# zhaihongjia/SplatLoc

Hardware: AMD Instinct MI355X
Metric: fwd+bwd frames/s @1080p, 500k Gaussians, 32 feat-ch; HBM GB/s vs roofline (higher is better)
Workload: dtype f32

## Files before the change

### include/splatraster.h

```cpp
#ifndef SPLATRASTER_H
#define SPLATRASTER_H

#include <stddef.h>
#include <stdint.h>

#ifdef __cplusplus
extern "C" {
#endif

#define SPLATRASTER_ABI_VERSION 14

#define SPLATRASTER_TILE 16

#define SPLATRASTER_OK 0
#define SPLATRASTER_ERR_BAD_ARG 1
#define SPLATRASTER_ERR_HIP 2
#define SPLATRASTER_ERR_UNSUPPORTED 3
#define SPLATRASTER_ERR_OVERFLOW 4
#define SPLATRASTER_WARN_LOOKBACK_STALL 5

typedef struct splatraster_settings {
    int32_t image_height;
    int32_t image_width;
    float tanfovx;
    float tanfovy;
    float scale_modifier;
    int32_t sh_degree;
    int32_t sh_coeffs;
    int32_t channels;
    int32_t bg_channels;
    int32_t prefiltered;
    int32_t debug;
} splatraster_settings;


size_t splatraster_geometry_bytes(int32_t P);
size_t splatraster_binning_bytes(int32_t P, int64_t R, int32_t width, int32_t height, int32_t channels);
size_t splatraster_image_bytes(int32_t width, int32_t height);


int splatraster_forward_geometry(const splatraster_settings* s, int32_t P,
                                 const float* means3D,
                                 const float* shs,
                                 const float* opacities,
                                 const float* scales,
                                 const float* rotations,
                                 const float* cov3D_precomp,
                                 const float* viewmatrix,
                                 const float* projmatrix,
                                 const float* campos,
                                 void* geometry, int32_t* radii, int64_t* num_rendered,
                                 void* stream);

int splatraster_forward_render(const splatraster_settings* s, int32_t P, int64_t R,
                               const float* bg,
                               const float* colors_precomp,
                               void* geometry, void* binning, void* image,
                               float* out_color, float* out_depth, float* out_alpha,
                               void* stream);


int splatraster_backward(const splatraster_settings* s, int32_t P, int64_t R,
                         const float* bg, const float* means3D, const float* shs,
                         const float* colors_precomp, const float* opacities,
                         const float* scales, const float* rotations,
                         const float* cov3D_precomp, const float* viewmatrix,
                         const float* projmatrix, const float* campos,
                         const int32_t* radii,
                         void* geometry ,
                         const void* binning, const void* image,
                         const float* out_color, const float* out_depth, const float* out_alpha,
                         const float* dL_dout_color,
                         const float* dL_dout_depth,
                         const float* dL_dout_alpha,
                         float* dL_dmeans3D,
                         float* dL_dmeans2D,
                         float* dL_dcolors,
                         float* dL_dopacities,
                         float* dL_dscales,
                         float* dL_drotations,
                         float* dL_dcov3D,
                         float* dL_dshs,
                         float* dL_dviewmatrix,
                         float* dL_dprojmatrix,
                         float* dL_dcampos,
                         void* stream);


#define SPLATRASTER_MAX_WINDOW_VIEWS 8

typedef struct splatraster_window_view {
    const float* viewmatrix;
    const float* projmatrix;
    const float* campos;
    float tanfovx, tanfovy;
    int32_t* radii;
    float* out_color;
    float* out_depth;
    float* out_alpha;
    const float* dL_dout_color;
    const float* dL_dout_depth;
    const float* dL_dout_alpha;
    float* dL_dmeans2D;
    const float* dL_dout_last;
    int32_t color_grad_channels;
} splatraster_window_view;

size_t splatraster_window_geometry_bytes(int32_t P, int32_t n_views);
size_t splatraster_window_binning_bytes(int32_t P, int32_t n_views, int64_t R_total, int32_t width, int32_t height,
                                        int32_t channels);
size_t splatraster_window_image_bytes(int32_t width, int32_t height, int32_t n_views);

int splatraster_forward_window_geometry(const splatraster_settings* s, int32_t n_views,
                                        const splatraster_window_view* views, int32_t P,
                                        const float* means3D, const float* opacities, const float* scales,
                                        const float* rotations, const float* cov3D_precomp, void* geometry,
                                        int64_t* num_rendered , void* stream);
int splatraster_forward_window_render(const splatraster_settings* s, int32_t n_views,
                                      const splatraster_window_view* views, int32_t P,
                                      const int64_t* num_rendered, const float* bg, const float* colors_precomp,
                                      void* geometry, void* binning, void* image, void* stream);
int splatraster_backward_window(const splatraster_settings* s, int32_t n_views, const splatraster_window_view* views,
                                int32_t P, const int64_t* num_rendered, const float* bg, const float* means3D,
                                const float* colors_precomp, const float* scales, const float* rotations,
                                const float* cov3D_precomp, void* geometry, const void* binning, const void* image,
                                float* dL_dmeans3D,
                                float* dL_dcolors,
                                float* dL_dopacities,
                                float* dL_dscales,
                                float* dL_drotations,
                                float* dL_dcov3D,
                                void* stream);

typedef struct splatraster_raw_forward {
    const float* scaling;
    const float* rotation;
    const float* opacity;
    const float* f_dc;
    const float* extra;
    int32_t extra_channels;
    float* scales;
    float* rotations;
    float* opacities;
    float* colors;
} splatraster_raw_forward;
int splatraster_forward_window_geometry_raw(const splatraster_settings* s, int32_t n_views, const splatraster_window_view* views,
                                            int32_t P, const float* means3D, const splatraster_raw_forward* raw, void* geometry,
                                            int64_t* num_rendered , void* stream);

typedef struct splatraster_raw_params {
    const float* scaling;
    const float* rotation;
    const float* opacity;
    const float* f_dc;
    int32_t extra_channels;
    float* dL_dscaling;
    float* dL_drotation;
    float* dL_dopacity;
    float* dL_df_dc;
    float* dL_dextra;
    const float* reg_row_grad;
    const float* reg_out;
    float reg_weight;
// ... 69 lines not shown
                                           float* max_radii2D, void* stream);


typedef struct splatraster_model {
    int32_t P;
    int32_t f_rest_width;
    int32_t marker_width;
    int32_t kp_width;
    int32_t scaling_width;
    float* xyz;
    float* f_dc;
    float* f_rest;
    float* opacity;
    float* marker;
    float* kp_score;
    float* scaling;
    float* rotation;
} splatraster_model;

size_t splatraster_densify_workspace_bytes(int32_t P);
int splatraster_densify_plan(const splatraster_model* model, const float* xyz_gradient_accum ,
                             const float* denom , float max_grad, float min_opacity, float extent,
                             float percent_dense, int32_t use_size_prune, int32_t primitive_reg, void* workspace,
                             int32_t* new_P, void* stream);
int splatraster_densify_apply(const splatraster_model* model, const splatraster_model* exp_avg ,
                              const splatraster_model* exp_avg_sq , const float* unit_noise ,
                              uint64_t seed, uint64_t draw_id, void* workspace , int32_t new_P,
                              splatraster_model* out_model, splatraster_model* out_exp_avg,
                              splatraster_model* out_exp_avg_sq, int32_t* source_row ,
                              int32_t* source_kind ,
                              void* stream);

int splatraster_model_append(const splatraster_model* model, const splatraster_model* exp_avg ,
                             const splatraster_model* exp_avg_sq , const splatraster_model* extra,
                             splatraster_model* out_model, splatraster_model* out_exp_avg,
                             splatraster_model* out_exp_avg_sq, void* stream);

typedef struct splatraster_adam_group {
    float* param;
    const float* grad;
    float* exp_avg;
    float* exp_avg_sq;
    const float* row_gate;
    int64_t numel;
    int32_t row_width;
    float lr;
    double step;
} splatraster_adam_group;
int splatraster_adam_step(int32_t n_groups, const splatraster_adam_group* groups, double beta1, double beta2, double eps,
                          float row_gate_threshold, void* stream);
int splatraster_adam_step_radii(int32_t n_groups, const splatraster_adam_group* groups, double beta1, double beta2, double eps,
                                float row_gate_threshold, int32_t P, const int32_t* radii, float* max_radii2D, void* stream);

size_t splatraster_isotropic_loss_workspace_bytes(int32_t P);
int splatraster_isotropic_loss(int32_t P, int32_t scaling_cols, const float* scaling, const float* marker,
                               float* row_grad , float* out , void* workspace, void* stream);


size_t splatraster_mapping_loss_workspace_bytes(int32_t pixels);
int splatraster_mapping_loss(int32_t pixels, const float* image, const float* depth, const float* marker,
                             const float* gt_image, const float* gt_depth, const float* kp,
                             float rgb_boundary_threshold, const float* exposure ,
                             float* g_image, float* g_depth, float* g_marker, float* out ,
                             void* workspace, void* stream);

typedef struct splatraster_loss_view {
    const float* image;
    const float* depth;
    const float* marker;
    const float* gt_image;
    const float* gt_depth;
    const float* kp;
    const float* exposure;
    float* g_image;
    float* g_depth;
    float* g_marker;
} splatraster_loss_view;
int splatraster_mapping_loss_window(int32_t n_views, int32_t pixels, const splatraster_loss_view* views,
                                    float rgb_boundary_threshold, float* out , void* workspace,
                                    void* stream);

size_t splatraster_refinement_loss_workspace_bytes(int32_t channels, int32_t height, int32_t width);
int splatraster_refinement_loss(int32_t channels, int32_t height, int32_t width, float lambda_dssim,
                                const float* image, const float* gt, float* g_image, float* out ,
                                void* workspace, void* stream);

size_t splatraster_eval_metrics_workspace_bytes(int32_t channels, int32_t height, int32_t width);
int splatraster_eval_metrics(int32_t channels, int32_t height, int32_t width, const float* render, const float* gt,
                             float* out , void* workspace, void* stream);


size_t splatknn_workspace_bytes(int32_t N);
int splatknn_dist2(int32_t N, const float* points , float* out ,
                   void* workspace, void* stream);

int splatknn_debug_set_grid_min(int32_t n);

#define SPLATRASTER_GRID_MAX_LEVELS 32
#define SPLATRASTER_GRID_HASH 0
#define SPLATRASTER_GRID_DENSE 1
#define SPLATRASTER_GRID_TILED 2
typedef struct splatraster_grid_layout {
    int32_t n_dims;
    int32_t n_levels;
    int32_t n_features;
    int32_t grid_type;
    uint32_t offset[SPLATRASTER_GRID_MAX_LEVELS];
    uint32_t size[SPLATRASTER_GRID_MAX_LEVELS];
    uint32_t resolution[SPLATRASTER_GRID_MAX_LEVELS];
    float scale[SPLATRASTER_GRID_MAX_LEVELS];
    int64_t n_params;
} splatraster_grid_layout;

int splatraster_grid_encoding_layout(int32_t n_dims, int32_t n_levels, int32_t n_features, int32_t log2_hashmap_size,
                                     int32_t base_resolution, double per_level_scale, int32_t grid_type,
                                     splatraster_grid_layout* out);
int splatraster_grid_encoding_forward(const splatraster_grid_layout* layout, int64_t N, const float* x, const float* params,
                                      float* out, void* stream);
int splatraster_grid_encoding_backward(const splatraster_grid_layout* layout, int64_t N, const float* x, const float* params,
                                       const float* dL_dout, float* dL_dparams, float* dL_dx, void* stream);

int splatraster_l1_rgbd_loss(int64_t n_color, const float* color, const float* target_color, int64_t n_depth, const float* depth,
                             const float* target_depth, float depth_weight, float* g_color, float* g_depth, float* loss_out,
                             void* stream);
int splatraster_pose_step(const float* dL_dviewmatrix, const float* dL_dprojmatrix, const float* dL_dcampos, const float* W2C_init,
                          const float* projection_matrix, float lr_rot, float lr_trans, float beta1, float beta2, float eps,
                          int advance, float* state, float* viewmatrix, float* projmatrix, float* campos, void* stream);


#define SPLATRASTER_STAGE_PREPROCESS 0
#define SPLATRASTER_STAGE_DEPTH_SORT 1
#define SPLATRASTER_STAGE_SCAN 2
#define SPLATRASTER_STAGE_EMIT 3
#define SPLATRASTER_STAGE_TILE_SORT 4
#define SPLATRASTER_STAGE_RANGES 5
#define SPLATRASTER_STAGE_COMPOSITE_FWD 6
#define SPLATRASTER_STAGE_COMPOSITE_BWD 7
#define SPLATRASTER_STAGE_PREPROCESS_BWD 8
#define SPLATRASTER_STAGE_PAYLOAD 9
#define SPLATRASTER_STAGE_COUNT 10

int splatraster_timing_enable(int on);
int splatraster_timing_select(uint32_t stage_mask);
int splatraster_timing_collect(double* ms, int64_t* counts);


int splatraster_poll_errors(void);
int splatraster_debug_set_spin_limit(uint32_t limit);
int splatraster_debug_set_deterministic(int on);
int splatraster_debug_set_small_panel_max_waves(int waves);
int splatraster_debug_set_split_max_waves(int waves);
int splatraster_debug_set_fwd_team(int mode);
int splatraster_debug_set_payload_stream_min(int64_t instances);
int splatraster_debug_set_front_end(int mode);
int splatraster_debug_set_tile_sort_cap(int keys);
int splatraster_debug_set_sort_fork(int mode);
int splatraster_debug_exp2(int64_t n, const float* x, float* y, void* stream);
int splatraster_debug_poison_lds(uint32_t pattern, void* stream);

const char* splatraster_error_string(int status);
const char* splatraster_last_hip_error(void);
int splatraster_abi_version(void);

#ifdef __cplusplus
}
#endif
#endif
```

### splatloc_amd/_native.py

```python
from __future__ import annotations

import ctypes as C
import os

from . import build as _build

_LIB = None
ABI_VERSION = 14

OK = 0
WARN_LOOKBACK_STALL = 5
_ERR_NAMES = {1: "bad argument", 2: "HIP runtime error", 3: "unsupported configuration",
              4: "tile instance count overflow", 5: "look-back stall (results late, never wrong)"}


class Settings(C.Structure):
    _fields_ = [
        ("image_height", C.c_int32),
        ("image_width", C.c_int32),
        ("tanfovx", C.c_float),
        ("tanfovy", C.c_float),
        ("scale_modifier", C.c_float),
        ("sh_degree", C.c_int32),
        ("sh_coeffs", C.c_int32),
        ("channels", C.c_int32),
        ("bg_channels", C.c_int32),
        ("prefiltered", C.c_int32),
        ("debug", C.c_int32),
    ]


MAX_WINDOW_VIEWS = 8


class WindowView(C.Structure):
    _fields_ = [("viewmatrix", C.c_void_p), ("projmatrix", C.c_void_p), ("campos", C.c_void_p),
                ("tanfovx", C.c_float), ("tanfovy", C.c_float),
                ("radii", C.c_void_p), ("out_color", C.c_void_p), ("out_depth", C.c_void_p), ("out_alpha", C.c_void_p),
                ("dL_dout_color", C.c_void_p), ("dL_dout_depth", C.c_void_p), ("dL_dout_alpha", C.c_void_p),
                ("dL_dmeans2D", C.c_void_p), ("dL_dout_last", C.c_void_p), ("color_grad_channels", C.c_int32)]


class LossView(C.Structure):
    _fields_ = [(n, C.c_void_p) for n in ("image", "depth", "marker", "gt_image", "gt_depth", "kp", "exposure", "g_image", "g_depth",
                                          "g_marker")]


class RawParams(C.Structure):
    _fields_ = [("scaling", C.c_void_p), ("rotation", C.c_void_p), ("opacity", C.c_void_p), ("f_dc", C.c_void_p),
                ("extra_channels", C.c_int32), ("dL_dscaling", C.c_void_p), ("dL_drotation", C.c_void_p), ("dL_dopacity", C.c_void_p),
                ("dL_df_dc", C.c_void_p), ("dL_dextra", C.c_void_p), ("reg_row_grad", C.c_void_p), ("reg_out", C.c_void_p),
                ("reg_weight", C.c_float)]


class RawForward(C.Structure):
    _fields_ = [("scaling", C.c_void_p), ("rotation", C.c_void_p), ("opacity", C.c_void_p), ("f_dc", C.c_void_p), ("extra", C.c_void_p),
                ("extra_channels", C.c_int32), ("scales", C.c_void_p), ("rotations", C.c_void_p), ("opacities", C.c_void_p),
                ("colors", C.c_void_p)]


class GeometryLayout(C.Structure):
    _fields_ = [(n, C.c_size_t) for n in
                ("rec0", "rec1", "tiles_touched", "depth_order", "offsets", "rgb", "clamped", "total")]


class BinningLayout(C.Structure):
    _fields_ = [(n, C.c_size_t) for n in ("point_list", "tile_list", "ranges", "total")]


class ImageLayout(C.Structure):
    _fields_ = [(n, C.c_size_t) for n in ("final_T", "n_contrib", "total")]


class Model(C.Structure):
    _fields_ = [("P", C.c_int32), ("f_rest_width", C.c_int32), ("marker_width", C.c_int32), ("kp_width", C.c_int32),
                ("scaling_width", C.c_int32)] + [(n, C.c_void_p) for n in
                                                 ("xyz", "f_dc", "f_rest", "opacity", "marker", "kp_score", "scaling",
                                                  "rotation")]


class AdamGroup(C.Structure):
    _fields_ = [("param", C.c_void_p), ("grad", C.c_void_p), ("exp_avg", C.c_void_p), ("exp_avg_sq", C.c_void_p),
                ("row_gate", C.c_void_p), ("numel", C.c_int64), ("row_width", C.c_int32), ("lr", C.c_float),
                ("step", C.c_double)]


GRID_MAX_LEVELS = 32
GRID_HASH, GRID_DENSE, GRID_TILED = 0, 1, 2


class GridLayout(C.Structure):
    _fields_ = [("n_dims", C.c_int32), ("n_levels", C.c_int32), ("n_features", C.c_int32), ("grid_type", C.c_int32),
                ("offset", C.c_uint32 * GRID_MAX_LEVELS), ("size", C.c_uint32 * GRID_MAX_LEVELS),
                ("resolution", C.c_uint32 * GRID_MAX_LEVELS), ("scale", C.c_float * GRID_MAX_LEVELS), ("n_params", C.c_int64)]


_vp, _i32, _i64, _sz = C.c_void_p, C.c_int32, C.c_int64, C.c_size_t
SYMBOLS = {
    "splatraster_geometry_bytes": (_sz, [_i32]),
    "splatraster_binning_bytes": (_sz, [_i32, _i64, _i32, _i32, _i32]),
    "splatraster_image_bytes": (_sz, [_i32, _i32]),
    "splatraster_forward_geometry": (C.c_int, [C.POINTER(Settings), _i32] + [_vp] * 9 + [_vp, _vp, C.POINTER(_i64), _vp]),
    "splatraster_forward_render": (C.c_int, [C.POINTER(Settings), _i32, _i64] + [_vp] * 9),
    "splatraster_backward": (C.c_int, [C.POINTER(Settings), _i32, _i64] + [_vp] * 33),
    "splatraster_window_geometry_bytes": (_sz, [_i32, _i32]),
    "splatraster_window_binning_bytes": (_sz, [_i32, _i32, _i64, _i32, _i32, _i32]),
    "splatraster_window_image_bytes": (_sz, [_i32, _i32, _i32]),
    "splatraster_forward_window_geometry": (C.c_int, [C.POINTER(Settings), _i32, C.POINTER(WindowView), _i32] + [_vp] * 6
                                            + [C.POINTER(_i64), _vp]),
    "splatraster_forward_window_render": (C.c_int, [C.POINTER(Settings), _i32, C.POINTER(WindowView), _i32, C.POINTER(_i64)]
                                          + [_vp] * 6),
    "splatraster_backward_window": (C.c_int, [C.POINTER(Settings), _i32, C.POINTER(WindowView), _i32, C.POINTER(_i64)]
                                    + [_vp] * 16),
    "splatraster_forward_window_geometry_raw": (C.c_int, [C.POINTER(Settings), _i32, C.POINTER(WindowView), _i32, _vp, C.POINTER(RawForward),
                                                          _vp, C.POINTER(_i64), _vp]),
    "splatraster_backward_window_raw": (C.c_int, [C.POINTER(Settings), _i32, C.POINTER(WindowView), _i32, C.POINTER(_i64)]
                                        + [_vp] * 8 + [C.POINTER(RawParams)] + [_vp] * 2),
    "splatraster_get_window_geometry_layout": (C.c_int, [_i32, _i32, C.POINTER(GeometryLayout)]),
    "splatraster_get_window_binning_layout": (C.c_int, [_i32, _i32, _i64, _i32, _i32, _i32, C.POINTER(BinningLayout)]),
    "splatraster_get_window_image_layout": (C.c_int, [_i32, _i32, _i32, C.POINTER(ImageLayout)]),
    "splatraster_debug_set_small_panel_max_waves": (C.c_int, [C.c_int]),
    "splatraster_debug_set_split_max_waves": (C.c_int, [C.c_int]),
    "splatraster_debug_set_fwd_team": (C.c_int, [C.c_int]),
    "splatraster_debug_set_front_end": (C.c_int, [C.c_int]),
    "splatraster_debug_set_tile_sort_cap": (C.c_int, [C.c_int]),
    "splatraster_debug_set_sort_fork": (C.c_int, [C.c_int]),
    "splatraster_debug_set_payload_stream_min": (C.c_int, [C.c_int64]),
    "splatraster_mark_visible": (C.c_int, [_i32, _vp, _vp, _vp, _vp, _vp]),
    "splatraster_get_geometry_layout": (C.c_int, [_i32, C.POINTER(GeometryLayout)]),
    "splatraster_get_binning_layout": (C.c_int, [_i32, _i64, _i32, _i32, _i32, C.POINTER(BinningLayout)]),
    "splatraster_get_image_layout": (C.c_int, [_i32, _i32, C.POINTER(ImageLayout)]),
    "splatraster_sort_tmp_bytes": (_sz, [_i64]),
    "splatraster_sort_pairs_u32": (C.c_int, [_i64, _vp, _vp, _i32, _vp, _vp]),
    "splatraster_timing_enable": (C.c_int, [C.c_int]),
    "splatraster_timing_select": (C.c_int, [C.c_uint32]),
    "splatraster_timing_collect": (C.c_int, [_vp, _vp]),
    "splatknn_workspace_bytes": (_sz, [_i32]),
    "splatknn_dist2": (C.c_int, [_i32, _vp, _vp, _vp, _vp]),
    "splatknn_debug_set_grid_min": (C.c_int, [_i32]),
    "splatraster_grid_encoding_layout": (C.c_int, [_i32] * 5 + [C.c_double, _i32, C.POINTER(GridLayout)]),
    "splatraster_grid_encoding_forward": (C.c_int, [C.POINTER(GridLayout), _i64, _vp, _vp, _vp, _vp]),
    "splatraster_grid_encoding_backward": (C.c_int, [C.POINTER(GridLayout), _i64] + [_vp] * 6),
    "splatraster_activate_forward": (C.c_int, [_i32] * 5 + [_vp] * 13),
    "splatraster_activate_backward": (C.c_int, [_i32] * 5 + [_vp] * 19),
    "splatraster_densification_stats": (C.c_int, [_i32] + [_vp] * 6),
    "splatraster_densification_stats_window": (C.c_int, [_i32, _i32] + [_vp] * 6),
    "splatraster_densify_workspace_bytes": (_sz, [_i32]),
    "splatraster_densify_plan": (C.c_int, [C.POINTER(Model), _vp, _vp, C.c_float, C.c_float, C.c_float, C.c_float, _i32,
                                           _i32, _vp, C.POINTER(_i32), _vp]),
    "splatraster_densify_apply": (C.c_int, [C.POINTER(Model), C.POINTER(Model), C.POINTER(Model), _vp, C.c_uint64,
                                            C.c_uint64, _vp, _i32, C.POINTER(Model), C.POINTER(Model), C.POINTER(Model),
                                            _vp, _vp, _vp]),
    "splatraster_model_append": (C.c_int, [C.POINTER(Model)] * 7 + [_vp]),
    "splatraster_adam_step": (C.c_int, [_i32, C.POINTER(AdamGroup), C.c_double, C.c_double, C.c_double, C.c_float, _vp]),
    "splatraster_adam_step_radii": (C.c_int, [_i32, C.POINTER(AdamGroup), C.c_double, C.c_double, C.c_double, C.c_float, _i32, _vp, _vp, _vp]),
    "splatraster_isotropic_loss_workspace_bytes": (_sz, [_i32]),
    "splatraster_isotropic_loss": (C.c_int, [_i32, _i32, _vp, _vp, _vp, _vp, _vp, _vp]),
    "splatraster_mapping_loss_workspace_bytes": (_sz, [_i32]),
    "splatraster_mapping_loss": (C.c_int, [_i32] + [_vp] * 6 + [C.c_float] + [_vp] * 7),
    "splatraster_mapping_loss_window": (C.c_int, [_i32, _i32, _vp, C.c_float, _vp, _vp, _vp]),
    "splatraster_refinement_loss_workspace_bytes": (_sz, [_i32, _i32, _i32]),
    "splatraster_refinement_loss": (C.c_int, [_i32, _i32, _i32, C.c_float] + [_vp] * 6),
    "splatraster_eval_metrics_workspace_bytes": (_sz, [_i32, _i32, _i32]),
    "splatraster_eval_metrics": (C.c_int, [_i32, _i32, _i32] + [_vp] * 5),
    "splatraster_l1_rgbd_loss": (C.c_int, [_i64, _vp, _vp, _i64, _vp, _vp, C.c_float, _vp, _vp, _vp, _vp]),
    "splatraster_pose_step": (C.c_int, [_vp] * 5 + [C.c_float] * 5 + [C.c_int] + [_vp] * 5),
    "splatraster_error_string": (C.c_char_p, [C.c_int]),
    "splatraster_last_hip_error": (C.c_char_p, []),
    "splatraster_abi_version": (C.c_int, []),
    "splatraster_poll_errors": (C.c_int, []),
    "splatraster_debug_set_spin_limit": (C.c_int, [C.c_uint32]),
    "splatraster_debug_set_deterministic": (C.c_int, [C.c_int]),
    "splatraster_debug_exp2": (C.c_int, [_i64, _vp, _vp, _vp]),
    "splatraster_debug_poison_lds": (C.c_int, [C.c_uint32, _vp]),
}


def lib_path() -> str:
    return _build.LIB_PATH


def load(build_if_missing: bool = True):
    global _LIB
    if _LIB is not None:
        return _LIB
    path = os.environ.get("SPLATRASTER_LIB", _build.LIB_PATH)
    if path == _build.LIB_PATH and build_if_missing and _build.have_hipcc():
        try:
            _build.build()
        except Exception as e:
            raise RuntimeError(
                "splatloc_amd: the HIP extension libsplatraster.so could not be built "
                f"({e}). There is no CPU fallback.") from e
    if not os.path.exists(path):
        raise RuntimeError(f"{path} is missing and hipcc is not available: run `python -m splatloc_amd.build` "
                           "on a machine with ROCm. There is no CPU fallback.")
    lib = C.CDLL(path)
    lib.splatraster_abi_version.restype = C.c_int
    got = int(lib.splatraster_abi_version())
    if got != ABI_VERSION:
        raise RuntimeError(f"{path} has ABI version {got}, this binding needs {ABI_VERSION}: stale library, "
                           "rebuild with `python -m splatloc_amd.build --force`")
    for name, (res, args) in SYMBOLS.items():
        fn = getattr(lib, name)
        fn.restype = res
        fn.argtypes = args
    _LIB = lib
    if os.environ.get("SPLATRASTER_SPLIT_MAX_WAVES"):
        lib.splatraster_debug_set_split_max_waves(int(os.environ["SPLATRASTER_SPLIT_MAX_WAVES"]))
    if os.environ.get("SPLATRASTER_FWD_TEAM"):
        lib.splatraster_debug_set_fwd_team(int(os.environ["SPLATRASTER_FWD_TEAM"]))
    if os.environ.get("SPLATRASTER_FRONT_END"):
        lib.splatraster_debug_set_front_end(int(os.environ["SPLATRASTER_FRONT_END"]))
    if os.environ.get("SPLATRASTER_TILE_SORT_CAP"):
        lib.splatraster_debug_set_tile_sort_cap(int(os.environ["SPLATRASTER_TILE_SORT_CAP"]))
    if os.environ.get("SPLATRASTER_SORT_FORK"):
        lib.splatraster_debug_set_sort_fork(int(os.environ["SPLATRASTER_SORT_FORK"]))
    if os.environ.get("SPLATRASTER_SMALL_PANEL_MAX_WAVES"):
        lib.splatraster_debug_set_small_panel_max_waves(int(os.environ["SPLATRASTER_SMALL_PANEL_MAX_WAVES"]))
    return lib


def check(status: int, what: str) -> None:
    if status != OK:
        lib = load()
        detail = lib.splatraster_last_hip_error().decode() if status in (2, 5) else ""
        raise RuntimeError(f"{what} failed: {_ERR_NAMES.get(status, status)} {detail}".strip())


STAGES = ("preprocess", "depth_sort", "scan", "emit", "tile_sort", "ranges", "composite_fwd", "composite_bwd",
          "preprocess_bwd", "payload")


def timing_enable(on: bool) -> None:
    check(load().splatraster_timing_enable(int(on)), "timing_enable")


def timing_select(stages) -> None:
    mask = 0
    for st in stages:
        mask |= 1 << STAGES.index(st)
    check(load().splatraster_timing_select(mask), "timing_select")


def timing_collect() -> dict:
    n = len(STAGES)
    ms = (C.c_double * n)()
    cnt = (C.c_int64 * n)()
    check(load().splatraster_timing_collect(ms, cnt), "timing_collect")
    return {s: (ms[i], cnt[i]) for i, s in enumerate(STAGES)}


def set_deterministic(on: bool) -> None:
    check(load().splatraster_debug_set_deterministic(int(bool(on))), "set_deterministic")


def set_front_end(mode: int) -> None:
    check(load().splatraster_debug_set_front_end(int(mode)), "set_front_end")


def poll_stall() -> bool:
    st = load().splatraster_poll_errors()
    if st == WARN_LOOKBACK_STALL:
        return True
    check(st, "poll_errors")
    return False
```

### splatloc_amd/csrc/binning.hip

```cpp
#include "tile_order.h"
#include "composite_common.h"

namespace sr {

__device__ __forceinline__ int f2i_sat_b(float v)
{
    if (!(v > -1.0e9f)) v = -1.0e9f;
    if (!(v < 1.0e9f)) v = 1.0e9f;
    return (int)v;
}

constexpr int EMIT_BLOCK = 256;
constexpr int EMIT_IPT = 4;
static_assert(EMIT_SPAN == EMIT_BLOCK * EMIT_IPT, "common.h: EMIT_SPAN");

__global__ void __launch_bounds__(EMIT_BLOCK)
emit_kernel(int64_t R, int P , int Pv , int tiles_per_view, int W, int H,
            const uint32_t* __restrict__ offsets,
            const uint32_t* __restrict__ depth_order, const float4* __restrict__ rec,
            uint32_t* __restrict__ keys, uint32_t* __restrict__ vals,
            const uint32_t* __restrict__ span_owner ,
            uint32_t* __restrict__ ranges, uint32_t nranges )
{
    for (uint32_t w = blockIdx.x * blockDim.x + threadIdx.x; w < nranges; w += gridDim.x * blockDim.x) ranges[w] = 0u;
    __shared__ uint32_t s_off[EMIT_SPAN + 1];
    __shared__ uint32_t s_gid[EMIT_SPAN], s_org[EMIT_SPAN], s_w[EMIT_SPAN];
    __shared__ int s_min;
    const int t = threadIdx.x;
    const int64_t j0 = (int64_t)blockIdx.x * EMIT_SPAN;
    const uint32_t j0u = (uint32_t)j0;
    int lo = 0, hi = P;
    if (span_owner && blockIdx.x < SPAN_OWNER_CAP) {
        lo = (int)span_owner[blockIdx.x];
        hi = lo + 1;
    }
    while (hi - lo > 1) {
        const int n = hi - lo;
        const int step = (n + EMIT_BLOCK - 1) / EMIT_BLOCK;
        if (t == 0) s_min = EMIT_BLOCK;
        __syncthreads();
        const int last = lo + (t + 1) * step - 1;
        if (last >= hi - 1 || offsets[last] > j0u) atomicMin(&s_min, t);
        __syncthreads();
        const int seg = s_min;
        __syncthreads();
        lo = lo + seg * step;
        hi = min(hi, lo + step);
    }
    const int r_lo = lo;
    for (int q = t; q <= EMIT_SPAN; q += EMIT_BLOCK) {
        const int r = r_lo - 1 + q;
        s_off[q] = r < 0 ? 0u : offsets[min(r, P - 1)];
    }
    __syncthreads();
    const int gx = (W + TILE - 1) / TILE, gy = (H + TILE - 1) / TILE;
    const uint32_t j_last = (uint32_t)(min(R, j0 + (int64_t)EMIT_SPAN) - 1);
    int nr;
    {
        int a = 1, b = EMIT_SPAN + 1;
        while (a < b) {
            const int mid = (a + b) >> 1;
            if (s_off[mid] > j_last) b = mid; else a = mid + 1;
        }
        nr = a;
    }
    for (int q = t; q < nr; q += EMIT_BLOCK) {
        const uint32_t g = depth_order[r_lo + q] & 0xFFFFFFu;
        const float4 p = rec[2 * g];
        const float rf = p.w;
        const int rminx = min(gx, max(0, f2i_sat_b((p.x - rf) / (float)TILE)));
        const int rminy = min(gy, max(0, f2i_sat_b((p.y - rf) / (float)TILE)));
        const int rmaxx = min(gx, max(0, f2i_sat_b((p.x + rf + (float)(TILE - 1)) / (float)TILE)));
        s_gid[q] = g;
        const uint32_t v = (P == Pv) ? 0u : g / (uint32_t)Pv;
        s_org[q] = v * (uint32_t)tiles_per_view + (uint32_t)rminy * (uint32_t)gx + (uint32_t)rminx;
        s_w[q] = (uint32_t)(rmaxx - rminx);
    }
    __syncthreads();
#pragma unroll
    for (int it = 0; it < EMIT_IPT; ++it) {
        const int64_t j = j0 + it * EMIT_BLOCK + t;
        if (j < R) {
            const uint32_t ju = (uint32_t)j;
            int a = 1, b = nr + 1;
            while (a < b) {
                const int mid = (a + b) >> 1;
                if (s_off[mid] > ju) b = mid; else a = mid + 1;
            }
            const uint32_t k = ju - s_off[a - 1];
            const uint32_t w = s_w[a - 1];
            const uint32_t row = k / w;
            keys[j] = s_org[a - 1] + row * (uint32_t)gx + (k - row * w);
            vals[j] = s_gid[a - 1];
        }
    }
}

int launch_emit(const splatraster_settings& s, int32_t P, int32_t V, int64_t R, const GeomView& g, uint32_t* keys,
                uint32_t* vals, uint32_t* ranges, uint32_t nranges, hipStream_t stream)
{
    if (R == 0) return SPLATRASTER_OK;
    const int64_t blocks = (R + EMIT_SPAN - 1) / EMIT_SPAN;
    const int n = P * V;
    const int tiles = ((s.image_width + TILE - 1) / TILE) * ((s.image_height + TILE - 1) / TILE);
    hipLaunchKernelGGL(emit_kernel, dim3((unsigned)blocks), dim3(EMIT_BLOCK), 0, stream, R, n, P, tiles, s.image_width,
                       s.image_height, g.offsets, g.depth_order, g.rec, keys, vals,
                       scan_state_bytes(n) ? g.span_owner : nullptr, ranges, nranges);
    SR_LAUNCH_CHECK();
    return SPLATRASTER_OK;
}

int launch_ranges_clear(int32_t tiles, uint32_t* ranges, hipStream_t stream)
{
    SR_HIP_CHECK(hipMemsetAsync(ranges, 0, sizeof(uint32_t) * 2 * (size_t)tiles, stream));
    return SPLATRASTER_OK;
}

#ifndef SR_PAYLOAD_NT_MIN
#define SR_PAYLOAD_NT_MIN (8ll << 20)
#endif
static int64_t g_payload_stream_min = SR_PAYLOAD_NT_MIN;
void set_payload_stream_min(int64_t instances) { g_payload_stream_min = instances < 0 ? (int64_t)SR_PAYLOAD_NT_MIN : instances; }

template <bool NT>
__global__ void __launch_bounds__(256)
payload_kernel(int64_t R, int gx, int tiles_per_view, int V, const uint32_t* __restrict__ point_list,
               const uint32_t* __restrict__ tile_list, const float4* __restrict__ rec,
               float4* __restrict__ irec, uint32_t* __restrict__ ipack, uint32_t* __restrict__ ranges)
{
    const int64_t j = (int64_t)blockIdx.x * blockDim.x + threadIdx.x;
    if (j >= R) return;
    const uint32_t g = point_list[j], t = tile_list[j];
    const float4 a0 = rec[2 * (size_t)g], a1 = rec[2 * (size_t)g + 1];
    uint32_t tl = t;
#pragma unroll 1
    for (int v = 1; v < V && tl >= (uint32_t)tiles_per_view; ++v) tl -= (uint32_t)tiles_per_view;
    const uint32_t ty = tl / (uint32_t)gx, tx = tl - ty * (uint32_t)gx;
    const float4 c1 = payload_conic(a1);
    const uint32_t m = g | (quadrant_reach_mask(a0, a1, (float)(tx * TILE), (float)(ty * TILE)) << 24);
    if (NT) {
        typedef float f32x4_t __attribute__((ext_vector_type(4)));
        f32x4_t* out = reinterpret_cast<f32x4_t*>(irec) + 2 * j;
        __builtin_nontemporal_store((f32x4_t){a0.x, a0.y, a0.z, a0.w}, out);
        __builtin_nontemporal_store((f32x4_t){c1.x, c1.y, c1.z, c1.w}, out + 1);
        __builtin_nontemporal_store(m, ipack + j);
    } else {
        irec[2 * j] = a0;
        irec[2 * j + 1] = c1;
        ipack[j] = m;
    }
    if (j == 0 || tile_list[j - 1] != t) ranges[2 * t] = (uint32_t)j;
    if (j == R - 1 || tile_list[j + 1] != t) ranges[2 * t + 1] = (uint32_t)(j + 1);
}

int launch_payload(const splatraster_settings& s, int32_t V, int64_t R, const GeomView& g, const BinView& b, hipStream_t stream)
{
    if (R == 0) return SPLATRASTER_OK;
    const int gx = (s.image_width + TILE - 1) / TILE, gy = (s.image_height + TILE - 1) / TILE;
    if (R >= g_payload_stream_min)
        hipLaunchKernelGGL(payload_kernel<true>, dim3((unsigned)((R + 255) / 256)), dim3(256), 0, stream, R, gx, gx * gy, V,
                           b.point_list, b.tile_list, g.rec, b.irec, b.ipack, b.ranges);
    else
        hipLaunchKernelGGL(payload_kernel<false>, dim3((unsigned)((R + 255) / 256)), dim3(256), 0, stream, R, gx, gx * gy, V,
                           b.point_list, b.tile_list, g.rec, b.irec, b.ipack, b.ranges);
    SR_LAUNCH_CHECK();
    return SPLATRASTER_OK;
}

__global__ void __launch_bounds__(ORDER_THREADS)
tile_order_kernel(int T, const uint32_t* __restrict__ ranges, uint32_t* __restrict__ order, uint32_t* __restrict__ nparts)
{
    __shared__ uint32_t s_cnt[ORDER_BUCKETS];
    __shared__ uint32_t s_wsum[ORDER_THREADS / WAVE];
    tile_order_block(T, [&](int i) { return ranges[2 * i + 1] - ranges[2 * i]; }, order, s_cnt, s_wsum, nparts);
}

int launch_tile_order(const splatraster_settings& s, int32_t V, const BinView& b, hipStream_t stream)
{
    const int gx = (s.image_width + TILE - 1) / TILE, gy = (s.image_height + TILE - 1) / TILE;
    if (!use_tile_order(V, gx * gy)) return SPLATRASTER_OK;
    hipLaunchKernelGGL(tile_order_kernel, dim3(1), dim3(ORDER_THREADS), 0, stream, V * gx * gy, b.ranges, b.tile_order, b.nparts);
    SR_LAUNCH_CHECK();
    return SPLATRASTER_OK;
}

__global__ void __launch_bounds__(256)
pad_features_kernel(int64_t n4 , int C, int PPR, const float* __restrict__ feat,
                    float4* __restrict__ featp4)
{
    const int64_t e = (int64_t)blockIdx.x * blockDim.x + threadIdx.x;
    if (e >= n4) return;
    const int64_t row = e / PPR;
    const int c = (int)(e - row * PPR) * 4;
    const float* src = feat + row * C + c;
    float4 v;
    v.x = src[0];
    v.y = c + 1 < C ? src[1] : 0.0f;
    v.z = c + 2 < C ? src[2] : 0.0f;
    v.w = c + 3 < C ? src[3] : 0.0f;
    featp4[e] = v;
}

int launch_pad_features(int32_t P, int C, const float* feat, float* featp, hipStream_t stream)
{
    const int CP = padded_channels(C);
    const int64_t n4 = (int64_t)P * CP / 4;
    if (n4 == 0 || CP == C) return SPLATRASTER_OK;
    hipLaunchKernelGGL(pad_features_kernel, dim3((unsigned)((n4 + 255) / 256)), dim3(256), 0, stream, n4, C, CP / 4,
                       feat, reinterpret_cast<float4*>(featp));
    SR_LAUNCH_CHECK();
    return SPLATRASTER_OK;
}

}
```

### splatloc_amd/csrc/capi.hip

```cpp
#include <string.h>

#include <mutex>
#include <unordered_map>
#include <string>
#include <vector>

#include "common.h"

namespace sr {

static thread_local std::string g_last_error;
static int g_deterministic = 0;
static int g_split_max_waves = SPLIT_MAX_WAVES;
void set_split_max_waves(int waves) { g_split_max_waves = waves < 0 ? SPLIT_MAX_WAVES : (waves > SPLIT_MAX_WAVES ? SPLIT_MAX_WAVES : waves); }
int split_max_waves() { return g_split_max_waves; }

void set_hip_error(hipError_t e, const char* what)
{
    g_last_error = std::string(what) + ": " + hipGetErrorString(e);
}

void set_error_text(const char* text) { g_last_error = text; }

struct StageRec { int stage; hipEvent_t a, b; };
static uint32_t g_timing_mask = 0;
static std::mutex g_timing_mu;
static std::vector<StageRec> g_recs;
static std::vector<hipEvent_t> g_pool;

static hipEvent_t get_event()
{
    if (!g_pool.empty()) { hipEvent_t e = g_pool.back(); g_pool.pop_back(); return e; }
    hipEvent_t e = nullptr;
    if (hipEventCreate(&e) != hipSuccess) return nullptr;
    return e;
}

struct StageTimer {
    hipStream_t stream;
    StageRec rec{};
    bool on;
    StageTimer(int stage, hipStream_t s) : stream(s), on((g_timing_mask >> stage) & 1u)
    {
        if (!on) return;
        std::lock_guard<std::mutex> lk(g_timing_mu);
        rec.stage = stage; rec.a = get_event(); rec.b = get_event();
        if (!rec.a || !rec.b) { on = false; return; }
        (void)hipEventRecord(rec.a, stream);
    }
    ~StageTimer()
    {
        if (!on) return;
        (void)hipEventRecord(rec.b, stream);
        std::lock_guard<std::mutex> lk(g_timing_mu);
        g_recs.push_back(rec);
    }
};

struct HostSlot {
    uint32_t* p = nullptr;
    uint32_t* dp = nullptr;
    size_t cap = 0;
    hipEvent_t ev = nullptr;
    int device = -1;
};
static thread_local HostSlot t_slot;

static int host_slot(size_t n, HostSlot** out)
{
    HostSlot& s = t_slot;
    int dev = 0;
    SR_HIP_CHECK(hipGetDevice(&dev));
    if (s.cap < n) {
        if (s.p) (void)hipHostFree(s.p);
        s.p = nullptr;
        s.dp = nullptr;
        s.cap = 0;
        const size_t cap = n < 4096 ? 4096 : n + n / 2;
        SR_HIP_CHECK(hipHostMalloc(reinterpret_cast<void**>(&s.p), sizeof(uint32_t) * cap, hipHostMallocMapped | hipHostMallocPortable | hipHostMallocCoherent));
        SR_HIP_CHECK(hipHostGetDevicePointer(reinterpret_cast<void**>(&s.dp), s.p, 0));
        s.cap = cap;
    }
    if (!s.ev || s.device != dev) {
        if (s.ev) (void)hipEventDestroy(s.ev);
        s.ev = nullptr;
        SR_HIP_CHECK(hipEventCreateWithFlags(&s.ev, hipEventDisableTiming));
        s.device = dev;
    }
    *out = &s;
    return SPLATRASTER_OK;
}

static inline int tile_bits(int tiles)
{
    int b = 1;
    while ((1 << b) < tiles) ++b;
    return b;
}

struct GeomLayout {
    size_t rec0, rec1, tiles_touched, depth_order, offsets, rgb, clamped, sort_keys, keys_alt, vals_alt,
        sort_tmp, scan_tmp, total, block_tiles, span_owner, bytes;
};
static GeomLayout geom_layout(int32_t P, int32_t V)
{
    const size_t p1 = (size_t)(P > 0 ? P : 1);
    const size_t n = p1 * (size_t)(V > 0 ? V : 1);
    GeomLayout L;
    size_t o = 0;
    auto take = [&](size_t bytes) { size_t at = o; o = align_up(o + bytes, 256); return at; };
    L.rec0 = take(32 * n);
    L.rec1 = L.rec0 + 16;
    L.tiles_touched = take(4 * n);
    L.depth_order = take(4 * n);
    L.offsets = take(4 * n);
    L.rgb = take(12 * p1);
    L.clamped = take(3 * p1);
    L.sort_keys = take(4 * n);
    L.keys_alt = take(4 * n);
    L.vals_alt = take(4 * n);
    L.sort_tmp = take(sort_tmp_bytes((int64_t)n));
    L.scan_tmp = take(scan_tmp_bytes((int64_t)n));
    L.total = take(16);
    L.block_tiles = take(4 * (size_t)preprocess_blocks((int32_t)p1) * (size_t)(V > 0 ? V : 1));
    L.span_owner = take(4 * (size_t)SPAN_OWNER_CAP);
    L.bytes = o;
    return L;
}

GeomView geom_view(void* base, int32_t P, int32_t V)
{
    const GeomLayout L = geom_layout(P, V);
    char* b = reinterpret_cast<char*>(base);
    GeomView g;
    g.rec = reinterpret_cast<float4*>(b + L.rec0);
    g.tiles_touched = reinterpret_cast<uint32_t*>(b + L.tiles_touched);
    g.depth_order = reinterpret_cast<uint32_t*>(b + L.depth_order);
    g.offsets = reinterpret_cast<uint32_t*>(b + L.offsets);
    g.rgb = reinterpret_cast<float*>(b + L.rgb);
    g.clamped = reinterpret_cast<uint8_t*>(b + L.clamped);
    g.sort_keys = reinterpret_cast<uint32_t*>(b + L.sort_keys);
    g.sort_tmp = reinterpret_cast<uint32_t*>(b + L.sort_tmp);
    g.total = reinterpret_cast<uint32_t*>(b + L.total);
    g.block_tiles = reinterpret_cast<uint32_t*>(b + L.block_tiles);
    g.span_owner = reinterpret_cast<uint32_t*>(b + L.span_owner);
    return g;
}

struct BinLayout {
    size_t keysA, valsA, keysB, valsB, ranges, sort_tmp, irec, ipack, featp, gacc, pose_acc, ckpt, tile_order, nparts, bytes;
};
static BinLayout bin_layout(int32_t P, int32_t V, int64_t R, int32_t W, int32_t H, int32_t C)
{
    const size_t n = (size_t)(R > 0 ? R : 1);
    const size_t nv = (size_t)(V > 0 ? V : 1);
    const size_t tiles = (size_t)((W + TILE - 1) / TILE) * (size_t)((H + TILE - 1) / TILE) * nv;
    BinLayout L;
    size_t o = 0;
    auto take = [&](size_t bytes) { size_t at = o; o = align_up(o + bytes, 256); return at; };
    L.valsA = take(4 * n);
    L.keysA = take(4 * n);
    L.keysB = take(4 * n);
    L.valsB = take(4 * n);
    L.ranges = take(8 * (tiles > 0 ? tiles : 1));
    L.sort_tmp = take(sort_tmp_bytes((int64_t)n));
    L.irec = take(32 * n);
    L.ipack = take(4 * n);
    L.featp = take((C % 4) ? (size_t)(P > 0 ? P : 1) * padded_channels(C) * sizeof(float) : 16);
    L.gacc = take((size_t)(P > 0 ? P : 1) * nv * gacc_row_floats(C) * sizeof(float));
    L.pose_acc = take(POSE_ACC_BYTES);
    const bool ck = C <= 4 && 4 * (size_t)tiles <= (size_t)SPLIT_MAX_WAVES;
    L.ckpt = take(ck ? nv * (size_t)SPLIT_PARTS_MAX * (size_t)(C + 2) * (size_t)W * (size_t)H * sizeof(float) : 16);
    L.tile_order = take(4 * (tiles > 0 ? tiles : 1));
    L.nparts = take(4 * (tiles > 0 ? tiles : 1));
    L.bytes = o;
    return L;
}

BinView bin_view(void* base, int32_t P, int32_t V, int64_t R, int32_t W, int32_t H, int32_t C)
{
    const BinLayout L = bin_layout(P, V, R, W, H, C);
    char* b = reinterpret_cast<char*>(base);
    BinView v;
    v.point_list = reinterpret_cast<uint32_t*>(b + L.valsA);
    v.tile_list = reinterpret_cast<uint32_t*>(b + L.keysA);
    v.keys_tmp = reinterpret_cast<uint32_t*>(b + L.keysB);
    v.vals_tmp = reinterpret_cast<uint32_t*>(b + L.valsB);
    v.ranges = reinterpret_cast<uint32_t*>(b + L.ranges);
    v.sort_tmp = b + L.sort_tmp;
    v.irec = reinterpret_cast<float4*>(b + L.irec);
    v.ipack = reinterpret_cast<uint32_t*>(b + L.ipack);
    v.featp = reinterpret_cast<float*>(b + L.featp);
    v.gacc = reinterpret_cast<float*>(b + L.gacc);
    v.pose_acc = reinterpret_cast<float*>(b + L.pose_acc);
    v.ckpt = reinterpret_cast<float*>(b + L.ckpt);
    v.tile_order = reinterpret_cast<uint32_t*>(b + L.tile_order);
    v.nparts = reinterpret_cast<uint32_t*>(b + L.nparts);
    return v;
}

static size_t img_plane_bytes(int32_t W, int32_t H, int32_t V)
{
    return align_up((size_t)W * H * 4 * (size_t)(V > 0 ? V : 1), 256);
}

ImgView img_view(void* base, int32_t W, int32_t H, int32_t V)
{
    char* b = reinterpret_cast<char*>(base);
    ImgView v;
    v.final_T = reinterpret_cast<float*>(b);
    v.n_contrib = reinterpret_cast<uint32_t*>(b + img_plane_bytes(W, H, V));
    return v;
}

static int check_row_index_range(int32_t P, int32_t V, int32_t C)
{
    const uint64_t row = (uint64_t)(gacc_row_floats(C) > padded_channels(C) ? gacc_row_floats(C) : padded_channels(C));
    const uint64_t n = (uint64_t)P * (uint64_t)V;
    if (n > (1ull << 24) || n * row >= (1ull << 32)) return SPLATRASTER_ERR_UNSUPPORTED;
    return SPLATRASTER_OK;
}

static int check_settings(const splatraster_settings* s)
{
    if (!s) return SPLATRASTER_ERR_BAD_ARG;
    if (s->image_width <= 0 || s->image_height <= 0 || s->channels <= 0) return SPLATRASTER_ERR_BAD_ARG;
    if (s->bg_channels < 0) return SPLATRASTER_ERR_BAD_ARG;
    return SPLATRASTER_OK;
}

}

using namespace sr;

extern "C" {

int splatraster_abi_version(void) { return SPLATRASTER_ABI_VERSION; }

const char* splatraster_error_string(int status)
{
    switch (status) {
        case SPLATRASTER_OK: return "ok";
        case SPLATRASTER_ERR_BAD_ARG: return "bad argument";
        case SPLATRASTER_ERR_HIP: return "HIP runtime error";
        case SPLATRASTER_ERR_UNSUPPORTED: return "unsupported configuration";
        case SPLATRASTER_ERR_OVERFLOW: return "tile instance count overflow";
        case SPLATRASTER_WARN_LOOKBACK_STALL: return "look-back stall (results late, never wrong)";
        default: return "unknown status";
    }
}

const char* splatraster_last_hip_error(void) { return g_last_error.c_str(); }

size_t splatraster_geometry_bytes(int32_t P) { return geom_layout(P, 1).bytes; }
size_t splatraster_binning_bytes(int32_t P, int64_t R, int32_t width, int32_t height, int32_t channels)
{
    return bin_layout(P, 1, R, width, height, channels).bytes;
}
size_t splatraster_image_bytes(int32_t width, int32_t height) { return 2 * img_plane_bytes(width, height, 1); }

size_t splatraster_window_geometry_bytes(int32_t P, int32_t n_views) { return geom_layout(P, n_views).bytes; }
size_t splatraster_window_binning_bytes(int32_t P, int32_t n_views, int64_t R_total, int32_t width, int32_t height,
                                        int32_t channels)
{
    return bin_layout(P, n_views, R_total, width, height, channels).bytes;
}
size_t splatraster_window_image_bytes(int32_t width, int32_t height, int32_t n_views)
{
    return 2 * img_plane_bytes(width, height, n_views);
}

int splatraster_get_geometry_layout(int32_t P, splatraster_geometry_layout* out)
{
    return splatraster_get_window_geometry_layout(P, 1, out);
}
int splatraster_get_window_geometry_layout(int32_t P, int32_t n_views, splatraster_geometry_layout* out)
{
    if (!out || n_views < 1 || n_views > MAX_VIEWS) return SPLATRASTER_ERR_BAD_ARG;
    const GeomLayout L = geom_layout(P, n_views);
    out->rec0 = L.rec0; out->rec1 = L.rec1; out->tiles_touched = L.tiles_touched;
    out->depth_order = L.depth_order; out->offsets = L.offsets; out->rgb = L.rgb;
    out->clamped = L.clamped; out->total = L.bytes;
    return SPLATRASTER_OK;
}
int splatraster_get_binning_layout(int32_t P, int64_t R, int32_t width, int32_t height, int32_t channels,
                                   splatraster_binning_layout* out)
{
    return splatraster_get_window_binning_layout(P, 1, R, width, height, channels, out);
}
int splatraster_get_window_binning_layout(int32_t P, int32_t n_views, int64_t R_total, int32_t width, int32_t height,
                                          int32_t channels, splatraster_binning_layout* out)
{
    if (!out || n_views < 1 || n_views > MAX_VIEWS) return SPLATRASTER_ERR_BAD_ARG;
    const BinLayout L = bin_layout(P, n_views, R_total, width, height, channels);
    out->point_list = L.valsA; out->tile_list = L.keysA; out->ranges = L.ranges; out->total = L.bytes;
    return SPLATRASTER_OK;
}
int splatraster_get_image_layout(int32_t width, int32_t height, splatraster_image_layout* out)
{
    return splatraster_get_window_image_layout(width, height, 1, out);
}
int splatraster_get_window_image_layout(int32_t width, int32_t height, int32_t n_views, splatraster_image_layout* out)
{
    if (!out || n_views < 1 || n_views > MAX_VIEWS) return SPLATRASTER_ERR_BAD_ARG;
    out->final_T = 0;
    out->n_contrib = img_plane_bytes(width, height, n_views);
    out->total = 2 * img_plane_bytes(width, height, n_views);
    return SPLATRASTER_OK;
}

}

namespace sr {

static int check_window(const splatraster_settings* s, int32_t V, const splatraster_window_view* views)
{
    int st = check_settings(s);
    if (st) return st;
    if (V < 1 || V > MAX_VIEWS || !views) return SPLATRASTER_ERR_BAD_ARG;
    return SPLATRASTER_OK;
}

static WinCams make_cams(int32_t V, const splatraster_window_view* views)
{
    WinCams c{};
    for (int v = 0; v < V; ++v) {
        c.view[v] = views[v].viewmatrix;
        c.proj[v] = views[v].projmatrix;
        c.campos[v] = views[v].campos;
        c.tanfovx[v] = views[v].tanfovx;
        c.tanfovy[v] = views[v].tanfovy;
        c.radii[v] = views[v].radii;
    }
    return c;
}

struct BinScratch { bool on; uint32_t* table; void* scan_tmp; int64_t entries; };

static std::mutex g_front_end_mu;
static std::unordered_map<const void*, bool> g_front_end;
static void front_end_record(const void* geometry, bool on)
{
    std::lock_guard<std::mutex> lk(g_front_end_mu);
    if (g_front_end.size() > (1u << 14)) g_front_end.clear();
    g_front_end[geometry] = on;
}
static int front_end_recorded(const void* geometry)
{
    std::lock_guard<std::mutex> lk(g_front_end_mu);
    auto it = g_front_end.find(geometry);
    return it == g_front_end.end() ? -1 : (it->second ? 1 : 0);
}

static BinScratch bin_scratch(const splatraster_settings& s, int32_t P, int32_t V, void* geometry, bool geometry_stage)
{
    const int gx = (s.image_width + TILE - 1) / TILE, gy = (s.image_height + TILE - 1) / TILE, tiles = gx * gy;
    const GeomLayout L = geom_layout(P, V);
    BinScratch b{};
    if (!geometry || P <= 0) return b;
    const int recorded = geometry_stage ? -1 : front_end_recorded(geometry);
    b.on = recorded >= 0 ? recorded == 1 : use_bins(P, V, gx, gy, L.total - L.sort_keys);
    if (geometry_stage) front_end_record(geometry, b.on);
    if (!b.on) return b;
    char* base = reinterpret_cast<char*>(geometry);
    b.entries = (int64_t)bin_table_entries(P, V, tiles);
    b.table = reinterpret_cast<uint32_t*>(base + L.sort_keys);
    b.scan_tmp = base + L.sort_keys + align_up((size_t)b.entries * sizeof(uint32_t), 256);
    return b;
}

static int window_geometry(const splatraster_settings* s, int32_t V, const splatraster_window_view* views, int32_t P,
                           const float* means3D, const float* shs, const float* opacities, const float* scales,
                           const float* rotations, const float* cov3D_precomp, void* geometry, int64_t* num_rendered,
                           hipStream_t stream, const RawFwd* raw = nullptr)
{
    int st = check_window(s, V, views);
    if (st) return st;
    if (P < 0 || !num_rendered) return SPLATRASTER_ERR_BAD_ARG;
    for (int v = 0; v < V; ++v) num_rendered[v] = 0;
    if (P == 0) return SPLATRASTER_OK;
    if (raw) {
        if (shs || cov3D_precomp || !raw->scaling || !raw->rotation || !raw->opacity || !raw->f_dc || !raw->scales || !raw->rotations ||
            !raw->opacities || !raw->colors || raw->E != s->channels - 3 || (raw->E > 0 && !raw->extra))
            return SPLATRASTER_ERR_BAD_ARG;
        opacities = raw->opacities; scales = raw->scales; rotations = raw->rotations;
    }
    if (!means3D || !opacities || !geometry) return SPLATRASTER_ERR_BAD_ARG;
    for (int v = 0; v < V; ++v)
        if (!views[v].viewmatrix || !views[v].projmatrix || !views[v].radii) return SPLATRASTER_ERR_BAD_ARG;
    const bool have_sr = scales && rotations;
    if (have_sr == (cov3D_precomp != nullptr)) return SPLATRASTER_ERR_BAD_ARG;
    if ((scales == nullptr) != (rotations == nullptr)) return SPLATRASTER_ERR_BAD_ARG;
    if (shs) {
        if (V != 1) return SPLATRASTER_ERR_UNSUPPORTED;
        if (s->channels != 3 || !views[0].campos) return SPLATRASTER_ERR_BAD_ARG;
        if (s->sh_degree < 0 || s->sh_degree > 3) return SPLATRASTER_ERR_UNSUPPORTED;
        if (s->sh_coeffs < (s->sh_degree + 1) * (s->sh_degree + 1)) return SPLATRASTER_ERR_BAD_ARG;
    }
    if ((int64_t)P * V >= ((int64_t)1 << 31)) return SPLATRASTER_ERR_OVERFLOW;
    st = check_row_index_range(P, V, s->channels);
    if (st) return st;
    st = lookback_error_init();
    if (st) return st;
    const int32_t n = P * V;
    const GeomLayout L = geom_layout(P, V);
    GeomView g = geom_view(geometry, P, V);
    char* base = reinterpret_cast<char*>(geometry);
    const WinCams cams = make_cams(V, views);
    const BinScratch bins = bin_scratch(*s, P, V, geometry, true);
    HostSlot* slot = nullptr;
    const size_t nblk = (size_t)preprocess_blocks(P);
    st = host_slot(nblk * (size_t)V, &slot);
    if (st) return st;
    g.block_tiles = slot->dp;
    struct SlotGuard {
        HostSlot* slot; hipStream_t stream; int state;
        ~SlotGuard() { if (state == 2) (void)hipEventSynchronize(slot->ev); else if (state == 1) (void)hipStreamSynchronize(stream); }
    } guard{slot, stream, 1};
    {
        StageTimer t(SPLATRASTER_STAGE_PREPROCESS, stream);
        if (bins.on)
            st = launch_preprocess(*s, P, V, cams, means3D, shs, opacities, scales, rotations, cov3D_precomp, g, nullptr, 0u,
                                   reinterpret_cast<uint32_t*>(bins.scan_tmp), (uint32_t)(scan_state_bytes(bins.entries) / 4),
                                   stream, false, raw);
        else
            st = launch_preprocess(*s, P, V, cams, means3D, shs, opacities, scales, rotations, cov3D_precomp, g,
                                   g.sort_tmp, (uint32_t)(sort_zero_bytes(n, 32) / 4),
                                   reinterpret_cast<uint32_t*>(base + L.scan_tmp), (uint32_t)(scan_state_bytes(n) / 4), stream, true, raw);
    }
    if (st) return st;
    SR_HIP_CHECK(hipEventRecord(slot->ev, stream));
    guard.state = 2;
    if (bins.on) {
        StageTimer t(SPLATRASTER_STAGE_DEPTH_SORT, stream);
        st = launch_bin_count(*s, P, V, g, bins.table, bins.scan_tmp, stream);
        if (st) return st;
    } else {
    {
        StageTimer t(SPLATRASTER_STAGE_DEPTH_SORT, stream);
        bool in_alt = false;
        uint32_t* keys_alt = reinterpret_cast<uint32_t*>(base + L.keys_alt);
        uint32_t* vals_alt = reinterpret_cast<uint32_t*>(base + L.vals_alt);
        st = sort_pairs_u32(n, g.sort_keys, g.depth_order, keys_alt, vals_alt, 32, g.sort_tmp, stream, &in_alt, true);
        if (st) return st;
        if (in_alt) return SPLATRASTER_ERR_UNSUPPORTED;
    }
    {
        StageTimer t(SPLATRASTER_STAGE_SCAN, stream);
        st = inclusive_scan_u32(n, g.tiles_touched, g.depth_order, g.offsets, g.total, base + L.scan_tmp, stream, true,
                                g.span_owner, (uint32_t)EMIT_SPAN, SPAN_OWNER_CAP);
    }
    if (st) return st;
    }
    SR_HIP_CHECK(hipEventSynchronize(slot->ev));
    guard.state = 0;
    uint64_t total = 0;
    for (int v = 0; v < V; ++v) {
        uint64_t tv = 0;
        for (size_t k = 0; k < nblk; ++k) tv += slot->p[(size_t)v * nblk + k];
        num_rendered[v] = (int64_t)tv;
        total += tv;
    }
    if (total >= ((uint64_t)1 << 31)) return SPLATRASTER_ERR_OVERFLOW;
    return SPLATRASTER_OK;
}

static int window_render(const splatraster_settings* s, int32_t V, const splatraster_window_view* views, int32_t P,
                         int64_t R, const float* bg, const float* colors_precomp, void* geometry, void* binning,
                         void* image, hipStream_t stream)
{
    int st = check_window(s, V, views);
    if (st) return st;
    if (P < 0 || R < 0 || !image) return SPLATRASTER_ERR_BAD_ARG;
    for (int v = 0; v < V; ++v)
        if (!views[v].out_color || !views[v].out_depth || !views[v].out_alpha) return SPLATRASTER_ERR_BAD_ARG;
    if (s->bg_channels > 0 && !bg) return SPLATRASTER_ERR_BAD_ARG;
    if (P > 0 && (!geometry || !binning)) return SPLATRASTER_ERR_BAD_ARG;
    if (V > 1 && !colors_precomp && P > 0) return SPLATRASTER_ERR_UNSUPPORTED;
    st = check_row_index_range(P, V, s->channels);
    if (st) return st;
    if (!binning) return SPLATRASTER_ERR_BAD_ARG;
    const int W = s->image_width, H = s->image_height;
    const int tiles = ((W + TILE - 1) / TILE) * ((H + TILE - 1) / TILE);
    const int64_t gtiles = (int64_t)tiles * V;
    if (gtiles >= ((int64_t)1 << 31)) return SPLATRASTER_ERR_OVERFLOW;
    ImgView im = img_view(image, W, H, V);
    GeomView g{};
    if (geometry) g = geom_view(geometry, P, V);
    BinView b = bin_view(binning, P, V, R, W, H, s->channels);
    const float* feat = colors_precomp ? colors_precomp : g.rgb;
    if (R > 0 && !feat) return SPLATRASTER_ERR_BAD_ARG;
    const int bits = tile_bits((int)gtiles);
    const int passes = (bits + 7) / 8;
    uint32_t* k0 = (passes & 1) ? b.keys_tmp : b.tile_list;
    uint32_t* v0 = (passes & 1) ? b.vals_tmp : b.point_list;
    uint32_t* k1 = (passes & 1) ? b.tile_list : b.keys_tmp;
    uint32_t* v1 = (passes & 1) ? b.point_list : b.vals_tmp;
    const BinScratch bins = bin_scratch(*s, P, V, geometry, false);
    if (R > 0 && bins.on) {
        StageTimer t(SPLATRASTER_STAGE_TILE_SORT, stream);
        st = launch_bin_scatter_sort(*s, P, V, R, g, bins.table, b, reinterpret_cast<uint64_t*>(b.keys_tmp), stream);
        if (st) return st;
    }
    if (R > 0 && !bins.on) {
        {
            StageTimer t(SPLATRASTER_STAGE_EMIT, stream);
            st = launch_emit(*s, P, V, R, g, k0, v0, b.ranges, 2u * (uint32_t)gtiles, stream);
        }
        if (st) return st;
        bool in_alt = false;
        {
            StageTimer t(SPLATRASTER_STAGE_TILE_SORT, stream);
            st = sort_pairs_u32(R, k0, v0, k1, v1, bits, b.sort_tmp, stream, &in_alt);
        }
        if (st) return st;
    }
    if (R == 0) {
        StageTimer t(SPLATRASTER_STAGE_RANGES, stream);
        st = launch_ranges_clear((int32_t)gtiles, b.ranges, stream);
    }
    if (st) return st;
    const float* featp = feat;
    if (R > 0) {
        StageTimer t(SPLATRASTER_STAGE_PAYLOAD, stream);
        if (!bins.on) st = launch_payload(*s, V, R, g, b, stream);
        if (st) return st;
        if (s->channels % 4) {
            st = launch_pad_features(P, s->channels, feat, b.featp, stream);
            featp = b.featp;
        }
    }
    if (st) return st;
    if (!(R > 0 && bins.on)) {
        StageTimer t(SPLATRASTER_STAGE_RANGES, stream);
        st = launch_tile_order(*s, V, b, stream);
    }
    if (st) return st;
    WinOut outs{};
    for (int v = 0; v < V; ++v) {
        outs.color[v] = views[v].out_color;
        outs.depth[v] = views[v].out_depth;
        outs.alpha[v] = views[v].out_alpha;
    }
    StageTimer t(SPLATRASTER_STAGE_COMPOSITE_FWD, stream);
    return launch_composite_fwd(*s, P, V, R, g, b, im, featp, bg, outs, stream);
}

static int window_backward(const splatraster_settings* s, int32_t V, const splatraster_window_view* views, int32_t P,
                           int64_t R, const float* bg, const float* means3D, const float* shs, const float* colors_precomp,
                           const float* scales, const float* rotations, const float* cov3D_precomp, void* geometry,
                           const void* binning, const void* image, float* dL_dmeans3D, float* dL_dcolors,
                           float* dL_dopacities, float* dL_dscales, float* dL_drotations, float* dL_dcov3D,
                           float* dL_dshs, float* dL_dviewmatrix, float* dL_dprojmatrix, float* dL_dcampos,
                           hipStream_t stream, const RawBwd* raw = nullptr)
{
    int st = check_window(s, V, views);
    if (st) return st;
    if (P < 0 || R < 0) return SPLATRASTER_ERR_BAD_ARG;
    if (V > 1 && (shs || dL_dviewmatrix || dL_dprojmatrix || dL_dcampos)) return SPLATRASTER_ERR_UNSUPPORTED;
    if (raw && (shs || cov3D_precomp || dL_dviewmatrix || dL_dprojmatrix || dL_dcampos)) return SPLATRASTER_ERR_UNSUPPORTED;
    if (P == 0) {
        if (dL_dviewmatrix) SR_HIP_CHECK(hipMemsetAsync(dL_dviewmatrix, 0, 16 * sizeof(float), stream));
        if (dL_dprojmatrix) SR_HIP_CHECK(hipMemsetAsync(dL_dprojmatrix, 0, 16 * sizeof(float), stream));
        if (dL_dcampos) SR_HIP_CHECK(hipMemsetAsync(dL_dcampos, 0, 3 * sizeof(float), stream));
        return SPLATRASTER_OK;
    }
    if (!means3D || !geometry || !binning || !image || !dL_dmeans3D || (!dL_dopacities && !raw)) return SPLATRASTER_ERR_BAD_ARG;
    if (raw && (P > 0) && (!raw->scaling || !raw->rotation || !raw->opacity || !raw->f_dc || !raw->d_scaling || !raw->d_rotation ||
                           !raw->d_opacity || !raw->d_f_dc || raw->E != s->channels - 3 || (raw->E > 0 && !raw->d_extra)))
        return SPLATRASTER_ERR_BAD_ARG;
    for (int v = 0; v < V; ++v)
        if (!views[v].viewmatrix || !views[v].projmatrix || !views[v].radii || !views[v].out_color || !views[v].out_depth ||
            !views[v].dL_dout_color || !views[v].dL_dmeans2D)
            return SPLATRASTER_ERR_BAD_ARG;
    if (shs && (!dL_dshs || !views[0].campos)) return SPLATRASTER_ERR_BAD_ARG;
    if (!shs && (!colors_precomp || (!dL_dcolors && !raw))) return SPLATRASTER_ERR_BAD_ARG;
    if (cov3D_precomp ? !dL_dcov3D : (!scales || !rotations || ((!dL_dscales || !dL_drotations) && !raw)))
        return SPLATRASTER_ERR_BAD_ARG;
    st = check_row_index_range(P, V, s->channels);
    if (st) return st;
    const int W = s->image_width, H = s->image_height;
    GeomView g = geom_view(geometry, P, V);
    BinView b = bin_view(const_cast<void*>(binning), P, V, R, W, H, s->channels);
    ImgView im = img_view(const_cast<void*>(image), W, H, V);
    const int C = s->channels;
    const float* feat = shs ? g.rgb : colors_precomp;
    const WinCams cams = make_cams(V, views);
    WinGrad grads{};
    grads.gc = C;
    for (int v = 0; v < V; ++v) {
        const int gcv = views[v].color_grad_channels;
        if (gcv < 0 || gcv > C) return SPLATRASTER_ERR_BAD_ARG;
        if (gcv != 0 && gcv < C) grads.gc = gcv;
    }
    for (int v = 0; v < V; ++v) {
        const int gcv = views[v].color_grad_channels ? views[v].color_grad_channels : C;
        if (gcv != grads.gc) return SPLATRASTER_ERR_BAD_ARG;
        grads.dL_dlast[v] = grads.gc < C ? views[v].dL_dout_last : nullptr;
    }
    for (int v = 0; v < V; ++v) {
        grads.out_color[v] = views[v].out_color;
        grads.out_depth[v] = views[v].out_depth;
        grads.dL_dcolor[v] = views[v].dL_dout_color;
        grads.dL_ddepth[v] = views[v].dL_dout_depth;
        grads.dL_dalpha[v] = views[v].dL_dout_alpha;
        grads.dL_dmeans2D[v] = views[v].dL_dmeans2D;
    }
    const size_t gacc_n = (size_t)gacc_row_floats(C) * (size_t)P * (size_t)V;
    const bool det = g_deterministic != 0;
    long long* gacc64 = nullptr;
    if (det) {
        SR_HIP_CHECK(hipMallocAsync(reinterpret_cast<void**>(&gacc64), sizeof(long long) * gacc_n, stream));
        SR_HIP_CHECK(hipMemsetAsync(gacc64, 0, sizeof(long long) * gacc_n, stream));
    }
    const bool pose = dL_dviewmatrix && dL_dprojmatrix;
    const size_t fill = pose ? (size_t)(reinterpret_cast<char*>(b.pose_acc) - reinterpret_cast<char*>(b.gacc)) + POSE_ACC_BYTES
                             : sizeof(float) * gacc_n;
    SR_HIP_CHECK(hipMemsetAsync(b.gacc, 0, fill, stream));
    grads.bg = bg;
    grads.bg_channels = bg ? s->bg_channels : 0;
    {
        StageTimer t(SPLATRASTER_STAGE_COMPOSITE_BWD, stream);
        if (det) st = launch_composite_bwd(*s, P, V, R, g, b, im, (C % 4) ? b.featp : feat, C, grads, b.gacc, gacc64, 0, stream);
        if (!st) st = launch_composite_bwd(*s, P, V, R, g, b, im, (C % 4) ? b.featp : feat, C, grads, b.gacc, gacc64, 1, stream);
    }
    if (det) {
        if (!st) st = launch_fixed_to_float((int64_t)gacc_n, gacc64, b.gacc, stream);
        (void)hipFreeAsync(gacc64, stream);
    }
    if (st) return st;
    StageTimer t(SPLATRASTER_STAGE_PREPROCESS_BWD, stream);
    return launch_preprocess_bwd(*s, P, V, cams, grads, means3D, shs, scales, rotations, cov3D_precomp, g.clamped, g.rec,
                                 b.gacc, C, shs ? nullptr : dL_dcolors, dL_dmeans3D, dL_dopacities,
                                 cov3D_precomp ? nullptr : dL_dscales, cov3D_precomp ? nullptr : dL_drotations,
                                 cov3D_precomp ? dL_dcov3D : nullptr, dL_dshs, dL_dviewmatrix, dL_dprojmatrix, dL_dcampos,
                                 b.pose_acc, stream, raw);
}

}

extern "C" {

int splatraster_forward_geometry(const splatraster_settings* s, int32_t P, const float* means3D,
                                 const float* shs, const float* opacities, const float* scales,
                                 const float* rotations, const float* cov3D_precomp,
                                 const float* viewmatrix, const float* projmatrix, const float* campos,
                                 void* geometry, int32_t* radii, int64_t* num_rendered, void* stream_)
{
    if (!s) return SPLATRASTER_ERR_BAD_ARG;
    splatraster_window_view w{};
    w.viewmatrix = viewmatrix; w.projmatrix = projmatrix; w.campos = campos;
    w.tanfovx = s->tanfovx; w.tanfovy = s->tanfovy; w.radii = radii;
    if (num_rendered) *num_rendered = 0;
    if (P > 0 && !radii) return SPLATRASTER_ERR_BAD_ARG;
    return window_geometry(s, 1, &w, P, means3D, shs, opacities, scales, rotations, cov3D_precomp, geometry, num_rendered,
                           reinterpret_cast<hipStream_t>(stream_));
}

int splatraster_forward_render(const splatraster_settings* s, int32_t P, int64_t R, const float* bg,
                               const float* colors_precomp, void* geometry, void* binning, void* image,
                               float* out_color, float* out_depth, float* out_alpha, void* stream_)
{
    if (!s) return SPLATRASTER_ERR_BAD_ARG;
    splatraster_window_view w{};
    w.tanfovx = s->tanfovx; w.tanfovy = s->tanfovy;
    w.out_color = out_color; w.out_depth = out_depth; w.out_alpha = out_alpha;
    return window_render(s, 1, &w, P, R, bg, colors_precomp, geometry, binning, image, reinterpret_cast<hipStream_t>(stream_));
}

int splatraster_backward(const splatraster_settings* s, int32_t P, int64_t R, const float* bg,
                         const float* means3D, const float* shs, const float* colors_precomp,
                         const float* opacities, const float* scales, const float* rotations,
                         const float* cov3D_precomp, const float* viewmatrix, const float* projmatrix,
                         const float* campos, const int32_t* radii, void* geometry,
                         const void* binning, const void* image, const float* out_color,
                         const float* out_depth, const float* out_alpha, const float* dL_dout_color,
                         const float* dL_dout_depth, const float* dL_dout_alpha, float* dL_dmeans3D,
                         float* dL_dmeans2D, float* dL_dcolors, float* dL_dopacities, float* dL_dscales,
                         float* dL_drotations, float* dL_dcov3D, float* dL_dshs, float* dL_dviewmatrix,
                         float* dL_dprojmatrix, float* dL_dcampos, void* stream_)
{
    (void)opacities; (void)out_alpha;
    if (!s) return SPLATRASTER_ERR_BAD_ARG;
    splatraster_window_view w{};
    w.viewmatrix = viewmatrix; w.projmatrix = projmatrix; w.campos = campos;
    w.tanfovx = s->tanfovx; w.tanfovy = s->tanfovy; w.radii = const_cast<int32_t*>(radii);
    w.out_color = const_cast<float*>(out_color); w.out_depth = const_cast<float*>(out_depth);
    w.dL_dout_color = dL_dout_color; w.dL_dout_depth = dL_dout_depth; w.dL_dout_alpha = dL_dout_alpha;
    w.dL_dmeans2D = dL_dmeans2D;
    return window_backward(s, 1, &w, P, R, bg, means3D, shs, colors_precomp, scales, rotations, cov3D_precomp, geometry, binning,
                           image, dL_dmeans3D, dL_dcolors, dL_dopacities, dL_dscales, dL_drotations, dL_dcov3D, dL_dshs,
                           dL_dviewmatrix, dL_dprojmatrix, dL_dcampos, reinterpret_cast<hipStream_t>(stream_));
}

int splatraster_forward_window_geometry(const splatraster_settings* s, int32_t n_views, const splatraster_window_view* views,
                                        int32_t P, const float* means3D, const float* opacities, const float* scales,
                                        const float* rotations, const float* cov3D_precomp, void* geometry,
                                        int64_t* num_rendered, void* stream)
{
    return window_geometry(s, n_views, views, P, means3D, nullptr, opacities, scales, rotations, cov3D_precomp, geometry,
                           num_rendered, reinterpret_cast<hipStream_t>(stream));
}

int splatraster_forward_window_render(const splatraster_settings* s, int32_t n_views, const splatraster_window_view* views,
                                      int32_t P, const int64_t* num_rendered, const float* bg, const float* colors_precomp,
                                      void* geometry, void* binning, void* image, void* stream)
{
    if (!num_rendered || n_views < 1 || n_views > MAX_VIEWS) return SPLATRASTER_ERR_BAD_ARG;
    int64_t R = 0;
    for (int v = 0; v < n_views; ++v) {
        if (num_rendered[v] < 0) return SPLATRASTER_ERR_BAD_ARG;
        R += num_rendered[v];
    }
    return window_render(s, n_views, views, P, R, bg, colors_precomp, geometry, binning, image,
                         reinterpret_cast<hipStream_t>(stream));
}

int splatraster_backward_window(const splatraster_settings* s, int32_t n_views, const splatraster_window_view* views,
                                int32_t P, const int64_t* num_rendered, const float* bg, const float* means3D, const float* colors_precomp,
                                const float* scales, const float* rotations, const float* cov3D_precomp, void* geometry,
                                const void* binning, const void* image, float* dL_dmeans3D, float* dL_dcolors,
                                float* dL_dopacities, float* dL_dscales, float* dL_drotations, float* dL_dcov3D, void* stream)
{
    if (!num_rendered || n_views < 1 || n_views > MAX_VIEWS) return SPLATRASTER_ERR_BAD_ARG;
    int64_t R = 0;
    for (int v = 0; v < n_views; ++v) {
        if (num_rendered[v] < 0) return SPLATRASTER_ERR_BAD_ARG;
        R += num_rendered[v];
    }
    return window_backward(s, n_views, views, P, R, bg, means3D, nullptr, colors_precomp, scales, rotations, cov3D_precomp,
                           geometry, binning, image, dL_dmeans3D, dL_dcolors, dL_dopacities, dL_dscales, dL_drotations,
                           dL_dcov3D, nullptr, nullptr, nullptr, nullptr, reinterpret_cast<hipStream_t>(stream));
}

int splatraster_forward_window_geometry_raw(const splatraster_settings* s, int32_t n_views, const splatraster_window_view* views,
                                            int32_t P, const float* means3D, const splatraster_raw_forward* rf, void* geometry,
                                            int64_t* num_rendered, void* stream)
{
    if (!rf) return SPLATRASTER_ERR_BAD_ARG;
    const RawFwd raw{rf->scaling, rf->rotation, rf->opacity, rf->f_dc, rf->extra, rf->extra_channels, rf->scales, rf->rotations,
                     rf->opacities, rf->colors};
    return window_geometry(s, n_views, views, P, means3D, nullptr, nullptr, nullptr, nullptr, nullptr, geometry, num_rendered,
                           reinterpret_cast<hipStream_t>(stream), &raw);
}

int splatraster_backward_window_raw(const splatraster_settings* s, int32_t n_views, const splatraster_window_view* views,
                                    int32_t P, const int64_t* num_rendered, const float* bg, const float* means3D,
                                    const float* colors_precomp, const float* scales, const float* rotations, void* geometry,
                                    const void* binning, const void* image, const splatraster_raw_params* rp, float* dL_dmeans3D,
                                    void* stream)
{
    if (!num_rendered || n_views < 1 || n_views > MAX_VIEWS || !rp) return SPLATRASTER_ERR_BAD_ARG;
    int64_t R = 0;
    for (int v = 0; v < n_views; ++v) {
        if (num_rendered[v] < 0) return SPLATRASTER_ERR_BAD_ARG;
        R += num_rendered[v];
    }
    if (rp->reg_row_grad && !rp->reg_out) return SPLATRASTER_ERR_BAD_ARG;
    const RawBwd raw{rp->scaling, rp->rotation, rp->opacity, rp->f_dc, rp->extra_channels, rp->dL_dscaling, rp->dL_drotation,
                     rp->dL_dopacity, rp->dL_df_dc, rp->dL_dextra, rp->reg_row_grad, rp->reg_out, rp->reg_weight};
    return window_backward(s, n_views, views, P, R, bg, means3D, nullptr, colors_precomp, scales, rotations, nullptr,
                           geometry, binning, image, dL_dmeans3D, nullptr, nullptr, nullptr, nullptr, nullptr, nullptr, nullptr,
                           nullptr, nullptr, reinterpret_cast<hipStream_t>(stream), &raw);
}

int splatraster_debug_set_small_panel_max_waves(int waves)
{
    set_small_panel_max_waves(waves);
    return SPLATRASTER_OK;
}

int splatraster_debug_set_payload_stream_min(int64_t instances)
{
    sr::set_payload_stream_min(instances);
    return SPLATRASTER_OK;
}

int splatraster_debug_set_front_end(int mode)
{
    set_bin_mode(mode);
    return SPLATRASTER_OK;
}

int splatraster_debug_set_sort_fork(int mode)
{
    set_bin_fork(mode);
    return SPLATRASTER_OK;
}

int splatraster_debug_set_tile_sort_cap(int keys)
{
    set_bin_tile_cap(keys);
    return SPLATRASTER_OK;
}

int splatraster_debug_set_split_max_waves(int waves)
{
    set_split_max_waves(waves);
    return SPLATRASTER_OK;
}

int splatraster_debug_set_fwd_team(int mode)
{
    set_fwd_team(mode < 0 ? -1 : (mode > 2 ? 2 : mode));
    return SPLATRASTER_OK;
}

int splatraster_mark_visible(int32_t P, const float* means3D, const float* viewmatrix,
                             const float* projmatrix, uint8_t* present, void* stream)
{
    (void)projmatrix;
    if (P < 0) return SPLATRASTER_ERR_BAD_ARG;
    if (P == 0) return SPLATRASTER_OK;
    if (!means3D || !viewmatrix || !present) return SPLATRASTER_ERR_BAD_ARG;
    return launch_mark_visible(P, means3D, viewmatrix, present, reinterpret_cast<hipStream_t>(stream));
}

int splatraster_poll_errors(void) { return lookback_error_poll(); }

int splatraster_debug_set_deterministic(int on)
{
    g_deterministic = on ? 1 : 0;
    return SPLATRASTER_OK;
}

int splatraster_debug_set_spin_limit(uint32_t limit)
{
    int st = lookback_error_init();
    if (st) return st;
    return lookback_set_spin_limit(limit);
}

int splatraster_debug_exp2(int64_t n, const float* x, float* y, void* stream)
{
    if (n < 0) return SPLATRASTER_ERR_BAD_ARG;
    if (n == 0) return SPLATRASTER_OK;
    if (!x || !y) return SPLATRASTER_ERR_BAD_ARG;
    return launch_debug_exp2(n, x, y, reinterpret_cast<hipStream_t>(stream));
}

int splatraster_debug_poison_lds(uint32_t pattern, void* stream)
{
    return launch_poison_lds(pattern, reinterpret_cast<hipStream_t>(stream));
}

size_t splatraster_sort_tmp_bytes(int64_t n)
{
    const size_t m = (size_t)(n > 0 ? n : 1);
    return align_up(4 * m, 256) * 2 + sort_tmp_bytes(n);
}

int splatraster_sort_pairs_u32(int64_t n, uint32_t* keys, uint32_t* vals, int32_t key_bits, void* tmp,
                               void* stream_)
{
    if (n < 0 || key_bits < 0 || key_bits > 32) return SPLATRASTER_ERR_BAD_ARG;
    if (n == 0 || key_bits == 0) return SPLATRASTER_OK;
    if (!keys || !vals || !tmp) return SPLATRASTER_ERR_BAD_ARG;
    {
        int st0 = lookback_error_init();
        if (st0) return st0;
    }
    hipStream_t stream = reinterpret_cast<hipStream_t>(stream_);
    char* t = reinterpret_cast<char*>(tmp);
    const size_t stride = align_up(4 * (size_t)n, 256);
    uint32_t* ka = reinterpret_cast<uint32_t*>(t);
    uint32_t* va = reinterpret_cast<uint32_t*>(t + stride);
    bool in_alt = false;
    int st = sort_pairs_u32(n, keys, vals, ka, va, key_bits, t + 2 * stride, stream, &in_alt);
    if (st) return st;
    if (in_alt) {
        SR_HIP_CHECK(hipMemcpyAsync(keys, ka, 4 * (size_t)n, hipMemcpyDeviceToDevice, stream));
        SR_HIP_CHECK(hipMemcpyAsync(vals, va, 4 * (size_t)n, hipMemcpyDeviceToDevice, stream));
    }
    return SPLATRASTER_OK;
}

int splatraster_timing_enable(int on)
{
    std::lock_guard<std::mutex> lk(g_timing_mu);
    g_timing_mask = on ? 0xffffffffu : 0u;
    return SPLATRASTER_OK;
}

int splatraster_timing_select(uint32_t stage_mask)
{
    std::lock_guard<std::mutex> lk(g_timing_mu);
    g_timing_mask = stage_mask;
    return SPLATRASTER_OK;
}

int splatraster_timing_collect(double* ms, int64_t* counts)
{
    if (!ms || !counts) return SPLATRASTER_ERR_BAD_ARG;
    std::lock_guard<std::mutex> lk(g_timing_mu);
    for (const StageRec& r : g_recs) {
        SR_HIP_CHECK(hipEventSynchronize(r.b));
        float t = 0.f;
        SR_HIP_CHECK(hipEventElapsedTime(&t, r.a, r.b));
        if (r.stage >= 0 && r.stage < SPLATRASTER_STAGE_COUNT) { ms[r.stage] += (double)t; counts[r.stage] += 1; }
        g_pool.push_back(r.a);
        g_pool.push_back(r.b);
    }
    g_recs.clear();
    return SPLATRASTER_OK;
}

size_t splatknn_workspace_bytes(int32_t N) { return knn_workspace_bytes(N); }

static int check_activate(int32_t P, int32_t K, int32_t deg, int32_t SC, int32_t E, const void* f_rest,
                          const void* extra)
{
    if (P < 0 || K < 1 || deg < 0 || E < 0) return SPLATRASTER_ERR_BAD_ARG;
    if (deg > 3) return SPLATRASTER_ERR_UNSUPPORTED;
    if ((deg + 1) * (deg + 1) > K) return SPLATRASTER_ERR_BAD_ARG;
    if (SC != 1 && SC != 3) return SPLATRASTER_ERR_BAD_ARG;
    if (P > 0 && K > 1 && !f_rest) return SPLATRASTER_ERR_BAD_ARG;
    if (P > 0 && E > 0 && !extra) return SPLATRASTER_ERR_BAD_ARG;
    return SPLATRASTER_OK;
}

int splatraster_activate_forward(int32_t P, int32_t sh_coeffs, int32_t active_sh_degree, int32_t scaling_cols,
                                 int32_t extras, const float* xyz, const float* f_dc, const float* f_rest,
                                 const float* scaling, const float* rotation, const float* opacity,
                                 const float* extra, const float* campos, float* scales, float* rotations,
                                 float* opacities, float* colors, void* stream)
{
    int st = check_activate(P, sh_coeffs, active_sh_degree, scaling_cols, extras, f_rest, extra);
    if (st) return st;
    if (P == 0) return SPLATRASTER_OK;
    if (!xyz || !f_dc || !scaling || !rotation || !opacity || !scales || !rotations || !opacities || !colors)
// ... 169 lines not shown
```

### splatloc_amd/csrc/common.h

```cpp
#pragma once
#include <hip/hip_runtime.h>
#include <stdint.h>

#include "../../include/splatraster.h"

namespace sr {

constexpr int TILE = SPLATRASTER_TILE;
constexpr int TILE_PIX = TILE * TILE;
constexpr float NEAR_Z = 0.2f;
constexpr float DILATION = 0.3f;
constexpr float ALPHA_MAX = 0.99f;
constexpr float ALPHA_MIN = 1.0f / 255.0f;
constexpr float T_EPS = 0.0001f;
constexpr int WAVE = 64;
constexpr int PREPROCESS_BLOCK = 256;
static inline int preprocess_blocks(int32_t P) { return (P + PREPROCESS_BLOCK - 1) / PREPROCESS_BLOCK; }

void set_hip_error(hipError_t e, const char* what);
void set_error_text(const char* text);

int lookback_error_init();
int lookback_error_poll();
int lookback_set_spin_limit(uint32_t limit);
int launch_debug_exp2(int64_t n, const float* x, float* y, hipStream_t stream);
int launch_poison_lds(uint32_t pattern, hipStream_t stream);

#define SR_HIP_CHECK(expr)                                 \
    do {                                                   \
        hipError_t _e = (expr);                            \
        if (_e != hipSuccess) {                            \
            ::sr::set_hip_error(_e, #expr);                \
            return SPLATRASTER_ERR_HIP;                    \
        }                                                  \
    } while (0)

#define SR_LAUNCH_CHECK()                                  \
    do {                                                   \
        hipError_t _e = hipGetLastError();                 \
        if (_e != hipSuccess) {                            \
            ::sr::set_hip_error(_e, "kernel launch");      \
            return SPLATRASTER_ERR_HIP;                    \
        }                                                  \
    } while (0)

static inline size_t align_up(size_t v, size_t a) { return (v + a - 1) / a * a; }

constexpr int MAX_VIEWS = SPLATRASTER_MAX_WINDOW_VIEWS;
struct WinCams {
    const float* view[MAX_VIEWS];
    const float* proj[MAX_VIEWS];
    const float* campos[MAX_VIEWS];
    float tanfovx[MAX_VIEWS], tanfovy[MAX_VIEWS];
    int32_t* radii[MAX_VIEWS];
};
struct WinOut {
    float* color[MAX_VIEWS];
    float* depth[MAX_VIEWS];
    float* alpha[MAX_VIEWS];
};
struct WinGrad {
    const float* out_color[MAX_VIEWS];
    const float* out_depth[MAX_VIEWS];
    const float* dL_dcolor[MAX_VIEWS];
    const float* dL_ddepth[MAX_VIEWS];
    const float* dL_dalpha[MAX_VIEWS];
    const float* dL_dlast[MAX_VIEWS];
    float* dL_dmeans2D[MAX_VIEWS];
    int gc;
    const float* bg;
    int bg_channels;
};

struct GeomView {
    float4* rec;
    uint32_t* tiles_touched;
    uint32_t* depth_order;
    uint32_t* offsets;
    float* rgb;
    uint8_t* clamped;
    uint32_t* sort_keys;
    uint32_t* sort_tmp;
    uint32_t* total;
    uint32_t* block_tiles;
    uint32_t* span_owner;
};
struct BinView {
    uint32_t* point_list;
    uint32_t* tile_list;
    uint32_t* ranges;
    uint32_t* keys_tmp;
    uint32_t* vals_tmp;
    void* sort_tmp;
    float4* irec;
    uint32_t* ipack;
    float* featp;
    float* gacc;
    float* pose_acc;
    uint32_t* nparts;
    float* ckpt;
    uint32_t* tile_order;
};
struct ImgView {
    float* final_T;
    uint32_t* n_contrib;
};

GeomView geom_view(void* base, int32_t P, int32_t V);
BinView bin_view(void* base, int32_t P, int32_t V, int64_t R, int32_t W, int32_t H, int32_t C);
ImgView img_view(void* base, int32_t W, int32_t H, int32_t V);

struct RawFwd {
    const float* scaling;
    const float* rotation;
    const float* opacity;
    const float* f_dc;
    const float* extra;
    int E;
    float* scales;
    float* rotations;
    float* opacities;
    float* colors;
};
int launch_preprocess(const splatraster_settings& s, int32_t P, int32_t V, const WinCams& cams, const float* means3D,
                      const float* shs , const float* opacities, const float* scales, const float* rotations,
                      const float* cov3D_precomp, GeomView g, uint32_t* zero0, uint32_t nzero0, uint32_t* zero1, uint32_t nzero1,
                      hipStream_t stream, bool depth_keys = true ,
                      const RawFwd* raw = nullptr);
struct RawBwd {
    const float* scaling;
    const float* rotation;
    const float* opacity;
    const float* f_dc;
    int E;
    float* d_scaling;
    float* d_rotation;
    float* d_opacity;
    float* d_f_dc;
    float* d_extra;
    const float* reg_row_grad;
    const float* reg_out;
    float reg_weight;
};
int launch_preprocess_bwd(const splatraster_settings& s, int32_t P, int32_t V, const WinCams& cams, const WinGrad& grads,
                          const float* means3D, const float* shs ,
                          const float* scales, const float* rotations, const float* cov3D_precomp,
                          const uint8_t* clamped, const float4* rec, const float* gacc, int C,
                          float* dL_dcolors,
                          float* dL_dmeans3D, float* dL_dopacities, float* dL_dscales,
                          float* dL_drotations, float* dL_dcov3D, float* dL_dshs,
                          float* dL_dview , float* dL_dproj, float* dL_dcampos,
                          float* pose_acc , hipStream_t stream,
                          const RawBwd* raw = nullptr);
int launch_mark_visible(int32_t P, const float* means3D, const float* view, uint8_t* present,
                        hipStream_t stream);

size_t sort_tmp_bytes(int64_t n);
size_t sort_zero_bytes(int64_t n, int key_bits);
int sort_pairs_u32(int64_t n, uint32_t* keys, uint32_t* vals, uint32_t* keys_alt, uint32_t* vals_alt,
                   int key_bits, void* tmp, hipStream_t stream, bool* result_in_alt, bool tmp_zeroed = false);
size_t scan_tmp_bytes(int64_t n);
size_t scan_state_bytes(int64_t n);
int inclusive_scan_u32(int64_t n, const uint32_t* in, const uint32_t* perm, uint32_t* out, uint32_t* total,
                       void* tmp, hipStream_t stream, bool state_zeroed = false, uint32_t* span_owner = nullptr,
                       uint32_t span = 0, uint32_t span_cap = 0);
constexpr int EMIT_SPAN = 1024;
constexpr uint32_t SPAN_OWNER_CAP = 1u << 16;

int exclusive_scan_u32(int64_t n, uint32_t* inout, uint32_t* total, void* tmp, hipStream_t stream, bool state_zeroed = false);

constexpr int BIN_THREADS = 1024;
#ifndef SR_BIN_SMALL_BLOCKS
#define SR_BIN_SMALL_BLOCKS 128
#endif
static inline int bin_rows_per_thread(int32_t P, int32_t V, int tiles)
{
    if (tiles > 2048) return 8;
    const int64_t blocks2 = (int64_t)(V > 0 ? V : 1) * ((P + 2 * BIN_THREADS - 1) / (2 * BIN_THREADS));
    return blocks2 < SR_BIN_SMALL_BLOCKS ? 1 : 2;
}
static inline int bin_chunk_rows(int32_t P, int32_t V, int tiles) { return BIN_THREADS * bin_rows_per_thread(P, V, tiles); }
static inline int bin_chunks(int32_t P, int32_t V, int tiles) { return (P + bin_chunk_rows(P, V, tiles) - 1) / bin_chunk_rows(P, V, tiles); }
constexpr int BIN_MAX_TILES = 16384;
#ifndef SR_BIN_AUTO_MAX_TILES
#define SR_BIN_AUTO_MAX_TILES 6144
#endif
constexpr int BIN_AUTO_MAX_TILES = SR_BIN_AUTO_MAX_TILES;
constexpr int BIN_SORT_TILE_NARROW = 2048, BIN_SORT_TILE_WIDE = 4096;
constexpr int BIN_WIDE_FRAMES = 64;
void set_bin_fork(int mode);
void set_bin_tile_cap(int cap);
constexpr int BIN_SORT_BIG = 16384, BIN_BIG_BLOCKS = 128;
constexpr int BIN_BIG_MINE = 1024;
static_assert((size_t)BIN_MAX_TILES * MAX_VIEWS <= (size_t)BIN_BIG_MINE * BIN_BIG_BLOCKS, "every (view, tile) list could be a long one");
void set_bin_mode(int mode);
size_t bin_table_entries(int32_t P, int32_t V, int tiles);
size_t bin_scratch_bytes(int32_t P, int32_t V, int tiles);
bool use_bins(int32_t P, int32_t V, int gx, int gy , size_t scratch_bytes);
int launch_bin_count(const splatraster_settings& s, int32_t P, int32_t V, const GeomView& g, uint32_t* table, void* scan_tmp,
                     hipStream_t stream);
int launch_bin_scatter_sort(const splatraster_settings& s, int32_t P, int32_t V, int64_t R, const GeomView& g,
                            const uint32_t* table, const BinView& b, uint64_t* keys, hipStream_t stream);

int launch_emit(const splatraster_settings& s, int32_t P, int32_t V, int64_t R, const GeomView& g, uint32_t* keys,
                uint32_t* vals, uint32_t* ranges, uint32_t nranges, hipStream_t stream);
int launch_ranges_clear(int32_t tiles, uint32_t* ranges, hipStream_t stream);
int launch_payload(const splatraster_settings& s, int32_t V, int64_t R, const GeomView& g, const BinView& b, hipStream_t stream);
int launch_pad_features(int32_t P, int C, const float* feat, float* featp, hipStream_t stream);
static inline int padded_channels(int C) { return (C + 3) & ~3; }
constexpr int POSE_SETS = 16, POSE_SET_FLOATS = 64;
constexpr size_t POSE_ACC_BYTES = (size_t)POSE_SETS * POSE_SET_FLOATS * sizeof(float) + 256;
__host__ __device__ static inline int gacc_moment_offset(int C) { return ((C & 15) + 7 <= 16) ? C : ((C + 15) & ~15); }
__host__ __device__ static inline int gacc_row_floats(int C) { return (gacc_moment_offset(C) + 7 + 15) & ~15; }
#ifndef SR_SPLIT_MAX_WAVES
#define SR_SPLIT_MAX_WAVES 6144
#endif
constexpr int SPLIT_MAX_WAVES = SR_SPLIT_MAX_WAVES;
constexpr int SPLIT_MIN_LIST = 256;
#ifndef SR_SPLIT_PARTS
#define SR_SPLIT_PARTS 4
#endif
constexpr int SPLIT_PARTS = SR_SPLIT_PARTS;
constexpr int SPLIT_PARTS_MAX = 4 * SPLIT_PARTS;
#ifndef SR_SPLIT_LONG
#define SR_SPLIT_LONG 1024
#endif
#ifndef SR_SPLIT_EXTRA_TILES
#define SR_SPLIT_EXTRA_TILES 512
#endif
constexpr int SPLIT_LONG = SR_SPLIT_LONG, SPLIT_EXTRA_TILES = SR_SPLIT_EXTRA_TILES;
static_assert(SPLIT_EXTRA_TILES % 8 == 0, "the extra workgroups use the quadrant id scheme (8 tiles per 32 ids)");
void set_split_max_waves(int waves);
void set_fwd_team(int mode);
void set_payload_stream_min(int64_t instances);
int split_max_waves();
static inline bool split_lists(int C, int V, int tiles) { return C <= 4 && 4 * V * tiles <= split_max_waves(); }
__host__ __device__ static inline uint32_t split_count(uint32_t len, uint32_t rank)
{
    if (rank >= (uint32_t)SPLIT_EXTRA_TILES || len < (uint32_t)SPLIT_LONG) return (uint32_t)SPLIT_PARTS;
    return len < 2u * (uint32_t)SPLIT_LONG ? 2u * (uint32_t)SPLIT_PARTS : (uint32_t)SPLIT_PARTS_MAX;
}
__host__ __device__ static inline uint32_t split_part(uint32_t len, uint32_t np = (uint32_t)SPLIT_PARTS)
{
    return len < (uint32_t)SPLIT_MIN_LIST ? len : ((len / np + 63u) & ~63u);
}

int launch_composite_fwd(const splatraster_settings& s, int32_t P, int32_t V, int64_t R, const GeomView& g, const BinView& b,
                         const ImgView& im, const float* featp , const float* bg,
                         const WinOut& out, hipStream_t stream);
#ifndef SR_TILE_ORDER
#define SR_TILE_ORDER 1
#endif
constexpr int TILE_ORDER_MAX_WAVES = 32768;
static inline bool use_tile_order(int V, int tiles_per_view) { return SR_TILE_ORDER && 4ll * V * tiles_per_view <= TILE_ORDER_MAX_WAVES; }
int launch_tile_order(const splatraster_settings& s, int32_t V, const BinView& b, hipStream_t stream);
int launch_composite_bwd(const splatraster_settings& s, int32_t P, int32_t V, int64_t R, const GeomView& g,
                         const BinView& b, const ImgView& im, const float* feat, int feat_stride,
                         const WinGrad& grads,
                         float* gacc ,
                         long long* gacc64 ,
                         int det_pass ,
                         hipStream_t stream);
void set_small_panel_max_waves(int waves);
int launch_fixed_to_float(int64_t n, const long long* src, float* dst, hipStream_t stream);

int launch_activate_fwd(int32_t P, int32_t K, int32_t deg, int32_t SC, int32_t E, const float* xyz,
                        const float* f_dc, const float* f_rest, const float* scaling, const float* rotation,
                        const float* opacity, const float* extra, const float* campos, float* scales,
                        float* rotations, float* opacities, float* colors, hipStream_t stream);
int launch_activate_bwd(int32_t P, int32_t K, int32_t deg, int32_t SC, int32_t E, const float* xyz,
                        const float* f_dc, const float* f_rest, const float* scaling, const float* rotation,
                        const float* opacity, const float* campos, const float* g_scales,
                        const float* g_rotations, const float* g_opacities, const float* g_colors, float* d_xyz,
                        float* d_f_dc, float* d_f_rest, float* d_scaling, float* d_rotation, float* d_opacity,
                        float* d_extra, hipStream_t stream);

struct StatsViews {
    const float* vs_grad[MAX_VIEWS];
    const int32_t* radii[MAX_VIEWS];
};
int launch_densification_stats(int32_t P, int32_t V, const StatsViews& views, float* accum ,
                               float* denom , float* max_radii, hipStream_t stream);
size_t mapping_loss_workspace_bytes(int32_t HW);
int launch_mapping_loss_window(int32_t V, int32_t HW, const splatraster_loss_view* views, float threshold, float* out,
                               void* workspace, hipStream_t stream);
int launch_mapping_loss(int32_t HW, const float* image, const float* depth, const float* marker,
                        const float* gt_image, const float* gt_depth, const float* kp, float threshold,
                        const float* exposure, float* g_image, float* g_depth, float* g_marker, float* out,
                        void* workspace, hipStream_t stream);

size_t refinement_loss_workspace_bytes(int32_t C, int32_t H, int32_t W);
int launch_refinement_loss(int32_t C, int32_t H, int32_t W, float lambda, const float* image, const float* gt,
                           float* g_image, float* out, void* workspace, hipStream_t stream);

size_t eval_metrics_workspace_bytes(int32_t C, int32_t H, int32_t W);
int launch_eval_metrics(int32_t C, int32_t H, int32_t W, const float* image, const float* gt, float* out, void* workspace,
                        hipStream_t stream);

int launch_l1_rgbd_loss(int64_t n_color, const float* color, const float* tgt_c, int64_t n_depth, const float* depth,
                        const float* tgt_d, float depth_weight, float* g_color, float* g_depth, float* loss_out, hipStream_t stream);
int launch_pose_step(const float* dL_dview, const float* dL_dproj, const float* dL_dcampos, const float* W2C0, const float* Pm,
                     float lr_rot, float lr_trans, float beta1, float beta2, float eps, int advance, float* state, float* view_out,
                     float* proj_out, float* campos_out, hipStream_t stream);

int knn_dist2(int32_t N, const float* points, float* out, void* workspace, hipStream_t stream);
size_t knn_workspace_bytes(int32_t N);
void knn_set_grid_min(int n);

int grid_layout(int32_t D, int32_t L, int32_t F, int32_t log2_T, int32_t base_res, double per_level_scale, int32_t grid_type,
                splatraster_grid_layout* out);
int grid_forward(const splatraster_grid_layout* lay, int64_t N, const float* x, const float* params, float* out, hipStream_t s);
int grid_backward(const splatraster_grid_layout* lay, int64_t N, const float* x, const float* params, const float* dL_dout,
                  float* dL_dparams, float* dL_dx, hipStream_t s);

}
```

### splatloc_amd/csrc/composite_bwd.hip

```cpp
#include <type_traits>

#include "composite_common.h"

#ifndef SR_BWD_FS
#define SR_BWD_FS 32
#endif
#ifndef SR_BWD_STAGE_UNROLL
#define SR_BWD_STAGE_UNROLL 3
#endif

#ifndef SR_BWD_MINW
#define SR_BWD_MINW 4
#endif

#ifndef SR_BWD_DOT_CHAINS
#define SR_BWD_DOT_CHAINS 2
#endif
#ifndef SR_BWD_SMALL_PANEL_MAX_WAVES
#define SR_BWD_SMALL_PANEL_MAX_WAVES 6144
#endif
#ifndef SR_BWD_DOT_PREFETCH
#define SR_BWD_DOT_PREFETCH 1
#endif
#ifndef SR_BWD_TM
#define SR_BWD_TM 1
#endif
#ifndef SR_BWD_MINW_TM
#define SR_BWD_MINW_TM 3
#endif
#ifndef SR_BWD_DOTM_MIN
#define SR_BWD_DOTM_MIN 8
#endif

namespace sr {

typedef float f32x4 __attribute__((ext_vector_type(4)));

template <int NC, bool SP, bool AUX = true>
struct BwdCfg {
    static constexpr bool SMALLP = NC <= 15 && SP;
    static constexpr bool MFMA = NC >= 32 || SMALLP;
    static constexpr int NM = NC >= 32 ? 32 : (SMALLP ? NC : 0);
    static constexpr int NB = NC >= 32 ? 2 : 1;
    static constexpr bool XD = SMALLP && AUX;
    static constexpr int NV = NC - NM;
    static constexpr bool TM = SR_BWD_TM && SMALLP;
    static constexpr int EG = 8;
    static constexpr int ES = 9;
    static constexpr int KV = NV + ((XD || !AUX) ? 0 : 1) + (TM ? 0 : 6);
    static constexpr int NCP = (NC + 3) & ~3;
    static constexpr int FS = SR_BWD_FS;
    static constexpr int GROUP = 16;
    static constexpr int WS = 17;
};

constexpr int DET_HEADROOM_EXP = 170;
__device__ __forceinline__ int det_scale_exp(unsigned max_bits)
{
    const int eb = (int)((max_bits >> 23) & 0xffu);
    return DET_HEADROOM_EXP - (eb > 0 ? eb : 1);
}
template <bool DET>
__device__ __forceinline__ void acc_add(float* gacc, long long* gacc64, size_t idx, float v, int det_pass)
{
    if (DET) {
        if (det_pass == 0) {
            atomicMax(reinterpret_cast<unsigned*>(gacc) + idx, __float_as_uint(fabsf(v)));
        } else {
            const unsigned mb = __builtin_nontemporal_load(reinterpret_cast<const unsigned*>(gacc) + idx);
            if (((mb >> 23) & 0xffu) == 0xffu) {
                if (__builtin_isinf(v)) atomicAdd(reinterpret_cast<unsigned long long*>(gacc64) + idx, v > 0.f ? 1ull : (1ull << 32));
                return;
            }
            const double scaled = ldexp((double)v, det_scale_exp(mb));
            atomicAdd(reinterpret_cast<unsigned long long*>(gacc64) + idx, (unsigned long long)__double2ll_rn(scaled));
        }
    } else {
        (void)det_pass;
        atomicAdd(gacc + idx, v);
    }
}

template <int NC, bool SP, bool AUX>
constexpr int bwd_min_waves() { return (BwdCfg<NC, SP, AUX>::TM && NC >= 32) ? SR_BWD_MINW_TM : SR_BWD_MINW; }

template <int NC, bool DET, bool SP, bool AUX>
__global__ void __launch_bounds__(WAVE, (bwd_min_waves<NC, SP, AUX>()))
composite_bwd_kernel(int W, int H, int C_total, int CP4, int c0, int first_pass, int tiles , int V,
                     int P ,
                     const uint32_t* __restrict__ ranges, const uint32_t* __restrict__ ipack ,
                     const float4* __restrict__ irec, const float4* __restrict__ featp4,
                     WinGrad grads,
                     const float* __restrict__ final_T_all, const uint32_t* __restrict__ n_contrib_all,
                     float* __restrict__ gacc , int GROW,
                     int MO, long long* __restrict__ gacc64 ,
                     const float* __restrict__ ckpt_all ,
                     const uint32_t* __restrict__ nparts ,
                     int extra_blocks ,
                     const uint32_t* __restrict__ tile_order ,
                     int det_pass )
{
    using Cfg = BwdCfg<NC, SP, AUX>;
    using ST = typename std::conditional<DET, double, float>::type;
    constexpr int NCP = Cfg::NCP, NM = Cfg::NM, NV = Cfg::NV, KV = Cfg::KV, FS = Cfg::FS;
    constexpr int WS = Cfg::WS, GROUP = Cfg::GROUP;
    constexpr bool MFMA = Cfg::MFMA, XD = Cfg::XD;
    constexpr int NB = Cfg::NB;
    constexpr bool TM = Cfg::TM;
    constexpr int EG = Cfg::EG, ES = Cfg::ES;
    constexpr bool DOTM = NC >= SR_BWD_DOTM_MIN;
    constexpr int PPR = NCP / 4;
    static_assert(2 * KV <= WAVE, "at most 25 butterfly-reduced channels per pass");
    __shared__ __attribute__((aligned(16))) float4 s_rec0[FS + 1];
    __shared__ __attribute__((aligned(16))) float4 s_rec1[FS + 1];
    __shared__ __attribute__((aligned(16))) float s_feat[(FS + (DOTM ? 0 : 1)) * NCP];
    __shared__ uint32_t s_cgid[FS + 1];
    __shared__ float s_w[MFMA ? WAVE * WS : 1];
    __shared__ uint32_t s_gid[MFMA ? GROUP : 1];
    __shared__ float s_e[TM ? WAVE * ES : 1];
    __shared__ float2 s_emean[TM ? GROUP : 1];

    int gtile, quad;
    const int gx = (W + TILE - 1) / TILE;
    int seg_y = (int)blockIdx.y;
    if (NC <= 4 && (int)blockIdx.x < extra_blocks) {
        const unsigned per = quadrant_blocks(SPLIT_EXTRA_TILES, gx);
        const unsigned group = blockIdx.x / per;
        int r;
        quadrant_of_block(blockIdx.x - group * per, SPLIT_EXTRA_TILES, gx, r, quad);
        if (r >= SPLIT_EXTRA_TILES || r >= V * tiles) return;
        gtile = (int)tile_order[r];
        seg_y += SPLIT_PARTS * (int)(group + 1u);
        if (seg_y >= (int)nparts[gtile]) return;
    } else {
        quadrant_of_block(blockIdx.x - (NC <= 4 ? (unsigned)extra_blocks : 0u), V * tiles, gx, gtile, quad, tile_order);
        if (gtile >= V * tiles) return;
    }
    const int view = (V == 1) ? 0 : gtile / tiles;
    const int tile = gtile - view * tiles;
    const uint32_t row0 = (uint32_t)view * (uint32_t)P;
    const float* __restrict__ dL_dcolor = grads.dL_dcolor[view];
    const float* __restrict__ dL_ddepth = grads.dL_ddepth[view];
    const float* __restrict__ dL_dalpha = grads.dL_dalpha[view];
    const float* __restrict__ dL_dlast = grads.dL_dlast[view];
    const int gc = grads.gc;
    const float* __restrict__ final_T = final_T_all + (size_t)view * H * W;
    const uint32_t* __restrict__ n_contrib = n_contrib_all + (size_t)view * H * W;
    const int lane = threadIdx.x;
    const int qx = (tile % gx) * TILE + (quad & 1) * 8, qy = (tile / gx) * TILE + (quad >> 1) * 8;
    const int px = qx + (lane & 7), py = qy + (lane >> 3);
    const bool inside = px < W && py < H;
    const float fx = (float)px, fy = (float)py;
    const size_t plane = (size_t)H * W;
    const size_t pix = inside ? (size_t)py * W + px : 0;
    uint32_t beg = ranges[2 * gtile], end0 = ranges[2 * gtile + 1];
    const uint32_t list0 = beg;
    const bool split = !DET && NC <= 4 && ckpt_all != nullptr;
    const int seg = split ? seg_y : 0;
    const int np = (split && nparts != nullptr) ? (int)nparts[gtile] : SPLIT_PARTS;
    if (split) {
        const uint32_t part = split_part(end0 - beg, (uint32_t)np);
        beg += (uint32_t)seg * part;
        if (seg < np - 1) end0 = min(end0, beg + part);
        if (beg >= end0) return;
    }
    float g[NC];
    ST A = 0;
    ST T = 1;
    float gD = 0.0f;
    uint32_t last = 0;
    if (inside) {
        last = n_contrib[pix];
        const bool from_ckpt = split && seg < np - 1 && list0 + last > end0;
        float s_end = 0.0f;
        float gvals[NC];
#pragma unroll
        for (int ch = 0; ch < NC; ++ch) {
            const int c = c0 + ch;
            const bool lastc = c == C_total - 1 && c >= gc && dL_dlast != nullptr;
            const float* src = lastc ? dL_dlast : dL_dcolor + (size_t)(c < gc ? c : 0) * plane;
            gvals[ch] = src[pix];
        }
#pragma unroll
        for (int ch = 0; ch < NC; ++ch) {
            const int c = c0 + ch;
            const bool take = c < gc || (c == C_total - 1 && dL_dlast != nullptr);
            g[ch] = take ? gvals[ch] : 0.0f;
        }
        {
            const float* bgp = grads.bg ? grads.bg : final_T_all;
            const int nb = grads.bg ? grads.bg_channels : 0;
            const int hi = nb > 0 ? nb - 1 : 0;
#pragma unroll
            for (int ch = 0; ch < NC; ++ch) {
                const int c = c0 + ch;
                const float b = bgp[c < hi ? c : hi];
                s_end = fmaf(c < nb ? b : 0.0f, g[ch], s_end);
            }
        }
        float gA = 0.0f;
        if (AUX && first_pass) {
            gD = dL_ddepth ? dL_ddepth[pix] : 0.0f;
            gA = dL_dalpha ? dL_dalpha[pix] : 0.0f;
            s_end -= gA;
        }
        T = (ST)final_T[pix];
        A = (ST)s_end;
        if constexpr (NC <= 4) {
            if (from_ckpt) {
                float sfx = final_T[pix] * s_end;
                const float* rec0 = ckpt_all + (size_t)view * SPLIT_PARTS_MAX * (C_total + 2) * plane + pix;
                for (int k = np - 1; k > seg; --k) {
                    const float* ck = rec0 + (size_t)k * (C_total + 2) * plane;
#pragma unroll
                    for (int ch = 0; ch < NC; ++ch) sfx = fmaf(ck[(size_t)(1 + c0 + ch) * plane], g[ch], sfx);
                    if (AUX) sfx = fmaf(ck[(size_t)(1 + C_total) * plane], gD, sfx);
                }
                const float Tb = rec0[(size_t)(seg + 1) * (C_total + 2) * plane];
                T = (ST)Tb;
                A = (ST)(sfx / Tb);
            }
        }
    } else {
#pragma unroll
        for (int ch = 0; ch < NC; ++ch) g[ch] = 0.0f;
    }
    float gt[MFMA ? 16 : 1][NB];
    if (MFMA) {
#pragma unroll
        for (int t = 0; t < NB; ++t) {
            __builtin_amdgcn_wave_barrier();
#pragma unroll
            for (int ch = 0; ch < 16; ++ch) {
                const int c = 16 * t + ch;
                s_w[lane * WS + ch] = c < NC ? g[c < NC ? c : 0] : ((XD && c == NC) ? gD : 0.0f);
            }
            __builtin_amdgcn_wave_barrier();
#pragma unroll
            for (int kk = 0; kk < 16; ++kk) gt[kk][t] = s_w[(4 * kk + (lane >> 4)) * WS + (lane & 15)];
        }
        __builtin_amdgcn_wave_barrier();
    }
    uint32_t wave_last = last;
#pragma unroll
    for (int d = 1; d < WAVE; d <<= 1) wave_last = max(wave_last, (uint32_t)__shfl_xor((int)wave_last, d, WAVE));
    const uint32_t end = min(end0, list0 + wave_last);
    if (NC <= 4) { if (split && beg >= end) return; }

    const int slotv = (int)(__brev((unsigned)lane) >> 26);
    const bool slot_second = slotv >= KV;
    const int sv = slot_second ? slotv - KV : slotv;
    const bool slot_col = sv < NV;
    const bool slot_ok = slotv < 2 * KV;
    const int slot_off = slot_col ? (c0 + NM + sv) : (TM ? MO + 6 : MO + sv - NV);
    int nslot = 0;
    int e0 = 0;

    auto flush_panel = [&](int count) {
        __builtin_amdgcn_wave_barrier();
        f32x4 D[NB];
#pragma unroll
        for (int t = 0; t < NB; ++t) D[t] = f32x4{0.f, 0.f, 0.f, 0.f};
        const int row = (lane >> 4) * WS + (lane & 15);
#pragma unroll
        for (int kk = 0; kk < 16; ++kk) {
            const float a = s_w[4 * kk * WS + row];
#pragma unroll
            for (int t = 0; t < NB; ++t) {
                D[t] = __builtin_amdgcn_mfma_f32_16x16x4f32(a, gt[kk][t], D[t], 0, 0, 0);
            }
        }
        const int j0c = lane & 15;
#pragma unroll
        for (int r = 0; r < 4; ++r) {
            const int gs = 4 * (lane >> 4) + r;
            if (gs < count) {
                const uint32_t rowi = __umul24(s_gid[gs], (uint32_t)GROW);
#pragma unroll
                for (int t = 0; t < NB; ++t) {
                    const int c = 16 * t + j0c;
                    const bool full = 16 * t + 16 <= NM;
                    const bool col_ok = full || c < NM || (XD && c == NM && first_pass);
                    const uint32_t col_off = (full || c < NM) ? (uint32_t)(c0 + c) : (uint32_t)(MO + 6);
                    if (col_ok) acc_add<DET>(gacc, gacc64, (size_t)(rowi + col_off), D[t][r], det_pass);
                }
            }
        }
        __builtin_amdgcn_wave_barrier();
    };

    auto reduce_e = [&](int count) {
        if constexpr (TM) {
            __builtin_amdgcn_wave_barrier();
            const int eg = lane & 7, ei = lane >> 3;
            const float2 mu = s_emean[min(e0 + eg, GROUP - 1)];
            const float dx = mu.x - (float)(qx + ei);
            const float dy0 = mu.y - (float)qy;
            float m[6] = {0.f, 0.f, 0.f, 0.f, 0.f, 0.f};
#pragma unroll
            for (int j = 0; j < 8; ++j) {
                const float e = s_e[(8 * j + ei) * ES + eg];
                const float dy = dy0 - (float)j;
                const float ey = e * dy;
                m[5] += e;
                m[1] += ey;
                m[4] = fmaf(ey, dy, m[4]);
            }
            m[0] = m[5] * dx;
            m[2] = m[0] * dx;
            m[3] = m[1] * dx;
            const float outv = wave_reduce_hi3<6>(m, lane);
            const int vi = ((lane >> 5) & 1) + 2 * ((lane >> 4) & 1) + 4 * ((lane >> 3) & 1);
            if (eg < count && vi < 6) {
                const size_t di = (size_t)(__umul24(s_gid[e0 + eg], (uint32_t)GROW) + (uint32_t)(MO + vi));
                acc_add<DET>(gacc, gacc64, di, outv, det_pass);
            }
            __builtin_amdgcn_wave_barrier();
        }
    };

    uint32_t pw = 0;
    auto fetch = [&](uint32_t base, uint32_t& w_) {
        w_ = 0u;
        if (base + (uint32_t)lane < end) w_ = ipack[base + (uint32_t)lane];
    };
    if (beg >= end) return;
    const uint64_t gt_mask = (lane == WAVE - 1) ? 0ull : (~0ull << (lane + 1));
    const int nchunks = (int)((end - beg + (WAVE - 1)) / WAVE);
    fetch(beg + (uint32_t)(nchunks - 1) * WAVE, pw);

#pragma unroll 1
    for (int chunk = nchunks - 1; chunk >= 0; --chunk) {
        const uint32_t base = beg + (uint32_t)chunk * WAVE;
        const bool cur_reach = (pw >> (24 + quad)) & 1u;
        uint64_t cand = __builtin_amdgcn_ballot_w64(cur_reach);
        const uint32_t cur_gid = pw & 0xFFFFFFu;
        fetch(chunk > 0 ? base - WAVE : 0xFFFFFF00u, pw);
        const uint32_t idx0 = base - list0;
#pragma unroll 1
        while (cand != 0) {
            const int ncand = min(FS, (int)__popcll(cand));
            const int rank = __popcll(cand & gt_mask);
            const bool mine = cur_reach && ((cand >> lane) & 1ull) && rank < FS;
            __builtin_amdgcn_wave_barrier();
            if (mine) s_cgid[rank] = cur_gid;
            float4 rec_a = make_float4(0.f, 0.f, 0.f, 0.f), rec_b = rec_a;
            if (mine) {
                const size_t j = (size_t)base + lane;
                rec_a = irec[2 * j];
                rec_b = irec[2 * j + 1];
            }
            __builtin_amdgcn_wave_barrier();
#pragma unroll SR_BWD_STAGE_UNROLL
            for (int e = lane; e < ncand * PPR; e += WAVE) {
                const int row = e / PPR, pc = e - row * PPR;
                reinterpret_cast<float4*>(s_feat)[e] = featp4[(size_t)(__umul24(s_cgid[row] - row0, (uint32_t)CP4) + (uint32_t)((c0 >> 2) + pc))];
            }
            if (mine) {
                s_rec0[rank] = rec_a;
                s_rec1[rank] = rec_b;
            }
            __builtin_amdgcn_wave_barrier();
            auto process_pair = [&](int j0, int j1, bool has1, int r0, int r1, float qm0, float qm1) {
                const float4 p0 = s_rec0[r0], q0 = s_rec1[r0];
                const float4 p1 = s_rec0[r1], q1 = s_rec1[r1];
                const float dx0 = p0.x - fx, dy0 = p0.y - fy, dx1 = p1.x - fx, dy1 = p1.y - fy;
                const float pw0 = gauss_log2(q0, dx0, dy0), pw1 = gauss_log2(q1, dx1, dy1);
                const float Gr0 = exp2_core(pw0), Gr1 = exp2_core(pw1);
                const float ar0 = q0.w * Gr0, ar1 = q1.w * Gr1;
                const float al0 = fminf(ALPHA_MAX, ar0), al1 = fminf(ALPHA_MAX, ar1);
                const bool hit0 = (idx0 + (uint32_t)j0 < last) && pw0 <= 0.0f && ar0 >= ALPHA_MIN;
                const bool hit1 = has1 && (idx0 + (uint32_t)j1 < last) && pw1 <= 0.0f && ar1 >= ALPHA_MIN;
                const float G0 = hit0 ? Gr0 : 0.0f, G1 = hit1 ? Gr1 : 0.0f;
                float qd0 = qm0, qd1 = qm1;
                if (!DOTM) {
                    const float* f0 = &s_feat[r0 * NCP];
                    const float* f1 = &s_feat[r1 * NCP];
                    qd0 = AUX ? p0.z * gD : 0.0f;
                    qd1 = AUX ? p1.z * gD : 0.0f;
#pragma unroll
                    for (int ch = 0; ch < NC; ++ch) {
                        qd0 += f0[ch] * g[ch];
                        qd1 += f1[ch] * g[ch];
                    }
                    qd1 = has1 ? qd1 : 0.0f;
                }
                float dA0, dA1, w0, w1;
                if constexpr (DET) {
                    const double Ti0 = hit0 ? T / (1.0 - (double)al0) : T;
                    const double d0 = (double)qd0 - A;
                    dA0 = (float)(Ti0 * d0);
                    const double ah0 = hit0 ? (double)al0 : 0.0;
                    A = fma(ah0, d0, A);
                    w0 = (float)(ah0 * Ti0);
                    const double Ti1 = hit1 ? Ti0 / (1.0 - (double)al1) : Ti0;
                    const double d1 = (double)qd1 - A;
                    dA1 = (float)(Ti1 * d1);
                    const double ah1 = hit1 ? (double)al1 : 0.0;
                    A = fma(ah1, d1, A);
                    w1 = (float)(ah1 * Ti1);
                    T = Ti1;
                } else {
                    const float Ti0 = hit0 ? T * __builtin_amdgcn_rcpf(1.0f - al0) : T;
                    const float d0 = qd0 - A;
                    dA0 = Ti0 * d0;
                    const float ah0 = hit0 ? al0 : 0.0f;
                    A = fmaf(ah0, d0, A);
                    w0 = ah0 * Ti0;
                    const float Ti1 = hit1 ? Ti0 * __builtin_amdgcn_rcpf(1.0f - al1) : Ti0;
                    const float d1 = qd1 - A;
                    dA1 = Ti1 * d1;
                    const float ah1 = hit1 ? al1 : 0.0f;
                    A = fmaf(ah1, d1, A);
                    w1 = ah1 * Ti1;
                    T = Ti1;
                }
                const float E0 = G0 * dA0, E1 = G1 * dA1;
                const uint32_t gi0 = s_cgid[r0], gi1 = s_cgid[r1];
                if constexpr (KV > 0) {
                    float red[2 * KV];
#pragma unroll
                    for (int ch = 0; ch < NV; ++ch) {
                        red[ch] = w0 * g[NM + ch];
                        red[KV + ch] = w1 * g[NM + ch];
                    }
                    if constexpr (!TM) {
                        const float Ex0 = E0 * dx0, Ey0 = E0 * dy0, Ex1 = E1 * dx1, Ey1 = E1 * dy1;
                        red[NV + 0] = Ex0;
                        red[NV + 1] = Ey0;
                        red[NV + 2] = Ex0 * dx0;
                        red[NV + 3] = Ex0 * dy0;
                        red[NV + 4] = Ey0 * dy0;
                        red[NV + 5] = E0;
                        red[KV + NV + 0] = Ex1;
                        red[KV + NV + 1] = Ey1;
                        red[KV + NV + 2] = Ex1 * dx1;
                        red[KV + NV + 3] = Ex1 * dy1;
                        red[KV + NV + 4] = Ey1 * dy1;
                        red[KV + NV + 5] = E1;
                    }
                    if constexpr (!XD && AUX) {
                        red[KV - 1] = w0 * gD;
                        red[2 * KV - 1] = w1 * gD;
                    }
                    {
                        const float outv = wave_reduce_pack<2 * KV>(red, lane);
                        const uint32_t gi = slot_second ? gi1 : gi0;
                        const size_t di = (size_t)(__umul24(gi, (uint32_t)GROW) + (uint32_t)slot_off);
                        if (slot_ok && (has1 || !slot_second)) acc_add<DET>(gacc, gacc64, di, outv, det_pass);
                    }
                }
                if constexpr (MFMA) {
                    s_w[lane * WS + nslot] = w0;
                    s_w[lane * WS + nslot + 1] = w1;
                    if constexpr (TM) {
                        s_e[lane * ES + (nslot - e0)] = E0;
                        s_e[lane * ES + (nslot - e0) + 1] = E1;
                    }
                    if (lane == 0) {
                        s_gid[nslot] = gi0;
                        s_gid[nslot + 1] = gi1;
                        if constexpr (TM) {
                            s_emean[nslot] = make_float2(p0.x, p0.y);
                            s_emean[nslot + 1] = make_float2(p1.x, p1.y);
                        }
                    }
                    nslot += has1 ? 2 : 1;
                    if constexpr (TM) {
                        if (nslot - e0 >= EG - 1 || nslot >= GROUP - 1) {
                            reduce_e(nslot - e0);
                            e0 = nslot;
                        }
                    }
                    if (nslot >= GROUP - 1) {
                        flush_panel(nslot);
                        nslot = 0;
                        e0 = 0;
                    }
                }
            };
            auto dot4 = [&](int slot4) -> f32x4 {
                const int k = lane & 3;
                const int srow = min(slot4 + k, ncand - 1);
                const float* fr = &s_feat[srow * NCP];
                const float zsel = reinterpret_cast<const float*>(&s_rec0[srow])[2];
                constexpr int CH = SR_BWD_DOT_CHAINS;
                f32x4 Qc[CH];
#pragma unroll
                for (int c = 0; c < CH; ++c) Qc[c] = f32x4{0.f, 0.f, 0.f, 0.f};
#if SR_BWD_DOT_PREFETCH
                const float4* f4 = reinterpret_cast<const float4*>(fr);
                float4 cur = f4[0];
#pragma unroll
                for (int i = 0; i < PPR; ++i) {
                    const float4 nxt = f4[i + 1 < PPR ? i + 1 : i];
                    const float v[4] = {cur.x, cur.y, cur.z, cur.w};
#pragma unroll
                    for (int q = 0; q < 4; ++q) {
                        const int ch = 4 * i + q;
                        if (ch < NC) Qc[ch % CH] = __builtin_amdgcn_mfma_f32_4x4x1f32(v[q], g[ch < NC ? ch : 0], Qc[ch % CH], 0, 0, 0);
                    }
                    cur = nxt;
                }
#else
#pragma unroll
                for (int ch = 0; ch < NC; ++ch)
                    Qc[ch % CH] = __builtin_amdgcn_mfma_f32_4x4x1f32(fr[ch], g[ch], Qc[ch % CH], 0, 0, 0);
#endif
                Qc[NC % CH] = __builtin_amdgcn_mfma_f32_4x4x1f32(zsel, gD, Qc[NC % CH], 0, 0, 0);
                f32x4 Q = Qc[0];
#pragma unroll
                for (int c = 1; c < CH; ++c) Q += Qc[c];
                return Q;
            };
#pragma unroll 1
            for (int slot = 0; slot < ncand; slot += (DOTM ? 4 : 2)) {
                const bool has1 = slot + 1 < ncand, has2 = DOTM && slot + 2 < ncand, has3 = DOTM && slot + 3 < ncand;
                const int j0 = 63 - __builtin_clzll(cand);
                cand &= ~(1ull << j0);
                const int j1 = has1 ? 63 - __builtin_clzll(cand) : j0;
                if (has1) cand &= ~(1ull << j1);
                const int j2 = has2 ? 63 - __builtin_clzll(cand) : j1;
                if (has2) cand &= ~(1ull << j2);
                const int j3 = has3 ? 63 - __builtin_clzll(cand) : j2;
                if (has3) cand &= ~(1ull << j3);
                float qm[4] = {0.f, 0.f, 0.f, 0.f};
                if (DOTM) {
                    const f32x4 Q = dot4(slot);
                    qm[0] = Q[0]; qm[1] = Q[1]; qm[2] = Q[2]; qm[3] = Q[3];
                }
                process_pair(j0, j1, has1, slot, slot + 1, qm[0], qm[1]);
                if (has2) process_pair(j2, j3, has3, slot + 2, slot + 3, qm[2], qm[3]);
            }
        }
    }
    if constexpr (TM) { if (nslot - e0 > 0) reduce_e(nslot - e0); }
    if (MFMA && nslot > 0) flush_panel(nslot);
}



static int g_small_panel_max_waves = SR_BWD_SMALL_PANEL_MAX_WAVES;
void set_small_panel_max_waves(int waves) { g_small_panel_max_waves = waves < 0 ? SR_BWD_SMALL_PANEL_MAX_WAVES : waves; }

struct BwdLaunch {
    int P, V;
    const WinGrad* grads;
    const float* ckpt;
    int det_pass;
};

template <int NC, bool DET, bool AUX = true>
static int launch_one_bwd(const splatraster_settings& s, int c0, int first, const GeomView& g,
                          const BinView& b, const ImgView& im, const float* feat, int feat_stride,
                          const BwdLaunch& L, float* gacc, long long* gacc64, hipStream_t stream)
{
    (void)g;
    const int gx = (s.image_width + TILE - 1) / TILE, gy = (s.image_height + TILE - 1) / TILE;
    const int tiles = gx * gy;
    const unsigned blocks = quadrant_blocks(L.V * tiles, gx);
    const float* ckpt = (NC <= 4 && c0 == 0 && first) ? L.ckpt : nullptr;
    const bool extras = ckpt != nullptr && use_tile_order(L.V, tiles);
    const unsigned extra_blocks = extras ? (unsigned)(SPLIT_PARTS_MAX / SPLIT_PARTS - 1) * quadrant_blocks(SPLIT_EXTRA_TILES, gx) : 0u;
    const dim3 grid(blocks + extra_blocks, ckpt ? (unsigned)SPLIT_PARTS : 1u);
#define SR_BWD_LAUNCH(SPV)                                                                                          \
    hipLaunchKernelGGL((composite_bwd_kernel<NC, DET, SPV, AUX>), grid, dim3(WAVE), 0, stream, s.image_width,           \
                       s.image_height, feat_stride, padded_channels(feat_stride) / 4, c0, first, tiles, L.V, L.P,      \
                       b.ranges, b.ipack, b.irec, reinterpret_cast<const float4*>(feat), *L.grads,       \
                       im.final_T, im.n_contrib, gacc, gacc_row_floats(s.channels),                                    \
                       gacc_moment_offset(s.channels), gacc64, ckpt, extras ? b.nparts : nullptr, (int)extra_blocks,               \
                       use_tile_order(L.V, tiles) ? b.tile_order : nullptr, L.det_pass)
    if constexpr (NC >= 4 && NC <= 15 && AUX) {
        if (4 * tiles <= g_small_panel_max_waves)
            SR_BWD_LAUNCH(true);
        else
            SR_BWD_LAUNCH(false);
    } else {
        SR_BWD_LAUNCH(false);
    }
#undef SR_BWD_LAUNCH
    SR_LAUNCH_CHECK();
    return SPLATRASTER_OK;
}

int launch_composite_bwd(const splatraster_settings& s, int32_t P, int32_t V, int64_t R, const GeomView& g,
                         const BinView& b, const ImgView& im, const float* feat, int feat_stride,
                         const WinGrad& grads, float* gacc, long long* gacc64, int det_pass, hipStream_t stream)
{
    if (R == 0) return SPLATRASTER_OK;
    const bool det = gacc64 != nullptr;
    int C = s.channels;
    const int tiles_v = ((s.image_width + TILE - 1) / TILE) * ((s.image_height + TILE - 1) / TILE);
    const BwdLaunch L{P, V, &grads, (!det && split_lists(s.channels, V, tiles_v)) ? b.ckpt : nullptr, det_pass};
    bool any_last = false, any_aux = false;
    for (int v = 0; v < V; ++v) {
        any_last = any_last || grads.dL_dlast[v] != nullptr;
        any_aux = any_aux || grads.dL_ddepth[v] != nullptr || grads.dL_dalpha[v] != nullptr;
    }
    if (grads.gc < C && !any_last) C = grads.gc;
    if (C == 3 && !any_aux && !det)
        return launch_one_bwd<3, false, false>(s, 0, 1, g, b, im, feat, feat_stride, L, gacc, gacc64, stream);
#define SR_BWD_ARGS g, b, im, feat, feat_stride, L, gacc, gacc64, stream
#define SR_BWD_ONE(N, c0_, first_) (det ? launch_one_bwd<N, true>(s, c0_, first_, SR_BWD_ARGS) : launch_one_bwd<N, false>(s, c0_, first_, SR_BWD_ARGS))
#define SR_BWD_CASE(N) \
    case N: return SR_BWD_ONE(N, 0, 1);
    switch (C) {
        SR_BWD_CASE(1) SR_BWD_CASE(2) SR_BWD_CASE(3) SR_BWD_CASE(4) SR_BWD_CASE(8) SR_BWD_CASE(16)
        SR_BWD_CASE(32) SR_BWD_CASE(35)
        default: break;
    }
#undef SR_BWD_CASE
    int c0 = 0, first = 1, st = SPLATRASTER_OK;
    while (c0 < C && st == SPLATRASTER_OK) {
        const int left = C - c0;
        if (left >= 32) { st = SR_BWD_ONE(32, c0, first); c0 += 32; }
        else if (left >= 16) { st = SR_BWD_ONE(16, c0, first); c0 += 16; }
        else if (left >= 8) { st = SR_BWD_ONE(8, c0, first); c0 += 8; }
        else if (left >= 4) { st = SR_BWD_ONE(4, c0, first); c0 += 4; }
        else if (left == 3) { st = SR_BWD_ONE(3, c0, first); c0 += 3; }
        else if (left == 2) { st = SR_BWD_ONE(2, c0, first); c0 += 2; }
        else { st = SR_BWD_ONE(1, c0, first); c0 += 1; }
        first = 0;
    }
#undef SR_BWD_ONE
#undef SR_BWD_ARGS
    return st;
}

}
```

### splatloc_amd/csrc/composite_common.h

```cpp
#pragma once
#include "common.h"

namespace sr {

__device__ __forceinline__ unsigned quadrant_reach_mask(const float4 r0, const float4 r1, float tile_x0,
                                                        float tile_y0)
{
    const float A = r1.x, B = r1.y, C = r1.z;
    const float lim0 = 2.0f * __logf(255.0f * r1.w);
    const float lim = lim0 + 0.02f + 1e-4f * fabsf(lim0);
    if (!(lim > 0.0f)) return 0u;
    const float nBrA = -B * __frcp_rn(A), nBrC = -B * __frcp_rn(C);
    unsigned mask = 0u;
#pragma unroll
    for (int q = 0; q < 4; ++q) {
        const float bx0 = tile_x0 + (float)((q & 1) * 8), by0 = tile_y0 + (float)((q >> 1) * 8);
        const float u0 = r0.x - (bx0 + 7.0f), u1 = r0.x - bx0;
        const float v0 = r0.y - (by0 + 7.0f), v1 = r0.y - by0;
        float qmin;
        if (u0 <= 0.0f && u1 >= 0.0f && v0 <= 0.0f && v1 >= 0.0f) {
            qmin = 0.0f;
        } else {
            qmin = 3.0e38f;
#pragma unroll
            for (int e = 0; e < 2; ++e) {
                const float ue = e ? u1 : u0;
                const float vs = fminf(v1, fmaxf(v0, nBrC * ue));
                qmin = fminf(qmin, A * ue * ue + 2.0f * B * ue * vs + C * vs * vs);
                const float ve = e ? v1 : v0;
                const float us = fminf(u1, fmaxf(u0, nBrA * ve));
                qmin = fminf(qmin, A * us * us + 2.0f * B * us * ve + C * ve * ve);
            }
        }
        if (qmin <= lim) mask |= 1u << q;
    }
    return mask;
}

__device__ __forceinline__ bool quadrant_reach(const float4 r0, const float4 r1, float bx0, float by0)
{
    const float A = r1.x, B = r1.y, C = r1.z;
    const float lim0 = 2.0f * __logf(255.0f * r1.w);
    const float lim = lim0 + 0.02f + 1e-4f * fabsf(lim0);
    const float u0 = r0.x - (bx0 + 7.0f), u1 = r0.x - bx0;
    const float v0 = r0.y - (by0 + 7.0f), v1 = r0.y - by0;
    float qmin = 0.0f;
    if (!(u0 <= 0.0f && u1 >= 0.0f && v0 <= 0.0f && v1 >= 0.0f)) {
        const float nBrA = -B * __frcp_rn(A), nBrC = -B * __frcp_rn(C);
        qmin = 3.0e38f;
#pragma unroll
        for (int e = 0; e < 2; ++e) {
            const float ue = e ? u1 : u0;
            const float vs = fminf(v1, fmaxf(v0, nBrC * ue));
            qmin = fminf(qmin, A * ue * ue + 2.0f * B * ue * vs + C * vs * vs);
            const float ve = e ? v1 : v0;
            const float us = fminf(u1, fmaxf(u0, nBrA * ve));
            qmin = fminf(qmin, A * us * us + 2.0f * B * us * ve + C * ve * ve);
        }
    }
    return (lim > 0.0f) && (qmin <= lim);
}

constexpr float LOG2E = 1.4426950408889634f;
__device__ __forceinline__ float4 payload_conic(const float4& conic_opacity)
{
    return make_float4(-0.5f * LOG2E * conic_opacity.x, -LOG2E * conic_opacity.y, -0.5f * LOG2E * conic_opacity.z,
                       conic_opacity.w);
}
__device__ __forceinline__ float gauss_log2(const float4& q, float dx, float dy)
{
    return fmaf(dx, fmaf(q.y, dy, q.x * dx), (q.z * dy) * dy);
}
constexpr float EXP2_C0 = 1.0f, EXP2_C1 = 0.6931470036506653f, EXP2_C2 = 0.24022242426872253f,
                EXP2_C3 = 0.05550733581185341f, EXP2_C4 = 0.009671512991189957f, EXP2_C5 = 0.001326472731307149f;
__device__ __forceinline__ float exp2_core(float x)
{
#ifdef SR_EXP2_HW
    return __builtin_amdgcn_exp2f(x);
#else
    const float n = __builtin_rintf(x);
    const float f = x - n;
    float p = fmaf(EXP2_C5, f, EXP2_C4);
    p = fmaf(p, f, EXP2_C3);
    p = fmaf(p, f, EXP2_C2);
    p = fmaf(p, f, EXP2_C1);
    p = fmaf(p, f, EXP2_C0);
    int e;
    asm("v_cvt_i32_f32 %0, %1" : "=v"(e) : "v"(n));
    return __builtin_amdgcn_ldexpf(p, e);
#endif
}
__device__ __forceinline__ float exp2_shared(float x)
{
    return exp2_core(fminf(fmaxf(x, -200.0f), 200.0f));
}
__device__ __forceinline__ float transmit(float T, float alpha)
{
#pragma clang fp contract(off)
    const float om = 1.0f - alpha;
    return T * om;
}

__device__ __forceinline__ void quadrant_of_block(unsigned id, int tiles, int gx, int& tile, int& quad,
                                                  const uint32_t* __restrict__ order = nullptr)
{
    (void)gx;
    tile = (int)((id >> 5) * 8u + (id & 7u));
    quad = (int)((id >> 3) & 3u);
    if (order && tile < tiles) tile = (int)order[tile];
}
__host__ __device__ static inline unsigned quadrant_blocks(int tiles, int gx)
{
    (void)gx;
    return (unsigned)((tiles + 7) / 8) * 32u;
}

__device__ __forceinline__ uint64_t uniform_u64(uint64_t v)
{
    const unsigned lo = __builtin_amdgcn_readfirstlane((unsigned)v);
    const unsigned hi = __builtin_amdgcn_readfirstlane((unsigned)(v >> 32));
    return ((uint64_t)hi << 32) | lo;
}

template <int CTRL, int ROW_MASK>
__device__ __forceinline__ float dpp_get(float v)
{
    return __builtin_bit_cast(
        float, __builtin_amdgcn_update_dpp(0, __builtin_bit_cast(int, v), CTRL, ROW_MASK, 0xf, false));
}

__device__ __forceinline__ float as_f(unsigned u) { return __builtin_bit_cast(float, u); }
__device__ __forceinline__ unsigned as_u(float f) { return __builtin_bit_cast(unsigned, f); }

template <int CTRL, int BANK_MASK>
__device__ __forceinline__ float dpp_mov_old(float old, float v)
{
    return __builtin_bit_cast(float, __builtin_amdgcn_update_dpp(__builtin_bit_cast(int, old),
                                                                 __builtin_bit_cast(int, v), CTRL, 0xf,
                                                                 BANK_MASK, false));
}

#ifndef SR_BUTTERFLY_ASM
#define SR_BUTTERFLY_ASM 1
#endif
__device__ __forceinline__ float fold_lane_bit3(float x, float y)
{
#if !SR_BUTTERFLY_ASM
    const bool lo = (__lane_id() & 8) == 0;
    const float keep = lo ? x : y, send = lo ? y : x;
    return keep + dpp_get<0x128, 0xf>(send);
#endif
    float d;
    asm("s_nop 1\n\t"
        "v_add_f32_dpp %0, %1, %1 row_ror:8 row_mask:0xf bank_mask:0x3\n\t"
        "v_add_f32_dpp %0, %2, %2 row_ror:8 row_mask:0xf bank_mask:0xc"
        : "=&v"(d)
        : "v"(x), "v"(y));
    return d;
}
__device__ __forceinline__ float fold_lane_bit2(float x, float y)
{
#if !SR_BUTTERFLY_ASM
    const bool lo = (__lane_id() & 4) == 0;
    const float keep = lo ? x : y, send = lo ? y : x;
    float t = dpp_mov_old<0x12C, 0x5>(0.0f, send);
    t = dpp_mov_old<0x124, 0xA>(t, send);
    return keep + t;
#endif
    float d;
    asm("s_nop 1\n\t"
        "v_add_f32_dpp %0, %1, %1 row_ror:12 row_mask:0xf bank_mask:0x5\n\t"
        "v_add_f32_dpp %0, %2, %2 row_ror:4 row_mask:0xf bank_mask:0xa"
        : "=&v"(d)
        : "v"(x), "v"(y));
    return d;
}

template <int K>
__device__ __forceinline__ float wave_reduce_pack(const float (&v)[K], int lane)
{
    static_assert(K >= 1 && K <= 64, "at most 64 values per wave");
    constexpr int N1 = (K + 1) / 2, N2 = (N1 + 1) / 2, N3 = (N2 + 1) / 2, N4 = (N3 + 1) / 2,
                  N5 = (N4 + 1) / 2, N6 = (N5 + 1) / 2;
    static_assert(N6 == 1, "");
    float a[N1];
#pragma unroll
    for (int m = 0; m < N1; ++m) {
        const float x = v[2 * m];
        const float y = (2 * m + 1 < K) ? v[2 * m + 1] : 0.0f;
        const auto r = __builtin_amdgcn_permlane32_swap(as_u(x), as_u(y), false, false);
        a[m] = as_f(r[0]) + as_f(r[1]);
    }
    float b[N2];
// ... 68 lines not shown
```

### splatloc_amd/csrc/composite_fwd.hip

```cpp
#include <type_traits>

#include "composite_common.h"

#ifndef SR_FWD_FS
#define SR_FWD_FS 24
#endif
#ifndef SR_FWD_STAGE_UNROLL
#define SR_FWD_STAGE_UNROLL 3
#endif

#ifndef SR_FWD_M4
#define SR_FWD_M4 1
#endif
#ifndef SR_FWD_MINW
#define SR_FWD_MINW 4
#endif

namespace sr {


typedef float f32x16 __attribute__((ext_vector_type(16)));
typedef float f32x4 __attribute__((ext_vector_type(4)));

__device__ __forceinline__ void swap_halves(float& x, float& y)
{
    asm volatile("s_nop 1\n\tv_permlane32_swap_b32 %0, %1\n\ts_nop 1" : "+v"(x), "+v"(y));
}

__device__ __forceinline__ void mfma_acc_32x32x2(f32x16& acc, float a, float b)
{
    asm volatile("s_nop 1\n\tv_mfma_f32_32x32x2_f32 %0, %1, %2, %0" : "+v"(acc) : "v"(a), "v"(b));
}
__device__ __forceinline__ void mfma_drain(f32x16& x, f32x16& y)
{
    asm volatile("s_nop 15\n\ts_nop 15" : "+v"(x), "+v"(y));
}
__device__ __forceinline__ void mfma_acc_4x4x1(f32x4& acc, float a, float b)
{
    asm volatile("s_nop 1\n\tv_mfma_f32_4x4x1_16b_f32 %0, %1, %2, %0" : "+v"(acc) : "v"(a), "v"(b));
}
__device__ __forceinline__ void mfma_drain4(f32x4& x)
{
    asm volatile("s_nop 7" : "+v"(x));
}

__device__ __forceinline__ int first_bit(uint64_t m)
{
    int j;
    asm("s_ff1_i32_b64 %0, %1" : "=s"(j) : "s"(m));
    return j;
}

template <int NC>
struct FwdCfg {
    static constexpr bool MFMA = NC >= 32;
    static constexpr int NM = MFMA ? 32 : 0;
    static constexpr int NV = NC - NM;
    static constexpr int NCP = (NC + 3) & ~3;
    static constexpr bool M4 = SR_FWD_M4 && MFMA && NV > 0 && NV <= 3 && NM + NV < NCP;
    static constexpr int FS = SR_FWD_FS;
};

template <int NC>
__global__ void __launch_bounds__(WAVE, SR_FWD_MINW)
composite_fwd_kernel(int W, int H, int CP4, int c0, int bg_channels, int write_aux, int tiles , int V,
                     int P ,
                     const uint32_t* __restrict__ ranges, const uint32_t* __restrict__ ipack ,
                     const float4* __restrict__ irec, const float4* __restrict__ featp4,
                     const float* __restrict__ bg, WinOut outs,
                     float* __restrict__ final_T_all, uint32_t* __restrict__ n_contrib_all,
                     const uint32_t* __restrict__ tile_order )
{
    static_assert(NC > 4, "narrow layouts have their own kernels");
    using Cfg = FwdCfg<NC>;
    constexpr int NCP = Cfg::NCP, NM = Cfg::NM, NV = Cfg::NV, FS = Cfg::FS;
    constexpr bool MFMA = Cfg::MFMA, M4 = Cfg::M4;
    constexpr int PPR = NCP / 4;
    __shared__ __attribute__((aligned(16))) float4 s_rec0[WAVE + 1];
    __shared__ __attribute__((aligned(16))) float4 s_rec1[WAVE + 1];
    static_assert(FS % 2 == 0, "pairs: an odd round ends below FS, its zeroed row FS - 1 at most");
    __shared__ __attribute__((aligned(16))) float s_feat[FS * NCP];
    __shared__ uint32_t s_cgid[FS];

    int gtile, quad;
    const int gx = (W + TILE - 1) / TILE;
    quadrant_of_block(blockIdx.x, V * tiles, gx, gtile, quad, tile_order);
    if (gtile >= V * tiles) return;
    const int view = (V == 1) ? 0 : gtile / tiles;
    const int tile = gtile - view * tiles;
    const uint32_t row0 = (uint32_t)view * (uint32_t)P;
    float* __restrict__ out_color = outs.color[view];
    float* __restrict__ out_depth = outs.depth[view];
    float* __restrict__ out_alpha = outs.alpha[view];
    float* __restrict__ final_T = final_T_all + (size_t)view * H * W;
    uint32_t* __restrict__ n_contrib = n_contrib_all + (size_t)view * H * W;
    const int lane = threadIdx.x;
    const int qx = (tile % gx) * TILE + (quad & 1) * 8, qy = (tile / gx) * TILE + (quad >> 1) * 8;
    const int px = qx + (lane & 7), py = qy + (lane >> 3);
    const bool inside = px < W && py < H;
    const float fx = (float)px, fy = (float)py;
    const uint32_t beg = ranges[2 * gtile], end = ranges[2 * gtile + 1];

    if (lane == 0) {
        s_rec0[0] = make_float4(0.f, 0.f, 0.f, 0.f);
        s_rec1[0] = make_float4(0.f, 0.f, 0.f, 0.f);
    }
    bool active = inside;
    float T = 1.0f, D = 0.0f;
    float acc[NV > 0 ? NV : 1];
#pragma unroll
    for (int ch = 0; ch < NV; ++ch) acc[ch] = 0.0f;
    f32x16 accA, accB;
#pragma unroll
    for (int r = 0; r < 16; ++r) { accA[r] = 0.0f; accB[r] = 0.0f; }
    f32x4 acc4 = {0.0f, 0.0f, 0.0f, 0.0f};
    uint32_t last = 0;
    const int lb32 = (lane >> 5) * NCP + (lane & 31);
    const uint64_t lt_mask = (lane == 0) ? 0ull : (~0ull >> (WAVE - lane));

    uint32_t pw = 0;
    float4 a0 = make_float4(0.f, 0.f, 0.f, 0.f), a1 = a0;
    auto fetch = [&](uint32_t base, uint32_t& w_, float4& x0, float4& x1) {
        w_ = 0u;
        if (base + (uint32_t)lane < end) {
            const uint32_t j = base + (uint32_t)lane;
            w_ = ipack[j];
            x0 = irec[2 * (size_t)j];
            x1 = irec[2 * (size_t)j + 1];
        }
    };
    fetch(beg, pw, a0, a1);

    bool wave_done = __builtin_amdgcn_ballot_w64(active) == 0;
#pragma unroll 1
    for (uint32_t base = beg; base < end && !wave_done; base += WAVE) {
        const bool cur_reach = (pw >> (24 + quad)) & 1u;
        uint64_t cand = __builtin_amdgcn_ballot_w64(cur_reach);
        const uint32_t cur_gid = pw & 0xFFFFFFu;
        if (cand != 0) {
            __builtin_amdgcn_wave_barrier();
            s_rec0[1 + lane] = a0;
            s_rec1[1 + lane] = a1;
        }
        fetch(base + WAVE, pw, a0, a1);
#pragma unroll 1
        while (cand != 0 && !wave_done) {
            const int rank = __popcll(cand & lt_mask);
            const int ncand = min(FS, (int)__popcll(cand));
            __builtin_amdgcn_wave_barrier();
            if (cur_reach && ((cand >> lane) & 1ull) && rank < FS) s_cgid[rank] = cur_gid - row0;
            __builtin_amdgcn_wave_barrier();
#pragma unroll SR_FWD_STAGE_UNROLL
            for (int e = lane; e < ncand * PPR; e += WAVE) {
                const int row = e / PPR, pc = e - row * PPR;
                reinterpret_cast<float4*>(s_feat)[e] = featp4[(size_t)(__umul24(s_cgid[row], (uint32_t)CP4) + (uint32_t)((c0 >> 2) + pc))];
            }
            __builtin_amdgcn_wave_barrier();
            if (ncand & 1) {
                if (lane < PPR) reinterpret_cast<float4*>(s_feat)[ncand * PPR + lane] = make_float4(0.f, 0.f, 0.f, 0.f);
                __builtin_amdgcn_wave_barrier();
            }
            if constexpr (M4) {
                if (cur_reach && ((cand >> lane) & 1ull) && rank < FS) s_feat[rank * NCP + NM + 3] = s_rec0[1 + lane].z;
                __builtin_amdgcn_wave_barrier();
            }
#pragma unroll 1
            for (int slot = 0; slot < ncand; slot += 2) {
                const int j0 = first_bit(cand);
                cand &= cand - 1;
                const int j1 = first_bit(cand);
                cand &= cand - 1;
                const float4 p0 = s_rec0[1 + j0], q0 = s_rec1[1 + j0];
                const float4 p1 = s_rec0[1 + j1], q1 = s_rec1[1 + j1];
                const int s1 = slot + 1;
                float a32 = 0.0f, a40 = 0.0f, a41 = 0.0f;
                if constexpr (MFMA) a32 = s_feat[slot * NCP + lb32];
                if constexpr (M4) {
                    const int l4 = NM + (lane & 3);
                    a40 = s_feat[slot * NCP + l4];
                    a41 = s_feat[s1 * NCP + l4];
                }
                if constexpr (MFMA) __builtin_amdgcn_sched_barrier(0);
                const float dx0 = p0.x - fx, dy0 = p0.y - fy, dx1 = p1.x - fx, dy1 = p1.y - fy;
                const float pw0 = gauss_log2(q0, dx0, dy0), pw1 = gauss_log2(q1, dx1, dy1);
                const float ar0 = q0.w * exp2_core(pw0), ar1 = q1.w * exp2_core(pw1);
                const float al0 = fminf(ALPHA_MAX, ar0), al1 = fminf(ALPHA_MAX, ar1);
                const bool live0 = active && pw0 <= 0.0f && ar0 >= ALPHA_MIN;
                const float tT0 = transmit(T, al0);
                const bool hit0 = live0 && tT0 >= T_EPS;
                const bool act1 = active && !(live0 && !hit0);
                const float w0 = hit0 ? al0 * T : 0.0f;
                const float T1 = hit0 ? tT0 : T;
                const bool live1 = act1 && pw1 <= 0.0f && ar1 >= ALPHA_MIN;
                const float tT1 = transmit(T1, al1);
                const bool hit1 = live1 && tT1 >= T_EPS;
                active = act1 && !(live1 && !hit1);
                const float w1 = hit1 ? al1 * T1 : 0.0f;
                T = hit1 ? tT1 : T1;
                const uint32_t idx = base - beg;
                last = hit1 ? idx + (uint32_t)j1 + 1u : (hit0 ? idx + (uint32_t)j0 + 1u : last);
                const float* f0 = &s_feat[slot * NCP + NM];
                const float* f1 = &s_feat[s1 * NCP + NM];
                if constexpr (M4) {
                    mfma_acc_4x4x1(acc4, a40, w0);
                    mfma_acc_4x4x1(acc4, a41, w1);
                } else {
#pragma unroll
                    for (int ch = 0; ch < NV; ++ch) {
                        if (MFMA) acc[ch] += f0[ch] * w0 + f1[ch] * w1;
                        else acc[ch] = fmaf(f1[ch], w1, fmaf(f0[ch], w0, acc[ch]));
                    }
                    if (MFMA) D += p0.z * w0 + p1.z * w1;
                    else D = fmaf(p1.z, w1, fmaf(p0.z, w0, D));
                }
                if (MFMA) {
                    float b0 = w0, b1 = w1;
                    swap_halves(b0, b1);
                    mfma_acc_32x32x2(accA, a32, b0);
                    mfma_acc_32x32x2(accB, a32, b1);
                }
                if (__builtin_amdgcn_ballot_w64(active) == 0) { wave_done = true; break; }
            }
        }
    }

    const size_t plane = (size_t)H * W;
    if constexpr (M4) {
        mfma_drain4(acc4);
#pragma unroll
        for (int ch = 0; ch < NV; ++ch) acc[ch] = acc4[ch];
        D = acc4[3];
    }
    if (MFMA) {
        mfma_drain(accA, accB);
        float TA = T, TB = T;
        swap_halves(TA, TB);
        const int pa = lane & 31, pb = 32 + (lane & 31);
        const int xa = qx + (pa & 7), ya = qy + (pa >> 3), xb = qx + (pb & 7), yb = qy + (pb >> 3);
        const bool ina = xa < W && ya < H, inb = xb < W && yb < H;
#pragma unroll
        for (int r = 0; r < 16; ++r) {
            const int c = c0 + (r & 3) + 8 * (r >> 2) + 4 * (lane >> 5);
            const float bgc = c < bg_channels ? bg[c] : 0.0f;
            if (ina) out_color[(size_t)c * plane + (size_t)ya * W + xa] = accA[r] + TA * bgc;
            if (inb) out_color[(size_t)c * plane + (size_t)yb * W + xb] = accB[r] + TB * bgc;
        }
    }
    if (inside) {
        const size_t pix = (size_t)py * W + px;
#pragma unroll
        for (int ch = 0; ch < NV; ++ch) {
            const int c = c0 + NM + ch;
            out_color[(size_t)c * plane + pix] = acc[ch] + T * (c < bg_channels ? bg[c] : 0.0f);
        }
        if (write_aux) {
            out_depth[pix] = D;
            out_alpha[pix] = 1.0f - T;
            final_T[pix] = T;
            n_contrib[pix] = last;
        }
    }
}

#define SR_FWD_PARAMS                                                                                                        \
    int W, int H, int CP4, int c0, int bg_channels, int write_aux, int tiles , int V, int P ,  \
        const uint32_t *__restrict__ ranges, const uint32_t *__restrict__ ipack ,                  \
        const float4 *__restrict__ irec, const float4 *__restrict__ featp4, const float *__restrict__ bg, WinOut outs,      \
        float *__restrict__ final_T_all, uint32_t *__restrict__ n_contrib_all,                                              \
        float *__restrict__ ckpt_all , \
        const uint32_t *__restrict__ nparts
#define SR_FWD_ARGS W, H, CP4, c0, bg_channels, write_aux, tiles, V, P, ranges, ipack, irec, featp4, bg, outs, final_T_all, n_contrib_all, ckpt_all, nparts

template <int NC>
__device__ __forceinline__ void narrow_quadrant(SR_FWD_PARAMS, int gtile, int quad, int lane, float4* __restrict__ s_rec0,
                                                float4* __restrict__ s_rec1, float4* __restrict__ s_fq)
{
    static_assert(NC >= 1 && NC <= 4, "one 16-byte piece per feature row");
    const int gx = (W + TILE - 1) / TILE;
    const int view = (V == 1) ? 0 : gtile / tiles;
    const int tile = gtile - view * tiles;
    const uint32_t row0 = (uint32_t)view * (uint32_t)P;
    float* __restrict__ out_color = outs.color[view];
    float* __restrict__ out_depth = outs.depth[view];
    float* __restrict__ out_alpha = outs.alpha[view];
    float* __restrict__ final_T = final_T_all + (size_t)view * H * W;
    uint32_t* __restrict__ n_contrib = n_contrib_all + (size_t)view * H * W;
    const int qx = (tile % gx) * TILE + (quad & 1) * 8, qy = (tile / gx) * TILE + (quad >> 1) * 8;
    const int px = qx + (lane & 7), py = qy + (lane >> 3);
    const bool inside = px < W && py < H;
    const float fx = (float)px, fy = (float)py;
    const uint32_t beg = ranges[2 * gtile], end = ranges[2 * gtile + 1];

    if (lane == 0) {
        s_rec0[0] = make_float4(0.f, 0.f, 0.f, 0.f);
        s_rec1[0] = make_float4(0.f, 0.f, 0.f, 0.f);
        s_fq[0] = make_float4(0.f, 0.f, 0.f, 0.f);
    }
    bool active = inside;
    float T = 1.0f, D = 0.0f;
    float acc[NC];
#pragma unroll
    for (int ch = 0; ch < NC; ++ch) acc[ch] = 0.0f;
    uint32_t last = 0;

    const uint32_t fo = (uint32_t)(c0 >> 2);
    uint32_t pw = 0, pw2 = 0;
    float4 a0 = make_float4(0.f, 0.f, 0.f, 0.f), a1 = a0, af = a0;
    auto fetch_word = [&](uint32_t base, uint32_t& w_) {
        w_ = 0u;
        if (base + (uint32_t)lane < end) w_ = ipack[base + (uint32_t)lane];
    };
    auto fetch_entry = [&](uint32_t base, uint32_t w_) {
        if (base + (uint32_t)lane < end) {
            const uint32_t j = base + (uint32_t)lane;
            a0 = irec[2 * (size_t)j];
            a1 = irec[2 * (size_t)j + 1];
            if ((w_ >> (24 + quad)) & 1u) af = featp4[(size_t)(__umul24((w_ & 0xFFFFFFu) - row0, (uint32_t)CP4) + fo)];
        }
    };
    fetch_word(beg, pw);
    fetch_word(beg + WAVE, pw2);
    fetch_entry(beg, pw);

    bool wave_done = __builtin_amdgcn_ballot_w64(active) == 0;
    const int np = (ckpt_all != nullptr && nparts != nullptr) ? (int)nparts[gtile] : SPLIT_PARTS;
    const uint32_t part = ckpt_all != nullptr ? split_part(end - beg, (uint32_t)np) : 0u;
    uint32_t ck_at = part ? beg + part : 0xFFFFFFFFu;
    int ck_k = 0;
    float sacc[NC], sD = 0.0f;
#pragma unroll
    for (int ch = 0; ch < NC; ++ch) sacc[ch] = 0.0f;
    auto store_segment = [&](int k, bool with_next_T) {
        if (inside) {
            const size_t pl = (size_t)H * W;
            float* ck = ckpt_all + ((size_t)view * SPLIT_PARTS_MAX + k) * (NC + 2) * pl + (size_t)py * W + px;
#pragma unroll
            for (int ch = 0; ch < NC; ++ch) ck[(size_t)(1 + ch) * pl] = sacc[ch];
            ck[(size_t)(1 + NC) * pl] = sD;
            if (with_next_T) ck[(size_t)(NC + 2) * pl] = T;
        }
    };
#pragma unroll 1
    for (uint32_t base = beg; base < end && !wave_done; base += WAVE) {
        if (base == ck_at) {
            store_segment(ck_k, true);
#pragma unroll
            for (int ch = 0; ch < NC; ++ch) sacc[ch] = 0.0f;
            sD = 0.0f;
            ++ck_k;
            ck_at = ck_k < np - 1 ? ck_at + part : 0xFFFFFFFFu;
        }
        uint64_t cand = __builtin_amdgcn_ballot_w64((pw >> (24 + quad)) & 1u);
        if (cand != 0) {
            __builtin_amdgcn_wave_barrier();
            s_rec0[1 + lane] = a0;
            s_rec1[1 + lane] = a1;
            s_fq[1 + lane] = af;
            __builtin_amdgcn_wave_barrier();
        }
        pw = pw2;
        fetch_entry(base + WAVE, pw);
        fetch_word(base + 2 * WAVE, pw2);
        const uint32_t idx = base - beg;
#pragma unroll 1
        while (cand != 0) {
            const int j0 = first_bit(cand);
            cand &= cand - 1;
            const int j1 = first_bit(cand);
            cand &= cand - 1;
            const float4 p0 = s_rec0[1 + j0], q0 = s_rec1[1 + j0], f0 = s_fq[1 + j0];
            const float4 p1 = s_rec0[1 + j1], q1 = s_rec1[1 + j1], f1 = s_fq[1 + j1];
            const float dx0 = p0.x - fx, dy0 = p0.y - fy, dx1 = p1.x - fx, dy1 = p1.y - fy;
            const float pw0 = gauss_log2(q0, dx0, dy0), pw1 = gauss_log2(q1, dx1, dy1);
            const float ar0 = q0.w * exp2_core(pw0), ar1 = q1.w * exp2_core(pw1);
            const float al0 = fminf(ALPHA_MAX, ar0), al1 = fminf(ALPHA_MAX, ar1);
            const bool live0 = active && pw0 <= 0.0f && ar0 >= ALPHA_MIN;
// ... 277 lines not shown
    for (int ch = 0; ch < NC; ++ch) sacc[ch] = 0.0f;
    auto store_sums = [&](int k) {
        if (inside) {
            float* ck = ckpt_all + ((size_t)view * SPLIT_PARTS_MAX + k) * (NC + 2) * plane + pix;
#pragma unroll
            for (int ch = 0; ch < NC; ++ch) ck[(size_t)(1 + ch) * plane] = sacc[ch];
            ck[(size_t)(1 + NC) * plane] = sD;
        }
    };
    auto boundary = [&] {
        if (base == ck_at) {
            store_sums(ck_k);
#pragma unroll
            for (int ch = 0; ch < NC; ++ch) sacc[ch] = 0.0f;
            sD = 0.0f;
            ++ck_k;
            ck_at = ck_k < np - 1 ? ck_at + part : 0xFFFFFFFFu;
        }
    };
#pragma unroll 1
    for (int it = 0;; ++it) {
        if (it > 1) {
            const uint64_t m = next_step(std::integral_constant<int, 3>{}, boundary);
            const int n = (int)__popcll(m);
            if (n) {
                __builtin_amdgcn_wave_barrier();
                if ((m >> lane) & 1ull) {
                    const int slot = (int)__popcll(m & lt_mask);
                    s_cf[slot] = c1r;
                    s_cz[slot] = c0r.x;
                }
                if (lane == 0 && (n & 1)) {
                    s_cf[n] = make_float4(0.f, 0.f, 0.f, 0.f);
                    s_cz[n] = 0.0f;
                }
                __builtin_amdgcn_wave_barrier();
                const float* __restrict__ buf = &s_buf[(it - 2) % 3][0][lane];
#pragma unroll
                for (int i = 0; i < STEP / 2; ++i) {
                    if (2 * i >= n) break;
                    const float w0 = buf[(2 * i) * WAVE], w1 = buf[(2 * i + 1) * WAVE];
                    const float4 f0 = s_cf[2 * i], f1 = s_cf[2 * i + 1];
                    const float2 zz = *reinterpret_cast<const float2*>(&s_cz[2 * i]);
                    const float fv0[4] = {f0.x, f0.y, f0.z, f0.w}, fv1[4] = {f1.x, f1.y, f1.z, f1.w};
#pragma unroll
                    for (int ch = 0; ch < NC; ++ch) acc[ch] = fmaf(fv1[ch], w1, fmaf(fv0[ch], w0, acc[ch]));
                    D = fmaf(zz.y, w1, fmaf(zz.x, w0, D));
                    if (part) {
#pragma unroll
                        for (int ch = 0; ch < NC; ++ch) sacc[ch] = fmaf(fv1[ch], w1, fmaf(fv0[ch], w0, sacc[ch]));
                        sD = fmaf(zz.y, w1, fmaf(zz.x, w0, sD));
                    }
                }
            }
        }
        __syncthreads();
        if (s_fin >= 0 && it >= s_fin) break;
    }
    if (part) {
        store_sums(ck_k);
#pragma unroll
        for (int ch = 0; ch < NC; ++ch) sacc[ch] = 0.0f;
        sD = 0.0f;
        for (int k = ck_k + 1; k < np; ++k) store_sums(k);
    }
    if (inside) {
        const float T = s_T[lane];
        float* __restrict__ out_color = outs.color[view];
#pragma unroll
        for (int ch = 0; ch < NC; ++ch) {
            const int c = c0 + ch;
            out_color[(size_t)c * plane + pix] = acc[ch] + T * (c < bg_channels ? bg[c] : 0.0f);
        }
        if (write_aux) outs.depth[view][pix] = D;
    }
}

#ifndef SR_FWD_TEAM_MAX
#define SR_FWD_TEAM_MAX 128
#endif
#ifndef SR_FWD_TEAM_MIN_LIST
#define SR_FWD_TEAM_MIN_LIST 512
#endif
constexpr int TEAM_MAX = SR_FWD_TEAM_MAX, TEAM_MIN_LIST = SR_FWD_TEAM_MIN_LIST;
__device__ __forceinline__ bool team_list(int r, int T, const uint32_t* __restrict__ ranges, const uint32_t* __restrict__ order, int force)
{
    if (r >= TEAM_MAX || r >= T) return false;
    if (force) return true;
    const uint32_t t = order[r];
    const uint32_t len = ranges[2 * t + 1] - ranges[2 * t];
    if (len < (uint32_t)TEAM_MIN_LIST) return false;
    if (4 * T <= 1024) return true;
    const uint32_t q = order[T >> 2];
    return 4u * len >= 5u * (ranges[2 * q + 1] - ranges[2 * q]);
}
static_assert(4 * 3 * (WAVE + 1) * sizeof(float4) <= sizeof(float) * 3 * TEAM_STEP * WAVE, "the four waves' chunk copies fit the team's buffers");
template <int NC>
__global__ void __launch_bounds__(4 * WAVE, 5)
composite_fwd_mixed_kernel(SR_FWD_PARAMS, const uint32_t* __restrict__ tile_order , int force)
{
    __shared__ __attribute__((aligned(16))) TeamLds L;
    const int T = V * tiles;
    const int b = (int)blockIdx.x;
    if (b < 4 * TEAM_MAX) {
        const int r = b >> 2;
        if (!team_list(r, T, ranges, tile_order, force)) return;
        team_quadrant<NC>(SR_FWD_ARGS, (int)tile_order[r], b & 3, L);
        return;
    }
    const int r = b - 4 * TEAM_MAX;
    if (r >= T || team_list(r, T, ranges, tile_order, force)) return;
    const int w = __builtin_amdgcn_readfirstlane((int)(threadIdx.x >> 6));
    float4* mine = reinterpret_cast<float4*>(&L.buf[0][0][0]) + w * 3 * (WAVE + 1);
    narrow_quadrant<NC>(SR_FWD_ARGS, (int)tile_order[r], w, (int)(threadIdx.x & (WAVE - 1)), mine, mine + (WAVE + 1), mine + 2 * (WAVE + 1));
}

__global__ void debug_exp2_kernel(int64_t n, const float* __restrict__ x, float* __restrict__ y)
{
    const int64_t i = (int64_t)blockIdx.x * blockDim.x + threadIdx.x;
    if (i < n) y[i] = exp2_shared(x[i]);
}

__global__ void __launch_bounds__(256) poison_lds_kernel(uint32_t pattern, uint32_t* __restrict__ sink)
{
    __shared__ uint32_t s_all[16384];
    for (int i = threadIdx.x; i < 16384; i += 256) s_all[i] = pattern;
    __syncthreads();
    const uint32_t v = s_all[(pattern + threadIdx.x * 61u) & 16383u];
    if (v != pattern) sink[0] = v;
    __builtin_amdgcn_s_sleep(64);
}

int launch_poison_lds(uint32_t pattern, hipStream_t stream)
{
    static uint32_t* sink = nullptr;
    if (!sink && hipMalloc(&sink, 256) != hipSuccess) return SPLATRASTER_ERR_HIP;
    hipLaunchKernelGGL(poison_lds_kernel, dim3(256 * 2 * 4), dim3(256), 0, stream, pattern, sink);
    SR_LAUNCH_CHECK();
    return SPLATRASTER_OK;
}

int launch_debug_exp2(int64_t n, const float* x, float* y, hipStream_t stream)
{
    hipLaunchKernelGGL(debug_exp2_kernel, dim3((unsigned)((n + 255) / 256)), dim3(256), 0, stream, n, x, y);
    SR_LAUNCH_CHECK();
    return SPLATRASTER_OK;
}

struct FwdLaunch {
    int P, V;
    const WinOut* outs;
    float* ckpt;
    bool team;
};

static int g_fwd_team = -1;
void set_fwd_team(int mode) { g_fwd_team = mode; }

template <int NC>
static int launch_one(const splatraster_settings& s, int c0, int write_aux, const GeomView& g,
                      const BinView& b, const ImgView& im, const float* featp, int feat_stride,
                      const float* bg, const FwdLaunch& L, hipStream_t stream)
{
    (void)g;
    const int gx = (s.image_width + TILE - 1) / TILE, gy = (s.image_height + TILE - 1) / TILE;
    const int tiles = gx * gy;
    const unsigned blocks = quadrant_blocks(L.V * tiles, gx);
    if constexpr (NC <= 4) {
        if (L.team && use_tile_order(L.V, tiles)) {
            hipLaunchKernelGGL(composite_fwd_mixed_kernel<NC>, dim3((unsigned)(L.V * tiles + 4 * TEAM_MAX)), dim3(4 * WAVE), 0, stream,
                               s.image_width, s.image_height, padded_channels(feat_stride) / 4, c0, s.bg_channels, write_aux, tiles, L.V, L.P,
                               b.ranges, b.ipack, b.irec, reinterpret_cast<const float4*>(featp), bg, *L.outs, im.final_T, im.n_contrib,
                               (c0 == 0 && write_aux) ? L.ckpt : nullptr, b.nparts, b.tile_order, g_fwd_team == 2 ? 1 : 0);
        } else {
            hipLaunchKernelGGL(composite_fwd_narrow_kernel<NC>, dim3(blocks), dim3(WAVE), 0, stream, s.image_width,
                               s.image_height, padded_channels(feat_stride) / 4, c0, s.bg_channels, write_aux, tiles, L.V, L.P, b.ranges,
                               b.ipack, b.irec, reinterpret_cast<const float4*>(featp), bg, *L.outs, im.final_T,
                               im.n_contrib, (c0 == 0 && write_aux) ? L.ckpt : nullptr, use_tile_order(L.V, tiles) ? b.nparts : nullptr,
                               use_tile_order(L.V, tiles) ? b.tile_order : nullptr);
        }
    } else {
        hipLaunchKernelGGL(composite_fwd_kernel<NC>, dim3(blocks), dim3(WAVE), 0, stream, s.image_width,
                           s.image_height, padded_channels(feat_stride) / 4, c0, s.bg_channels, write_aux, tiles, L.V, L.P, b.ranges,
                           b.ipack, b.irec, reinterpret_cast<const float4*>(featp), bg, *L.outs, im.final_T,
                           im.n_contrib, use_tile_order(L.V, tiles) ? b.tile_order : nullptr);
    }
    SR_LAUNCH_CHECK();
    return SPLATRASTER_OK;
}

int launch_composite_fwd(const splatraster_settings& s, int32_t P, int32_t V, int64_t R, const GeomView& g, const BinView& b,
                         const ImgView& im, const float* featp, const float* bg, const WinOut& outs, hipStream_t stream)
{
    (void)R;
    const int C = s.channels;
    const int tiles_v = ((s.image_width + TILE - 1) / TILE) * ((s.image_height + TILE - 1) / TILE);
    const bool team = g_fwd_team < 0 ? split_lists(C, V, tiles_v) : (g_fwd_team != 0 && C <= 4);
    const FwdLaunch L{P, V, &outs, split_lists(C, V, tiles_v) ? b.ckpt : nullptr, team};
    int c0 = 0, aux = 1, st = SPLATRASTER_OK;
#define SR_FWD_CASE(N)                                                                              \
    case N:                                                                                         \
        return launch_one<N>(s, 0, 1, g, b, im, featp, C, bg, L, stream);
    switch (C) {
        SR_FWD_CASE(1) SR_FWD_CASE(2) SR_FWD_CASE(3) SR_FWD_CASE(4) SR_FWD_CASE(8) SR_FWD_CASE(16)
        SR_FWD_CASE(32) SR_FWD_CASE(35)
        default: break;
    }
#undef SR_FWD_CASE
    while (c0 < C && st == SPLATRASTER_OK) {
        const int left = C - c0;
        if (left >= 32) { st = launch_one<32>(s, c0, aux, g, b, im, featp, C, bg, L, stream); c0 += 32; }
        else if (left >= 16) { st = launch_one<16>(s, c0, aux, g, b, im, featp, C, bg, L, stream); c0 += 16; }
        else if (left >= 8) { st = launch_one<8>(s, c0, aux, g, b, im, featp, C, bg, L, stream); c0 += 8; }
        else if (left >= 4) { st = launch_one<4>(s, c0, aux, g, b, im, featp, C, bg, L, stream); c0 += 4; }
        else if (left == 3) { st = launch_one<3>(s, c0, aux, g, b, im, featp, C, bg, L, stream); c0 += 3; }
        else if (left == 2) { st = launch_one<2>(s, c0, aux, g, b, im, featp, C, bg, L, stream); c0 += 2; }
        else { st = launch_one<1>(s, c0, aux, g, b, im, featp, C, bg, L, stream); c0 += 1; }
        aux = 0;
    }
    return st;
}

}
```

Baseline: 733.2.

## Replace payload materialization with on-the-fly gather and forward-recorded hit masks for wide channels

For wide channel counts (C>4, multiple of 8 or 35) the per-instance payload kernel is skipped. A small ranges kernel is launched instead, and the composite kernels gather Gaussian records by point id from the per-Gaussian rec array, computing quadrant reach on the fly. The forward pass also records per-chunk, per-quadrant 64-bit hit masks that the backward pass reuses as candidate masks. This removes writing and reading the large per-instance irec/ipack arrays, at the cost of uncoalesced gathers, extra ballots in the inner loop, and a hit-mask buffer. It also disables checkpoint splitting in backward when gathering and changes occupancy bounds.

```diff
diff --git a/include/splatraster.h b/include/splatraster.h
--- a/include/splatraster.h
+++ b/include/splatraster.h
@@ -8,7 +8,7 @@
 extern "C" {
 #endif
 
-#define SPLATRASTER_ABI_VERSION 14
+#define SPLATRASTER_ABI_VERSION 15
 
 #define SPLATRASTER_TILE 16
 
@@ -384,6 +384,7 @@
 int splatraster_debug_set_split_max_waves(int waves);
 int splatraster_debug_set_fwd_team(int mode);
 int splatraster_debug_set_payload_stream_min(int64_t instances);
+int splatraster_debug_set_force_payload(int on);
 int splatraster_debug_set_front_end(int mode);
 int splatraster_debug_set_tile_sort_cap(int keys);
 int splatraster_debug_set_sort_fork(int mode);
diff --git a/splatloc_amd/_native.py b/splatloc_amd/_native.py
--- a/splatloc_amd/_native.py
+++ b/splatloc_amd/_native.py
@@ -6,7 +6,7 @@
 from . import build as _build
 
 _LIB = None
-ABI_VERSION = 14
+ABI_VERSION = 15
 
 OK = 0
 WARN_LOOKBACK_STALL = 5
@@ -126,6 +126,7 @@
     "splatraster_debug_set_tile_sort_cap": (C.c_int, [C.c_int]),
     "splatraster_debug_set_sort_fork": (C.c_int, [C.c_int]),
     "splatraster_debug_set_payload_stream_min": (C.c_int, [C.c_int64]),
+    "splatraster_debug_set_force_payload": (C.c_int, [C.c_int]),
     "splatraster_mark_visible": (C.c_int, [_i32, _vp, _vp, _vp, _vp, _vp]),
     "splatraster_get_geometry_layout": (C.c_int, [_i32, C.POINTER(GeometryLayout)]),
     "splatraster_get_binning_layout": (C.c_int, [_i32, _i64, _i32, _i32, _i32, C.POINTER(BinningLayout)]),
diff --git a/splatloc_amd/csrc/binning.hip b/splatloc_amd/csrc/binning.hip
--- a/splatloc_amd/csrc/binning.hip
+++ b/splatloc_amd/csrc/binning.hip
@@ -167,6 +167,24 @@
     return SPLATRASTER_OK;
 }
 
+__global__ void __launch_bounds__(256)
+ranges_kernel(int64_t R, const uint32_t* __restrict__ tile_list, uint32_t* __restrict__ ranges)
+{
+    const int64_t j = (int64_t)blockIdx.x * blockDim.x + threadIdx.x;
+    if (j >= R) return;
+    const uint32_t t = tile_list[j];
+    if (j == 0 || tile_list[j - 1] != t) ranges[2 * t] = (uint32_t)j;
+    if (j == R - 1 || tile_list[j + 1] != t) ranges[2 * t + 1] = (uint32_t)(j + 1);
+}
+
+int launch_ranges(int64_t R, const BinView& b, hipStream_t stream)
+{
+    if (R == 0) return SPLATRASTER_OK;
+    hipLaunchKernelGGL(ranges_kernel, dim3((unsigned)((R + 255) / 256)), dim3(256), 0, stream, R, b.tile_list, b.ranges);
+    SR_LAUNCH_CHECK();
+    return SPLATRASTER_OK;
+}
+
 __global__ void __launch_bounds__(ORDER_THREADS)
 tile_order_kernel(int T, const uint32_t* __restrict__ ranges, uint32_t* __restrict__ order, uint32_t* __restrict__ nparts)
 {
diff --git a/splatloc_amd/csrc/capi.hip b/splatloc_amd/csrc/capi.hip
--- a/splatloc_amd/csrc/capi.hip
+++ b/splatloc_amd/csrc/capi.hip
@@ -148,7 +148,7 @@
 }
 
 struct BinLayout {
-    size_t keysA, valsA, keysB, valsB, ranges, sort_tmp, irec, ipack, featp, gacc, pose_acc, ckpt, tile_order, nparts, bytes;
+    size_t keysA, valsA, keysB, valsB, ranges, sort_tmp, irec, ipack, featp, gacc, pose_acc, ckpt, tile_order, nparts, hits, bytes;
 };
 static BinLayout bin_layout(int32_t P, int32_t V, int64_t R, int32_t W, int32_t H, int32_t C)
 {
@@ -173,6 +173,7 @@
     L.ckpt = take(ck ? nv * (size_t)SPLIT_PARTS_MAX * (size_t)(C + 2) * (size_t)W * (size_t)H * sizeof(float) : 16);
     L.tile_order = take(4 * (tiles > 0 ? tiles : 1));
     L.nparts = take(4 * (tiles > 0 ? tiles : 1));
+    L.hits = take(4 * sizeof(uint64_t) * hit_slots((int64_t)n, (int64_t)tiles));
     L.bytes = o;
     return L;
 }
@@ -196,6 +197,7 @@
     v.ckpt = reinterpret_cast<float*>(b + L.ckpt);
     v.tile_order = reinterpret_cast<uint32_t*>(b + L.tile_order);
     v.nparts = reinterpret_cast<uint32_t*>(b + L.nparts);
+    v.hits = reinterpret_cast<uint64_t*>(b + L.hits);
     return v;
 }
 
@@ -350,6 +352,26 @@
     std::lock_guard<std::mutex> lk(g_front_end_mu);
     auto it = g_front_end.find(geometry);
     return it == g_front_end.end() ? -1 : (it->second ? 1 : 0);
+}
+
+static std::unordered_map<const void*, bool> g_gathered;
+#ifndef SR_FORCE_PAYLOAD
+#define SR_FORCE_PAYLOAD 0
+#endif
+static int g_force_payload = SR_FORCE_PAYLOAD;
+void set_force_payload(int on) { g_force_payload = on ? 1 : 0; }
+bool force_payload() { return g_force_payload != 0; }
+static void gathered_record(const void* binning, bool on)
+{
+    std::lock_guard<std::mutex> lk(g_front_end_mu);
+    if (g_gathered.size() > (1u << 14)) g_gathered.clear();
+    g_gathered[binning] = on;
+}
+static int gathered_recorded(const void* binning)
+{
+    std::lock_guard<std::mutex> lk(g_front_end_mu);
+    auto it = g_gathered.find(binning);
+    return it == g_gathered.end() ? -1 : (it->second ? 1 : 0);
 }
 
 static BinScratch bin_scratch(const splatraster_settings& s, int32_t P, int32_t V, void* geometry, bool geometry_stage)
@@ -521,9 +543,16 @@
     }
     if (st) return st;
     const float* featp = feat;
+    const bool gather = R > 0 && !bins.on && gather_layout(s->channels) && !force_payload();
+    gathered_record(binning, gather);
+    if (gather) {
+        StageTimer t(SPLATRASTER_STAGE_RANGES, stream);
+        st = launch_ranges(R, b, stream);
+        if (st) return st;
+    }
     if (R > 0) {
         StageTimer t(SPLATRASTER_STAGE_PAYLOAD, stream);
-        if (!bins.on) st = launch_payload(*s, V, R, g, b, stream);
+        if (!bins.on && !gather) st = launch_payload(*s, V, R, g, b, stream);
         if (st) return st;
         if (s->channels % 4) {
             st = launch_pad_features(P, s->channels, feat, b.featp, stream);
@@ -543,7 +572,7 @@
         outs.alpha[v] = views[v].out_alpha;
     }
     StageTimer t(SPLATRASTER_STAGE_COMPOSITE_FWD, stream);
-    return launch_composite_fwd(*s, P, V, R, g, b, im, featp, bg, outs, stream);
+    return launch_composite_fwd(*s, P, V, R, g, b, im, featp, bg, outs, gather, stream);
 }
 
 static int window_backward(const splatraster_settings* s, int32_t V, const splatraster_window_view* views, int32_t P,
@@ -613,6 +642,9 @@
         SR_HIP_CHECK(hipMallocAsync(reinterpret_cast<void**>(&gacc64), sizeof(long long) * gacc_n, stream));
         SR_HIP_CHECK(hipMemsetAsync(gacc64, 0, sizeof(long long) * gacc_n, stream));
     }
+    const int rec_gather = gathered_recorded(binning);
+    const bool gather = rec_gather >= 0 ? rec_gather == 1
+                                        : (!bin_scratch(*s, P, V, geometry, false).on && gather_layout(C) && !force_payload());
     const bool pose = dL_dviewmatrix && dL_dprojmatrix;
     const size_t fill = pose ? (size_t)(reinterpret_cast<char*>(b.pose_acc) - reinterpret_cast<char*>(b.gacc)) + POSE_ACC_BYTES
                              : sizeof(float) * gacc_n;
@@ -621,8 +653,8 @@
     grads.bg_channels = bg ? s->bg_channels : 0;
     {
         StageTimer t(SPLATRASTER_STAGE_COMPOSITE_BWD, stream);
-        if (det) st = launch_composite_bwd(*s, P, V, R, g, b, im, (C % 4) ? b.featp : feat, C, grads, b.gacc, gacc64, 0, stream);
-        if (!st) st = launch_composite_bwd(*s, P, V, R, g, b, im, (C % 4) ? b.featp : feat, C, grads, b.gacc, gacc64, 1, stream);
+        if (det) st = launch_composite_bwd(*s, P, V, R, g, b, im, (C % 4) ? b.featp : feat, C, grads, b.gacc, gacc64, 0, gather, stream);
+        if (!st) st = launch_composite_bwd(*s, P, V, R, g, b, im, (C % 4) ? b.featp : feat, C, grads, b.gacc, gacc64, 1, gather, stream);
     }
     if (det) {
         if (!st) st = launch_fixed_to_float((int64_t)gacc_n, gacc64, b.gacc, stream);
@@ -776,6 +808,12 @@
     return SPLATRASTER_OK;
 }
 
+int splatraster_debug_set_force_payload(int on)
+{
+    sr::set_force_payload(on);
+    return SPLATRASTER_OK;
+}
+
 int splatraster_debug_set_front_end(int mode)
 {
     set_bin_mode(mode);
diff --git a/splatloc_amd/csrc/common.h b/splatloc_amd/csrc/common.h
--- a/splatloc_amd/csrc/common.h
+++ b/splatloc_amd/csrc/common.h
@@ -100,6 +100,7 @@
     uint32_t* nparts;
     float* ckpt;
     uint32_t* tile_order;
+    uint64_t* hits;
 };
 struct ImgView {
     float* final_T;
@@ -206,6 +207,11 @@
                 uint32_t* vals, uint32_t* ranges, uint32_t nranges, hipStream_t stream);
 int launch_ranges_clear(int32_t tiles, uint32_t* ranges, hipStream_t stream);
 int launch_payload(const splatraster_settings& s, int32_t V, int64_t R, const GeomView& g, const BinView& b, hipStream_t stream);
+int launch_ranges(int64_t R, const BinView& b, hipStream_t stream);
+static inline bool gather_layout(int C) { return C > 4 && (C == 35 || C % 8 == 0); }
+__host__ __device__ static inline size_t hit_slots(int64_t R, int64_t gtiles) { return (size_t)(R / 64) + (size_t)gtiles + 1; }
+void set_force_payload(int on);
+bool force_payload();
 int launch_pad_features(int32_t P, int C, const float* feat, float* featp, hipStream_t stream);
 static inline int padded_channels(int C) { return (C + 3) & ~3; }
 constexpr int POSE_SETS = 16, POSE_SET_FLOATS = 64;
@@ -247,7 +253,7 @@
 
 int launch_composite_fwd(const splatraster_settings& s, int32_t P, int32_t V, int64_t R, const GeomView& g, const BinView& b,
                          const ImgView& im, const float* featp , const float* bg,
-                         const WinOut& out, hipStream_t stream);
+                         const WinOut& out, bool gather , hipStream_t stream);
 #ifndef SR_TILE_ORDER
 #define SR_TILE_ORDER 1
 #endif
@@ -260,7 +266,7 @@
                          float* gacc ,
                          long long* gacc64 ,
                          int det_pass ,
-                         hipStream_t stream);
+                         bool gather , hipStream_t stream);
 void set_small_panel_max_waves(int waves);
 int launch_fixed_to_float(int64_t n, const long long* src, float* dst, hipStream_t stream);
 
diff --git a/splatloc_amd/csrc/composite_bwd.hip b/splatloc_amd/csrc/composite_bwd.hip
--- a/splatloc_amd/csrc/composite_bwd.hip
+++ b/splatloc_amd/csrc/composite_bwd.hip
@@ -88,8 +88,9 @@
 __global__ void __launch_bounds__(WAVE, (bwd_min_waves<NC, SP, AUX>()))
 composite_bwd_kernel(int W, int H, int C_total, int CP4, int c0, int first_pass, int tiles , int V,
                      int P ,
-                     const uint32_t* __restrict__ ranges, const uint32_t* __restrict__ ipack ,
-                     const float4* __restrict__ irec, const float4* __restrict__ featp4,
+                     const uint32_t* __restrict__ ranges,
+                     const uint32_t* __restrict__ ipack ,
+                     const float4* __restrict__ irec , const float4* __restrict__ featp4,
                      WinGrad grads,
                      const float* __restrict__ final_T_all, const uint32_t* __restrict__ n_contrib_all,
                      float* __restrict__ gacc , int GROW,
@@ -98,7 +99,8 @@
                      const uint32_t* __restrict__ nparts ,
                      int extra_blocks ,
                      const uint32_t* __restrict__ tile_order ,
-                     int det_pass )
+                     int det_pass ,
+                     const uint32_t* __restrict__ hits )
 {
     using Cfg = BwdCfg<NC, SP, AUX>;
     using ST = typename std::conditional<DET, double, float>::type;
@@ -320,6 +322,7 @@
     };
 
     uint32_t pw = 0;
+    const uint32_t slot0 = (list0 >> 6) + (uint32_t)gtile;
     auto fetch = [&](uint32_t base, uint32_t& w_) {
         w_ = 0u;
         if (base + (uint32_t)lane < end) w_ = ipack[base + (uint32_t)lane];
@@ -332,7 +335,13 @@
 #pragma unroll 1
     for (int chunk = nchunks - 1; chunk >= 0; --chunk) {
         const uint32_t base = beg + (uint32_t)chunk * WAVE;
-        const bool cur_reach = (pw >> (24 + quad)) & 1u;
+        bool cur_reach;
+        if (hits != nullptr) {
+            const uint64_t hm = reinterpret_cast<const uint64_t*>(hits)[4 * (size_t)(slot0 + (uint32_t)chunk) + (size_t)quad];
+            cur_reach = base + (uint32_t)lane < end && ((hm >> lane) & 1ull);
+        } else {
+            cur_reach = (pw >> (24 + quad)) & 1u;
+        }
         uint64_t cand = __builtin_amdgcn_ballot_w64(cur_reach);
         const uint32_t cur_gid = pw & 0xFFFFFFu;
         fetch(chunk > 0 ? base - WAVE : 0xFFFFFF00u, pw);
@@ -346,9 +355,10 @@
             if (mine) s_cgid[rank] = cur_gid;
             float4 rec_a = make_float4(0.f, 0.f, 0.f, 0.f), rec_b = rec_a;
             if (mine) {
-                const size_t j = (size_t)base + lane;
+                const size_t j = hits != nullptr ? (size_t)cur_gid : (size_t)base + lane;
                 rec_a = irec[2 * j];
                 rec_b = irec[2 * j + 1];
+                if (hits != nullptr) rec_b = payload_conic(rec_b);
             }
             __builtin_amdgcn_wave_barrier();
 #pragma unroll SR_BWD_STAGE_UNROLL
@@ -548,6 +558,7 @@
     const WinGrad* grads;
     const float* ckpt;
     int det_pass;
+    bool gather;
 };
 
 template <int NC, bool DET, bool AUX = true>
@@ -555,7 +566,6 @@
                           const BinView& b, const ImgView& im, const float* feat, int feat_stride,
                           const BwdLaunch& L, float* gacc, long long* gacc64, hipStream_t stream)
 {
-    (void)g;
     const int gx = (s.image_width + TILE - 1) / TILE, gy = (s.image_height + TILE - 1) / TILE;
     const int tiles = gx * gy;
     const unsigned blocks = quadrant_blocks(L.V * tiles, gx);
@@ -566,10 +576,12 @@
 #define SR_BWD_LAUNCH(SPV)                                                                                          \
     hipLaunchKernelGGL((composite_bwd_kernel<NC, DET, SPV, AUX>), grid, dim3(WAVE), 0, stream, s.image_width,           \
                        s.image_height, feat_stride, padded_channels(feat_stride) / 4, c0, first, tiles, L.V, L.P,      \
-                       b.ranges, b.ipack, b.irec, reinterpret_cast<const float4*>(feat), *L.grads,       \
+                       b.ranges, L.gather ? b.point_list : b.ipack, L.gather ? g.rec : b.irec,                         \
+                       reinterpret_cast<const float4*>(feat), *L.grads,                                                \
                        im.final_T, im.n_contrib, gacc, gacc_row_floats(s.channels),                                    \
                        gacc_moment_offset(s.channels), gacc64, ckpt, extras ? b.nparts : nullptr, (int)extra_blocks,               \
-                       use_tile_order(L.V, tiles) ? b.tile_order : nullptr, L.det_pass)
+                       use_tile_order(L.V, tiles) ? b.tile_order : nullptr, L.det_pass,                                \
+                       L.gather ? reinterpret_cast<const uint32_t*>(b.hits) : nullptr)
     if constexpr (NC >= 4 && NC <= 15 && AUX) {
         if (4 * tiles <= g_small_panel_max_waves)
             SR_BWD_LAUNCH(true);
@@ -585,13 +597,13 @@
 
 int launch_composite_bwd(const splatraster_settings& s, int32_t P, int32_t V, int64_t R, const GeomView& g,
                          const BinView& b, const ImgView& im, const float* feat, int feat_stride,
-                         const WinGrad& grads, float* gacc, long long* gacc64, int det_pass, hipStream_t stream)
+                         const WinGrad& grads, float* gacc, long long* gacc64, int det_pass, bool gather, hipStream_t stream)
 {
     if (R == 0) return SPLATRASTER_OK;
     const bool det = gacc64 != nullptr;
     int C = s.channels;
     const int tiles_v = ((s.image_width + TILE - 1) / TILE) * ((s.image_height + TILE - 1) / TILE);
-    const BwdLaunch L{P, V, &grads, (!det && split_lists(s.channels, V, tiles_v)) ? b.ckpt : nullptr, det_pass};
+    const BwdLaunch L{P, V, &grads, (!gather && !det && split_lists(s.channels, V, tiles_v)) ? b.ckpt : nullptr, det_pass, gather};
     bool any_last = false, any_aux = false;
     for (int v = 0; v < V; ++v) {
         any_last = any_last || grads.dL_dlast[v] != nullptr;
diff --git a/splatloc_amd/csrc/composite_common.h b/splatloc_amd/csrc/composite_common.h
--- a/splatloc_amd/csrc/composite_common.h
+++ b/splatloc_amd/csrc/composite_common.h
@@ -6,6 +6,7 @@
 __device__ __forceinline__ unsigned quadrant_reach_mask(const float4 r0, const float4 r1, float tile_x0,
                                                         float tile_y0)
 {
+#pragma clang fp contract(off)
     const float A = r1.x, B = r1.y, C = r1.z;
     const float lim0 = 2.0f * __logf(255.0f * r1.w);
     const float lim = lim0 + 0.02f + 1e-4f * fabsf(lim0);
@@ -39,6 +40,7 @@
 
 __device__ __forceinline__ bool quadrant_reach(const float4 r0, const float4 r1, float bx0, float by0)
 {
+#pragma clang fp contract(off)
     const float A = r1.x, B = r1.y, C = r1.z;
     const float lim0 = 2.0f * __logf(255.0f * r1.w);
     const float lim = lim0 + 0.02f + 1e-4f * fabsf(lim0);
diff --git a/splatloc_amd/csrc/composite_fwd.hip b/splatloc_amd/csrc/composite_fwd.hip
--- a/splatloc_amd/csrc/composite_fwd.hip
+++ b/splatloc_amd/csrc/composite_fwd.hip
@@ -61,15 +61,17 @@
     static constexpr int FS = SR_FWD_FS;
 };
 
-template <int NC>
-__global__ void __launch_bounds__(WAVE, SR_FWD_MINW)
+template <int NC, bool GATHER>
+__global__ void __launch_bounds__(WAVE, (GATHER && NC != 32) ? 5 : SR_FWD_MINW)
 composite_fwd_kernel(int W, int H, int CP4, int c0, int bg_channels, int write_aux, int tiles , int V,
                      int P ,
-                     const uint32_t* __restrict__ ranges, const uint32_t* __restrict__ ipack ,
-                     const float4* __restrict__ irec, const float4* __restrict__ featp4,
+                     const uint32_t* __restrict__ ranges,
+                     const uint32_t* __restrict__ ipack ,
+                     const float4* __restrict__ irec , const float4* __restrict__ featp4,
                      const float* __restrict__ bg, WinOut outs,
                      float* __restrict__ final_T_all, uint32_t* __restrict__ n_contrib_all,
-                     const uint32_t* __restrict__ tile_order )
+                     const uint32_t* __restrict__ tile_order ,
+                     uint64_t* __restrict__ hits )
 {
     static_assert(NC > 4, "narrow layouts have their own kernels");
     using Cfg = FwdCfg<NC>;
@@ -119,6 +121,7 @@
     const uint64_t lt_mask = (lane == 0) ? 0ull : (~0ull >> (WAVE - lane));
 
     uint32_t pw = 0;
+    uint32_t pw2 = 0;
     float4 a0 = make_float4(0.f, 0.f, 0.f, 0.f), a1 = a0;
     auto fetch = [&](uint32_t base, uint32_t& w_, float4& x0, float4& x1) {
         w_ = 0u;
@@ -129,12 +132,36 @@
             x1 = irec[2 * (size_t)j + 1];
         }
     };
-    fetch(beg, pw, a0, a1);
+    auto fetch_id = [&](uint32_t base, uint32_t& w_) {
+        w_ = 0u;
+        if (base + (uint32_t)lane < end) w_ = ipack[base + (uint32_t)lane];
+    };
+    auto gather = [&](uint32_t base, uint32_t id) {
+        if (base + (uint32_t)lane < end) {
+            a0 = irec[2 * (size_t)id];
+            a1 = irec[2 * (size_t)id + 1];
+        }
+    };
+    if constexpr (GATHER) {
+        fetch_id(beg, pw);
+        fetch_id(beg + WAVE, pw2);
+        gather(beg, pw);
+    } else {
+        fetch(beg, pw, a0, a1);
+    }
+    const float qfx = (float)qx, qfy = (float)qy;
+    const uint32_t slot0 = (beg >> 6) + (uint32_t)gtile;
 
     bool wave_done = __builtin_amdgcn_ballot_w64(active) == 0;
 #pragma unroll 1
     for (uint32_t base = beg; base < end && !wave_done; base += WAVE) {
-        const bool cur_reach = (pw >> (24 + quad)) & 1u;
+        bool cur_reach;
+        if constexpr (GATHER) {
+            cur_reach = base + (uint32_t)lane < end && quadrant_reach(a0, a1, qfx, qfy);
+            a1 = payload_conic(a1);
+        } else {
+            cur_reach = (pw >> (24 + quad)) & 1u;
+        }
         uint64_t cand = __builtin_amdgcn_ballot_w64(cur_reach);
         const uint32_t cur_gid = pw & 0xFFFFFFu;
         if (cand != 0) {
@@ -142,7 +169,14 @@
             s_rec0[1 + lane] = a0;
             s_rec1[1 + lane] = a1;
         }
-        fetch(base + WAVE, pw, a0, a1);
+        if constexpr (GATHER) {
+            pw = pw2;
+            gather(base + WAVE, pw);
+            fetch_id(base + 2 * WAVE, pw2);
+        } else {
+            fetch(base + WAVE, pw, a0, a1);
+        }
+        uint64_t hm = 0;
 #pragma unroll 1
         while (cand != 0 && !wave_done) {
             const int rank = __popcll(cand & lt_mask);
@@ -199,6 +233,10 @@
                 T = hit1 ? tT1 : T1;
                 const uint32_t idx = base - beg;
                 last = hit1 ? idx + (uint32_t)j1 + 1u : (hit0 ? idx + (uint32_t)j0 + 1u : last);
+                if constexpr (GATHER) {
+                    if (__builtin_amdgcn_ballot_w64(hit0) != 0) hm |= 1ull << j0;
+                    if (__builtin_amdgcn_ballot_w64(hit1) != 0) hm |= 1ull << (j1 & 63);
+                }
                 const float* f0 = &s_feat[slot * NCP + NM];
                 const float* f1 = &s_feat[s1 * NCP + NM];
                 if constexpr (M4) {
@@ -222,6 +260,7 @@
                 if (__builtin_amdgcn_ballot_w64(active) == 0) { wave_done = true; break; }
             }
         }
+        if (GATHER && hits != nullptr && lane == 0) hits[4 * (size_t)(slot0 + ((base - beg) >> 6)) + (size_t)quad] = hm;
     }
 
     const size_t plane = (size_t)H * W;
@@ -805,6 +844,7 @@
     const WinOut* outs;
     float* ckpt;
     bool team;
+    bool gather;
 };
 
 static int g_fwd_team = -1;
@@ -815,7 +855,6 @@
                       const BinView& b, const ImgView& im, const float* featp, int feat_stride,
                       const float* bg, const FwdLaunch& L, hipStream_t stream)
 {
-    (void)g;
     const int gx = (s.image_width + TILE - 1) / TILE, gy = (s.image_height + TILE - 1) / TILE;
     const int tiles = gx * gy;
     const unsigned blocks = quadrant_blocks(L.V * tiles, gx);
@@ -832,24 +871,31 @@
                                im.n_contrib, (c0 == 0 && write_aux) ? L.ckpt : nullptr, use_tile_order(L.V, tiles) ? b.nparts : nullptr,
                                use_tile_order(L.V, tiles) ? b.tile_order : nullptr);
         }
+    } else if (L.gather) {
+        hipLaunchKernelGGL((composite_fwd_kernel<NC, true>), dim3(blocks), dim3(WAVE), 0, stream, s.image_width,
+                           s.image_height, padded_channels(feat_stride) / 4, c0, s.bg_channels, write_aux, tiles, L.V, L.P, b.ranges,
+                           b.point_list, g.rec, reinterpret_cast<const float4*>(featp), bg, *L.outs, im.final_T,
+                           im.n_contrib, use_tile_order(L.V, tiles) ? b.tile_order : nullptr, write_aux ? b.hits : nullptr);
     } else {
-        hipLaunchKernelGGL(composite_fwd_kernel<NC>, dim3(blocks), dim3(WAVE), 0, stream, s.image_width,
+        hipLaunchKernelGGL((composite_fwd_kernel<NC, false>), dim3(blocks), dim3(WAVE), 0, stream, s.image_width,
                            s.image_height, padded_channels(feat_stride) / 4, c0, s.bg_channels, write_aux, tiles, L.V, L.P, b.ranges,
                            b.ipack, b.irec, reinterpret_cast<const float4*>(featp), bg, *L.outs, im.final_T,
-                           im.n_contrib, use_tile_order(L.V, tiles) ? b.tile_order : nullptr);
+                           im.n_contrib, use_tile_order(L.V, tiles) ? b.tile_order : nullptr, nullptr);
     }
     SR_LAUNCH_CHECK();
     return SPLATRASTER_OK;
 }
 
 int launch_composite_fwd(const splatraster_settings& s, int32_t P, int32_t V, int64_t R, const GeomView& g, const BinView& b,
-                         const ImgView& im, const float* featp, const float* bg, const WinOut& outs, hipStream_t stream)
+                         const ImgView& im, const float* featp, const float* bg, const WinOut& outs, bool gather,
+                         hipStream_t stream)
 {
     (void)R;
     const int C = s.channels;
+    if (gather && !gather_layout(C)) return SPLATRASTER_ERR_UNSUPPORTED;
     const int tiles_v = ((s.image_width + TILE - 1) / TILE) * ((s.image_height + TILE - 1) / TILE);
     const bool team = g_fwd_team < 0 ? split_lists(C, V, tiles_v) : (g_fwd_team != 0 && C <= 4);
-    const FwdLaunch L{P, V, &outs, split_lists(C, V, tiles_v) ? b.ckpt : nullptr, team};
+    const FwdLaunch L{P, V, &outs, split_lists(C, V, tiles_v) ? b.ckpt : nullptr, team, gather};
     int c0 = 0, aux = 1, st = SPLATRASTER_OK;
 #define SR_FWD_CASE(N)                                                                              \
     case N:                                                                                         \
```

New measurement: 747.2 (median of 6 runs). 1.9% higher.
